# glacierbliss/iceberg_tracking_code

Measured on AMD Instinct MI355X. Metric: frame_pairs_per_sec, higher is better.
Workload: dtype u8/int32/f32

## Files before the change

### iceberg_tracking_code_amd/_lib.py

```python
import ctypes as C
import os

_HERE = os.path.dirname(os.path.abspath(__file__))
LIB_PATH = os.environ.get("ICELK_LIBRARY") or os.path.join(_HERE, "libicelk.so")

OK, EARG, ENOMEM, EHIP, ECAP, ESTATE, EUNSUP = 0, -1, -2, -3, -4, -5, -6

u8p = C.POINTER(C.c_uint8)
f32p = C.POINTER(C.c_float)
i32p = C.POINTER(C.c_int)
i64p = C.POINTER(C.c_int64)
f64p = C.POINTER(C.c_double)
vp = C.c_void_p
handle_p = C.c_void_p
i16p = C.POINTER(C.c_int16)


class JpegInfo(C.Structure):
    _fields_ = [("width", C.c_int32), ("height", C.c_int32), ("ncomp", C.c_int32), ("hmax", C.c_int32), ("vmax", C.c_int32),
                ("mcus_x", C.c_int32), ("mcus_y", C.c_int32), ("restart_interval", C.c_int32),
                ("comp_w", C.c_int32 * 3), ("comp_h", C.c_int32 * 3), ("blocks_x", C.c_int32 * 3), ("blocks_y", C.c_int32 * 3),
                ("coef_offset", C.c_uint64 * 3), ("coef_count", C.c_uint64), ("quant", (C.c_uint16 * 64) * 3)]


jpeg_info_p = C.POINTER(JpegInfo)


class JpegScan(C.Structure):
    _fields_ = [("segments", C.c_uint32), ("blocks_per_mcu", C.c_uint32), ("blocks_per_segment", C.c_uint32),
                ("total_blocks", C.c_uint32), ("component", C.c_uint8 * 8), ("dc_table", C.c_uint8 * 8), ("ac_table", C.c_uint8 * 8)]


class JpegHuffStats(C.Structure):
    _fields_ = [("segments", C.c_uint32), ("subsequences", C.c_uint32), ("rounds", C.c_uint32), ("max_hops", C.c_uint32),
                ("lanes_in_step", C.c_uint32), ("spanning_blocks", C.c_uint32), ("fallback", C.c_uint32), ("reserved", C.c_uint32),
                ("total_hops", C.c_uint64)]


JPEG_TABLE_BYTES = 11328
JPEG_FALLBACK_NONE, JPEG_FALLBACK_BOUND, JPEG_FALLBACK_STREAM, JPEG_FALLBACK_SIZE = 0, 1, 2, 3
jpeg_stats_p = C.POINTER(JpegHuffStats)

SIGNATURES = {
    "icelk_version": (C.c_int, []),
    "icelk_last_error": (C.c_char_p, [handle_p]),
    "icelk_create": (C.c_int, [C.c_int, C.c_int, C.c_int, C.c_int, C.c_int, C.POINTER(handle_p)]),
    "icelk_destroy": (C.c_int, [handle_p]),
    "icelk_set_stream": (C.c_int, [handle_p, vp]),
    "icelk_sync": (C.c_int, [handle_p]),
    "icelk_set_fb_distance": (C.c_int, [handle_p, C.c_int]),
    "icelk_set_lk_kernel": (C.c_int, [handle_p, C.c_int]),
    "icelk_upload_gray": (C.c_int, [handle_p, C.c_int, u8p, C.c_int, C.c_int, C.c_int]),
    "icelk_upload_bgr": (C.c_int, [handle_p, C.c_int, u8p, C.c_int, C.c_int, C.c_int, C.c_int]),
    "icelk_jpeg_describe": (C.c_int, [vp, C.c_uint64, jpeg_info_p]),
    "icelk_jpeg_read_coefficients": (C.c_int, [vp, C.c_uint64, vp, C.c_uint64]),
    "icelk_upload_jpeg": (C.c_int, [handle_p, C.c_int, jpeg_info_p, vp, C.c_int, C.c_int, C.c_int, C.c_int, C.c_int]),
    "icelk_jpeg_decode_rgb": (C.c_int, [handle_p, jpeg_info_p, vp, u8p, C.c_int]),
    "icelk_jpeg_index": (C.c_int, [vp, C.c_uint64, jpeg_info_p, C.POINTER(JpegScan), vp, vp, C.c_uint64, vp]),
    "icelk_jpeg_read_coefficients_lanes": (C.c_int, [vp, C.c_uint64, vp, C.c_uint64, C.c_int, C.c_int, C.c_int, jpeg_stats_p]),
    "icelk_jpeg_huff_config": (C.c_int, [handle_p, C.c_int, C.c_int, C.c_int]),
    "icelk_jpeg_huff_stats": (C.c_int, [handle_p, jpeg_stats_p]),
    "icelk_upload_jpeg_file": (C.c_int, [handle_p, C.c_int, vp, C.c_uint64, C.c_int, C.c_int, C.c_int, C.c_int, C.c_int]),
    "icelk_jpeg_decode_rgb_file": (C.c_int, [handle_p, vp, C.c_uint64, u8p, C.c_int]),
    "icelk_jpeg_device_coefficients": (C.c_int, [handle_p, vp, C.c_uint64, vp, C.c_uint64]),
    "icelk_set_gray_device": (C.c_int, [handle_p, C.c_int, vp, C.c_int, C.c_int, C.c_int]),
    "icelk_cvt_bgr_device": (C.c_int, [handle_p, C.c_int, vp, C.c_int, C.c_int, C.c_int, C.c_int]),
    "icelk_upload_gray_async": (C.c_int, [handle_p, C.c_int, vp, C.c_int, C.c_int, C.c_int]),
    "icelk_host_alloc": (C.c_int, [C.POINTER(vp), C.c_uint64]),
    "icelk_host_free": (C.c_int, [vp]),
    "icelk_synth_frame": (C.c_int, [handle_p, C.c_int, C.c_int, C.c_int, C.c_int64, C.c_int64, C.c_uint32]),
    "icelk_synth_frame_affine": (C.c_int, [handle_p, C.c_int, C.c_int, C.c_int, C.c_int64, C.c_int64, C.c_uint32, i32p]),
    "icelk_drop_pyramid": (C.c_int, [handle_p, C.c_int]),
    "icelk_download_level": (C.c_int, [handle_p, C.c_int, C.c_int, u8p, C.c_int, i32p, i32p]),
    "icelk_build_pyramid": (C.c_int, [handle_p, C.c_int, C.c_int, C.c_int, C.c_int, i32p]),
    "icelk_pyrlk": (C.c_int, [handle_p, C.c_int, C.c_int, f32p, f32p, u8p, f32p, C.c_int, C.c_int, C.c_int, C.c_int,
                              C.c_int, C.c_int, C.c_double, C.c_int, C.c_double]),
    "icelk_track_fb": (C.c_int, [handle_p, C.c_int, C.c_int, f32p, C.c_int, C.c_int, C.c_int, C.c_int, C.c_int,
                                 C.c_int, C.c_double, C.c_double, C.c_float, f32p, f32p, u8p, u8p, f32p, f32p, f32p,
                                 u8p]),
    "icelk_fb_filter": (C.c_int, [handle_p, f32p, f32p, C.c_int, C.c_float, f32p, u8p]),
    "icelk_set_mask": (C.c_int, [handle_p, u8p, C.c_int, C.c_int, C.c_int]),
    "icelk_min_eig_map": (C.c_int, [handle_p, C.c_int, C.c_int, f32p, C.c_int]),
    "icelk_good_features": (C.c_int, [handle_p, C.c_int, C.c_int, C.c_int, C.c_double, C.c_double, C.c_int, f32p,
                                      C.c_int, i32p]),
    "icelk_detect_stats": (C.c_int, [handle_p, i32p, i32p]),
    "icelk_seg_detect": (C.c_int, [handle_p, C.c_int, C.c_int, C.c_int, C.c_double, C.c_double, C.c_int, i32p]),
    "icelk_set_mask_polygon": (C.c_int, [handle_p, f64p, C.c_int, C.c_double, C.c_double, C.c_int, C.c_int]),
    "icelk_download_mask": (C.c_int, [handle_p, u8p, C.c_int, i32p, i32p]),
    "icelk_build_pyramid_ahead": (C.c_int, [handle_p, C.c_int, C.c_int, C.c_int, C.c_int]),
    "icelk_seg_detect_prepare": (C.c_int, [handle_p, C.c_int, C.c_int, C.c_int]),
    "icelk_seg_detect_begin": (C.c_int, [handle_p, C.c_int, C.c_int, C.c_int, C.c_double, C.c_double, C.c_int]),
    "icelk_seg_detect_finish": (C.c_int, [handle_p, C.c_int, i32p]),
    "icelk_seg_detect_cancel": (C.c_int, [handle_p]),
    "icelk_set_variant": (C.c_int, [handle_p, C.c_char_p, C.c_int]),
    "icelk_seg_detect_stage_try": (C.c_int, [handle_p, C.c_int, i32p, i32p]),
    "icelk_detect_fast_stats": (C.c_int, [handle_p, C.c_int, C.c_int, C.POINTER(C.c_longlong)]),
    "icelk_seg_detect_stage": (C.c_int, [handle_p, C.c_int, i32p]),
    "icelk_seg_switch": (C.c_int, [handle_p]),
    "icelk_seg_track": (C.c_int, [handle_p, C.c_int, C.c_int, C.c_int, C.c_int, C.c_int, C.c_int, C.c_int,
                                  C.c_double, C.c_double, C.c_float, i32p]),
    "icelk_seg_track_async": (C.c_int, [handle_p, C.c_int, C.c_int, C.c_int, C.c_int, C.c_int, C.c_int, C.c_int,
                                        C.c_double, C.c_double, C.c_float]),
    "icelk_seg_track_defer": (C.c_int, [handle_p, C.c_int, C.c_int, C.c_int, C.c_int, C.c_int, C.c_int, C.c_int,
                                        C.c_double, C.c_double, C.c_float]),
    "icelk_seg_flush": (C.c_int, [handle_p]),
    "icelk_seg_track_len_hint": (C.c_int, [handle_p, C.c_int]),
    "icelk_seg_template_stats": (C.c_int, [handle_p, C.POINTER(C.c_longlong)]),
    "icelk_seg_tail_stats": (C.c_int, [handle_p, C.POINTER(C.c_longlong)]),
    "icelk_seg_template_info": (C.c_int, [handle_p, C.POINTER(C.c_longlong), C.POINTER(C.c_longlong), i32p]),
    "icelk_seg_read_closed": (C.c_int, [handle_p, f32p, f32p, C.c_int, C.c_int, i32p, i32p]),
    "icelk_seg_archive_closed": (C.c_int, [handle_p, vp, vp, vp, C.c_int, i32p]),
    "icelk_seg_live": (C.c_int, [handle_p, i32p, i64p]),
    "icelk_seg_archive": (C.c_int, [handle_p, vp, vp, vp, C.c_int, i32p]),
    "icelk_project_tracks": (C.c_int, [handle_p, f32p, C.c_int, C.c_int, vp, vp, f64p, f64p, f64p, f64p, f64p, u8p]),
    "icelk_seg_project": (C.c_int, [handle_p, vp, vp, C.c_int, C.c_int, f64p, f64p, f64p, f64p, f64p, u8p, i32p, i32p]),
    "icelk_points_in_polygon": (C.c_int, [handle_p, f64p, C.c_int, f64p, C.c_int, u8p]),
    "icelk_grid_bin": (C.c_int, [handle_p, f64p, f64p, f64p, f64p, C.c_int, C.c_double, C.c_double, C.c_double, C.c_int,
                                 C.c_int, u8p, i32p, f64p, f64p, f64p]),
    "icelk_grid_bin_windows": (C.c_int, [handle_p, f64p, f64p, f64p, f64p, f64p, C.c_int, i64p, i32p, i32p, i32p,
                                         C.c_int, i64p, i64p, C.c_int, C.c_int, C.c_double, C.c_double, C.c_double,
                                         C.c_int, C.c_int, u8p, i32p, f64p, f64p, f64p, i32p, f64p, f64p, f64p]),
    "icelk_cube_set": (C.c_int, [handle_p, f64p, f64p, f64p, C.c_int, C.c_int]),
    "icelk_cube_release": (C.c_int, [handle_p]),
    "icelk_cube_average": (C.c_int, [handle_p, i32p, i32p, C.c_int, C.c_int, C.c_int, C.c_int, f64p, f64p, f64p, f64p,
                                     i32p, f64p]),
    "icelk_calib_set": (C.c_int, [handle_p, f64p, C.c_int, f64p, C.c_int, C.c_double, C.c_double]),
    "icelk_calib_release": (C.c_int, [handle_p]),
    "icelk_calib_residuals": (C.c_int, [handle_p, f64p, C.c_int, f64p, f64p, f64p, f64p]),
    "icelk_calib_cost": (C.c_int, [handle_p, f64p, C.c_int, f64p, f64p]),
    "icelk_seg_read": (C.c_int, [handle_p, f32p, f32p, C.c_int, C.c_int, i32p, i32p]),
    "icelk_prof_enable": (C.c_int, [handle_p, C.c_int]),
    "icelk_prof_reset": (C.c_int, [handle_p]),
    "icelk_prof_iterations": (C.c_int, [handle_p, C.POINTER(C.c_uint32), C.c_int, i32p]),
    "icelk_stream_probe_info": (C.c_int, [handle_p, i32p, f64p, f64p]),
    "icelk_prof_count": (C.c_int, []),
    "icelk_prof_name": (C.c_char_p, [C.c_int]),
    "icelk_prof_get": (C.c_int, [handle_p, C.c_int, i32p, f64p]),
}

_lib = None


class IcelkError(RuntimeError):
    """Raised for ICELK_EHIP / ICELK_ECAP / ICELK_ESTATE; bad arguments raise ValueError."""


def load():
    global _lib
    if _lib is None:
        if not os.path.exists(LIB_PATH):
            raise IcelkError(
                "libicelk.so is missing (%s). Build it with `python -m iceberg_tracking_code_amd.build` "
                "(needs hipcc); this package has no CPU fallback." % LIB_PATH)
        lib = C.CDLL(LIB_PATH)
        for name, (res, args) in SIGNATURES.items():
            fn = getattr(lib, name)
            fn.restype = res
            fn.argtypes = args
        _lib = lib
    return _lib


def check(rc, handle=None):
    if rc == OK:
        return
    msg = load().icelk_last_error(handle)
    msg = msg.decode() if msg else ""
    text = "icelk error %d: %s" % (rc, msg)
    if rc == EARG:
        raise ValueError(text)
    if rc == ENOMEM:
        raise MemoryError(text)
    raise IcelkError(text)
```

### iceberg_tracking_code_amd/context.py

```python
import ctypes as C

import numpy as np

from . import _lib
from ._lib import check, f32p, u8p

TERM_CRITERIA_COUNT = 1
TERM_CRITERIA_MAX_ITER = 1
TERM_CRITERIA_EPS = 2
OPTFLOW_USE_INITIAL_FLOW = 4
OPTFLOW_LK_GET_MIN_EIGENVALS = 8
GRAY_CV3 = 3
GRAY_CV4 = 4
LK_GENERIC_KERNEL = 0x100
LK_MULTI_PER_WAVE = 0x200
FB_HYPOT = 0
FB_SQRT = 1

DEFAULT_CRITERIA = (TERM_CRITERIA_COUNT | TERM_CRITERIA_EPS, 30, 0.01)


def _u8(a):
    return a.ctypes.data_as(u8p)

# ... 175 lines not shown
        st = np.zeros(n, np.uint8)
        er = np.zeros(n, np.float32)
        t, cnt, eps = _criteria(criteria)
        self._ck(self._lib.icelk_pyrlk(self._h, prev_slot, next_slot, _f32(p0), _f32(p1), _u8(st), _f32(er), n,
                                       winSize[0], winSize[1], maxLevel, t, cnt, eps, flags, minEigThreshold))
        return p1.reshape(-1, 1, 2), st.reshape(-1, 1), er.reshape(-1, 1)

    def track_fb(self, slot0, slot1, p0, winSize=(21, 21), maxLevel=3, criteria=DEFAULT_CRITERIA,
                 minEigThreshold=1e-4, fb_threshold=1.0):
        p0 = np.ascontiguousarray(p0, dtype=np.float32).reshape(-1, 2)
        n = p0.shape[0]
        out = dict(p1=np.zeros((n, 2), np.float32), p0r=np.zeros((n, 2), np.float32),
                   st_fwd=np.zeros(n, np.uint8), st_bwd=np.zeros(n, np.uint8),
                   err_fwd=np.zeros(n, np.float32), err_bwd=np.zeros(n, np.float32),
                   dist=np.zeros(n, np.float32), valid=np.zeros(n, np.uint8))
        t, cnt, eps = _criteria(criteria)
        self._ck(self._lib.icelk_track_fb(self._h, slot0, slot1, _f32(p0), n, winSize[0], winSize[1], maxLevel, t,
                                          cnt, eps, minEigThreshold, fb_threshold, _f32(out["p1"]),
                                          _f32(out["p0r"]), _u8(out["st_fwd"]), _u8(out["st_bwd"]),
                                          _f32(out["err_fwd"]), _f32(out["err_bwd"]), _f32(out["dist"]),
                                          _u8(out["valid"])))
        return out

    def fb_filter(self, p0, p0r, fb_threshold=1.0):
        a = np.ascontiguousarray(p0, dtype=np.float32).reshape(-1, 2)
        b = np.ascontiguousarray(p0r, dtype=np.float32).reshape(-1, 2)
        if a.shape != b.shape:
            raise ValueError("p0 and p0r differ in length")
        n = a.shape[0]
        dist, valid = np.zeros(n, np.float32), np.zeros(n, np.uint8)
        self._ck(self._lib.icelk_fb_filter(self._h, _f32(a), _f32(b), n, float(fb_threshold), _f32(dist), _u8(valid)))
        return dist, valid

    def set_mask(self, mask):
        if mask is None:
            self._ck(self._lib.icelk_set_mask(self._h, None, 0, 0, 0))
            return
        m = _gray2d(mask, "mask")
        self._ck(self._lib.icelk_set_mask(self._h, _u8(m), m.shape[1], m.shape[0], m.strides[0]))

    def set_mask_polygon(self, poly, crop_left, crop_top, w, h):
        p = np.ascontiguousarray(poly, dtype=np.float64).reshape(-1, 2)
        self._ck(self._lib.icelk_set_mask_polygon(self._h, p.ctypes.data_as(_lib.f64p), len(p), float(crop_left),
                                                  float(crop_top), int(w), int(h)))

    def download_mask(self):
        w, h = C.c_int(0), C.c_int(0)
        self._ck(self._lib.icelk_download_mask(self._h, None, 0, C.byref(w), C.byref(h)))
        m = np.empty((h.value, w.value), np.uint8)
        self._ck(self._lib.icelk_download_mask(self._h, _u8(m), w.value, C.byref(w), C.byref(h)))
        return m

    def min_eig_map(self, slot, blockSize=3):
        lvl = self.download_level(slot, 0)
        out = np.empty(lvl.shape, np.float32)
        self._ck(self._lib.icelk_min_eig_map(self._h, slot, blockSize, _f32(out), out.shape[1]))
        return out

    def good_features(self, slot, maxCorners, qualityLevel, minDistance, use_mask=False, blockSize=3):
        cap = self.max_pts if maxCorners <= 0 else min(int(maxCorners), self.max_pts)
        out = np.empty((max(cap, 1), 2), np.float32)
        n = C.c_int(0)
        self._ck(self._lib.icelk_good_features(self._h, slot, 1 if use_mask else 0, int(maxCorners),
                                               float(qualityLevel), float(minDistance), int(blockSize), _f32(out), cap,
                                               C.byref(n)))
        if n.value == 0:
            return None
        return out[:n.value].reshape(-1, 1, 2).copy()

    def detect_fast_stats(self, w, h):
        out = (C.c_longlong * 8)()
        self._ck(self._lib.icelk_detect_fast_stats(self._h, int(w), int(h), out))
        return dict(tiles=out[0], listed=out[1], whole_tiles=out[2], ties=out[3], max_listed=out[4], max_overflow_tiles=out[5],
                    longest_list=out[6], evaluated=out[7])

    def detect_stats(self):
        a, b = C.c_int(0), C.c_int(0)
        self._ck(self._lib.icelk_detect_stats(self._h, C.byref(a), C.byref(b)))
        return dict(candidates=a.value, accepted=b.value)

    def seg_detect(self, slot, maxCorners, qualityLevel, minDistance, use_mask=False, blockSize=3):
        n = C.c_int(0)
        self._ck(self._lib.icelk_seg_detect(self._h, slot, 1 if use_mask else 0, int(maxCorners), float(qualityLevel),
                                            float(minDistance), int(blockSize), C.byref(n)))
        return n.value

    def build_pyramid_ahead(self, slot, winSize=(21, 21), maxLevel=3):
        self._ck(self._lib.icelk_build_pyramid_ahead(self._h, slot, winSize[0], winSize[1], maxLevel))

    def seg_detect_prepare(self, slot, use_mask=False, blockSize=3):
        self._ck(self._lib.icelk_seg_detect_prepare(self._h, slot, 1 if use_mask else 0, int(blockSize)))

    def seg_detect_begin(self, slot, maxCorners, qualityLevel, minDistance, use_mask=False, blockSize=3):
        self._ck(self._lib.icelk_seg_detect_begin(self._h, slot, 1 if use_mask else 0, int(maxCorners),
                                                  float(qualityLevel), float(minDistance), int(blockSize)))

    def seg_detect_finish(self, maxCorners):
        n = C.c_int(0)
        self._ck(self._lib.icelk_seg_detect_finish(self._h, int(maxCorners), C.byref(n)))
        return n.value

    def seg_detect_stage(self, maxCorners):
        n = C.c_int(0)
        self._ck(self._lib.icelk_seg_detect_stage(self._h, int(maxCorners), C.byref(n)))
        return n.value

    def seg_detect_stage_try(self, maxCorners):
        n, done = C.c_int(0), C.c_int(0)
        self._ck(self._lib.icelk_seg_detect_stage_try(self._h, int(maxCorners), C.byref(n), C.byref(done)))
        return n.value if done.value else None

    def seg_detect_cancel(self):
        self._ck(self._lib.icelk_seg_detect_cancel(self._h))

    def seg_switch(self):
        self._ck(self._lib.icelk_seg_switch(self._h))

    def seg_track(self, slot_prev, slot_next, winSize=(21, 21), maxLevel=3, criteria=DEFAULT_CRITERIA,
                  minEigThreshold=1e-4, fb_threshold=1.0, wait=True):
        t, cnt, eps = _criteria(criteria)
        if wait:
            n = C.c_int(0)
            self._ck(self._lib.icelk_seg_track(self._h, slot_prev, slot_next, winSize[0], winSize[1], maxLevel, t, cnt,
                                               eps, minEigThreshold, fb_threshold, C.byref(n)))
            return n.value
        self._ck(self._lib.icelk_seg_track_async(self._h, slot_prev, slot_next, winSize[0], winSize[1], maxLevel, t,
                                                 cnt, eps, minEigThreshold, fb_threshold))
        return None

    def seg_track_defer(self, slot_prev, slot_next, winSize=(21, 21), maxLevel=3, criteria=DEFAULT_CRITERIA,
                        minEigThreshold=1e-4, fb_threshold=1.0):
        t, cnt, eps = _criteria(criteria)
        self._ck(self._lib.icelk_seg_track_defer(self._h, slot_prev, slot_next, winSize[0], winSize[1], maxLevel, t,
                                                 cnt, eps, minEigThreshold, fb_threshold))

    def seg_flush(self):
        self._ck(self._lib.icelk_seg_flush(self._h))

    def seg_template_stats(self):
        out = (C.c_longlong * 2)()
        self._ck(self._lib.icelk_seg_template_stats(self._h, out))
        return int(out[0]), int(out[1])

    def seg_template_info(self):
        by, rows, st = C.c_longlong(0), C.c_longlong(0), C.c_int(0)
        self._ck(self._lib.icelk_seg_template_info(self._h, C.byref(by), C.byref(rows), C.byref(st)))
        return int(by.value), int(rows.value), int(st.value)

    def seg_tail_stats(self):
        out = (C.c_longlong * 2)()
        self._ck(self._lib.icelk_seg_tail_stats(self._h, out))
        return int(out[0]), int(out[1])

    def seg_track_len_hint(self, track_len):
        self._ck(self._lib.icelk_seg_track_len_hint(self._h, int(track_len)))

    def seg_live(self):
        n, tot = C.c_int(0), C.c_int64(0)
        self._ck(self._lib.icelk_seg_live(self._h, C.byref(n), C.byref(tot)))
        return n.value, tot.value

    def seg_archive(self, dev_tracks_ptr, dev_quality_ptr, dev_count_ptr, cap_rows, closed=False):
        nv = C.c_int(0)
        fn = self._lib.icelk_seg_archive_closed if closed else self._lib.icelk_seg_archive
        self._ck(fn(self._h, C.c_void_p(dev_tracks_ptr), C.c_void_p(dev_quality_ptr or 0),
                                             C.c_void_p(dev_count_ptr), int(cap_rows), C.byref(nv)))
        return nv.value

    def seg_read(self, closed=False):
        n, nv = C.c_int(0), C.c_int(0)
        fn = self._lib.icelk_seg_read_closed if closed else self._lib.icelk_seg_read
        self._ck(fn(self._h, None, None, 0, 0, C.byref(n), C.byref(nv)))
        tracks = np.zeros((n.value, nv.value, 2), np.float32)
        quality = np.zeros((n.value, max(nv.value - 1, 0)), np.float32)
        if n.value:
            self._ck(fn(self._h, _f32(tracks), _f32(quality), n.value, nv.value, C.byref(n),
                                              C.byref(nv)))
        return tracks, quality

    def prof_enable(self, on=True):
        self._ck(self._lib.icelk_prof_enable(self._h, int(on)))

    def prof_reset(self):
        self._ck(self._lib.icelk_prof_reset(self._h))

    def prof_iterations(self):
        n = C.c_int(0)
        self._ck(self._lib.icelk_prof_iterations(self._h, None, 0, C.byref(n)))
        buf = np.zeros(max(n.value, 1), np.uint32)
        if n.value:
            self._ck(self._lib.icelk_prof_iterations(self._h, buf.ctypes.data_as(C.POINTER(C.c_uint32)), n.value,
                                                     C.byref(n)))
        buf = buf[:n.value]
        buf = buf[buf != 0xffffffff]
        return (buf & 0xffff).astype(np.int64), (buf >> 16).astype(np.int64)

    def stream_probe_info(self):
        picks = (C.c_int * 4)()
        q, lim = C.c_double(0), C.c_double(0)
        self._ck(self._lib.icelk_stream_probe_info(self._h, picks, C.byref(q), C.byref(lim)))
        return dict(detection=picks[0], candidates=picks[1], pyramid=picks[2], tail=picks[3], quickest=q.value,
                    limit=lim.value, probed=picks[0] >= 0)

    def prof_table(self):
        out = {}
        for k in range(self._lib.icelk_prof_count()):
            n, ms = C.c_int(0), C.c_double(0)
            self._ck(self._lib.icelk_prof_get(self._h, k, C.byref(n), C.byref(ms)))
            if n.value:
                out[self._lib.icelk_prof_name(k).decode()] = dict(launches=n.value, total_ms=ms.value,
                                                                  avg_us=1e3 * ms.value / n.value)
        return out
```

### iceberg_tracking_code_amd/csrc/abi_detect.hip

```cpp
#include "icelk_ctx.h"

namespace icelk {

int alloc_eig_out(Ctx* c, Ctx::EigOut& e, int cand_cap)
{
    const int w = c->max_w, h = c->max_h;
    int rc;
    if ((rc = dmalloc(c, &e.max_key, 1)) || (rc = dmalloc(c, &e.raw, (size_t)cand_cap)) ||
        (rc = dmalloc(c, &e.blk_count, candidate_blocks(w, h) * 4)))
        return rc;
    if (getenv("ICELK_TWO_PASS_CORNERS") &&
        ((rc = dmalloc(c, &e.acand, fast_cand_entries(w, h))) || (rc = dmalloc(c, &e.acount, fast_tiles(w, h))) ||
         (rc = dmalloc(c, &e.amaxc, fast_max_entries(w, h))) || (rc = dmalloc(c, &e.amaxn, fast_tiles(w, h))) ||
         (rc = dmalloc(c, &e.aemax, fast_tiles(w, h))) || (rc = dmalloc(c, &e.fmax_key, 8)) ||
         (rc = dmalloc(c, &e.aties, fast_cand_entries(w, h) + fast_tiles(w, h)))))
        return rc;
    if (hipEventCreateWithFlags(&e.done, hipEventDisableTiming) != hipSuccess) FAIL(c, ICELK_EHIP, "hipEventCreate failed");
    return ICELK_OK;
}

void free_eig_out(Ctx::EigOut& e)
{
    void* p[] = {e.raw, e.blk_count, e.max_key, e.acand, e.acount, e.amaxc, e.amaxn, e.aemax, e.fmax_key, e.aties};
    for (void* q : p)
// ... 135 lines not shown
static inline bool counts_here(const int* h_counts, int seq)
{
    return __atomic_load_n(h_counts + kCountsSeq, __ATOMIC_ACQUIRE) == seq;
}

static int fetch_counts(Ctx* c, Ctx::DetSet& S, bool published = false)
{
    if (!published) {
        int rc = publish_counts(c, S);
        if (rc) return rc;
    }
    for (unsigned it = 1;; it++) {
        if (counts_here(S.h_counts, S.counts_seq)) return ICELK_OK;
        if ((it & 4095u) == 0) {
            const hipError_t q = hipEventQuery(S.counts_ev);
            if (q == hipSuccess) break;
            if (q != hipErrorNotReady) HIPCHK(c, q);
            (void)hipGetLastError();
        }
        __builtin_ia32_pause();
    }
    HIPCHK(c, hipEventSynchronize(S.counts_ev));
    return ICELK_OK;
}

static int pick_mask(Ctx* c, int use_mask, int w, int h, const uint8_t** mask)
{
    *mask = nullptr;
    if (!use_mask) return ICELK_OK;
    if (!c->has_mask) FAIL(c, ICELK_ESTATE, "use_mask set but no mask uploaded");
    if (c->mask_w != w || c->mask_h != h) FAIL(c, ICELK_EARG, "mask size differs from the frame");
    *mask = c->d_mask;
    return ICELK_OK;
}

int detect_prepare(Ctx* c, int slot, int use_mask, int block_size)
{
    Range rg("icelk detect_prepare (corner candidates ahead)");
    int rc = check_slot(c, slot, true);
    if (rc) return rc;
    if (!fused_block_size(block_size) || getenv("ICELK_GENERIC_CORNERS") || c->corner_variant) return ICELK_OK;
    Slot& s = c->slots[slot];
    const uint8_t* mask = nullptr;
    if ((rc = pick_mask(c, use_mask, s.w, s.h, &mask))) return rc;
    const Ctx::EigOut want = eo_want(c, slot, use_mask, block_size);
    Ctx::EigOut& e = c->eo[eo_free(c, want)];
    if (eo_holds(e, want)) return ICELK_OK;
    const hipStream_t es = c->eig_stream;
    if (int rcw = wait_event(c, es, s.frame_ev)) return rcw;
    HIPCHK(c, hipMemsetAsync(e.max_key, 0, sizeof(unsigned), es));
    DetectScratch T{};
    point_at_eig_out(T, e);
    const double prep_quality = c->prep_quality;
    {
        ProfScope p(c, K_EIG, es);
        launch_candidates(es, T, s.lv[0], block_size, mask, c->mask_pitch, prep_quality, false, nullptr);
    }
    rc = check_launch(c, "corner candidates (prepared)");
    if (rc) return rc;
    HIPCHK(c, hipEventRecord(e.done, es));
    HIPCHK(c, hipEventRecord(s.eig_used, es));
    e.nblk = T.src_nblk;
    e.region = T.src_region;
    e.valid = true;
    e.slot = slot;
    e.gen = s.gen;
    e.block_size = block_size;
    e.use_mask = use_mask;
    e.mask_gen = c->mask_gen;
    e.quality = prep_quality;
    return ICELK_OK;
}

int detect_begin(Ctx* c, int slot, int use_mask, int max_corners, double quality, double min_distance, int block_size,
                 bool for_segment)
{
    Range rg("icelk detect_begin (candidates + min-distance stage)");
    int rc = check_slot(c, slot, true);
    if (rc) return rc;
    if (!(quality > 0) || min_distance < 0 || block_size <= 0) FAIL(c, ICELK_EARG, "bad detector parameters");
    if (min_eig_lds_bytes(block_size) > 150 * 1024) FAIL(c, ICELK_EARG, "blockSize too large");
    const int k = det_free(c);
    if (k < 0) FAIL(c, ICELK_ESTATE, "two detections are in flight already");
    c->dset_last = k;
    Ctx::DetSet& S = c->dset[k];
    Slot& s = c->slots[slot];
    const hipStream_t ds = c->det_stream;
    const int w = s.w, h = s.h;
    const uint8_t* mask = nullptr;
    if ((rc = pick_mask(c, use_mask, w, h, &mask))) return rc;
    DetectScratch& D = S.D;
    size_t ncell = 0;
    if (min_distance >= 1) {
        const int cell = (int)lrint(min_distance);
        ncell = (size_t)((w + cell - 1) / cell) * ((h + cell - 1) / cell);
        if (ncell + 1 > c->ncell_cap) FAIL(c, ICELK_ECAP, "cell grid larger than allocated");
    }
    if (int rcw = wait_event(c, ds, s.frame_ev)) return rcw;
    if (int rcw = wait_event(c, ds, S.tail_done)) return rcw;
    const bool generic = getenv("ICELK_GENERIC_CORNERS") != nullptr || c->corner_variant != 0;
    const bool need_reset = !S.counters_clean || ncell > S.reset_ncell;
    const Ctx::EigOut want = eo_want(c, slot, use_mask, block_size);
    const int spare_idx = eo_free(c, want);
    Ctx::EigOut& spare = c->eo[spare_idx];
    const bool prepared = eo_holds(spare, want) && !generic && spare.quality <= quality;
    c->prep_quality = quality;
    spare.valid = false;
    if (prepared) {
        if (need_reset) launch_detect_reset(ds, D, (int)ncell, 1);
        activate_eig_out(c, S, spare_idx);
        if (int rcw = wait_event(c, ds, spare.done)) return rcw;
    } else {
        ProfScope p(c, K_EIG, ds);
        activate_eig_out(c, S, spare_idx);
        if (int rcw = wait_event(c, ds, spare.done)) return rcw;
        HIPCHK(c, hipMemsetAsync(spare.max_key, 0, sizeof(unsigned), ds));
        if (need_reset) launch_detect_reset(ds, D, (int)ncell, 1);
        launch_candidates(ds, D, s.lv[0], block_size, mask, c->mask_pitch, quality, generic, nullptr, c->corner_variant);
        HIPCHK(c, hipEventRecord(s.det_used, ds));
    }
    S.counters_clean = false;
    rc = check_launch(c, "corner candidates");
    if (rc) return rc;
    DetectJob& J = S.job;
    J.w = w;
    J.h = h;
    J.quality = quality;
    J.min_distance = min_distance;
    J.ncell = ncell;
    J.prune_want = 0;
    if (min_distance >= 1 && max_corners > 0 && max_corners <= (1 << 24) && !getenv("ICELK_NO_PRUNE"))
        J.prune_want = (int)std::min(8.0 * max_corners, std::ceil(c->prune_factor * max_corners));
    J.dev_tail = false;
    J.seg_set = -1;
    J.max_corners = max_corners;
    const bool dev_tail = for_segment && !c->host_tail && min_distance >= 1;
    if (min_distance >= 1) {
        J.cand_count_ptr = D.cell_start + ncell;
        ProfScope p(c, K_SUPPRESS, ds);
        launch_min_distance(ds, D, w, h, min_distance, quality, J.prune_want, dev_tail);
        if (dev_tail)
            launch_tail_gather(ds, D, (int)ncell, quality, suppress_launch_count() - 1, max_corners, c->max_pts, c->tail_force_status);
    } else {
        J.cand_count_ptr = D.cand_count;
        launch_flatten(ds, D, quality);
    }
    rc = check_launch(c, "min_distance");
    if (rc) return rc;
    if (dev_tail) {
        const Ctx::DetSet& other = c->dset[k ^ 1];
        const int ahead = (c->seg_staged ? 1 : 0) + (other.job.active ? 1 : 0);
        const int target = (c->sb_cur + 1 + ahead) % kSegSets;
        Ctx::SegBuf& nb = c->sb[target];
        if (int rcw = wait_event(c, ds, nb.used)) return rcw;
        S.counts_seq = (S.counts_seq + 1) & 0x3fffffff;
        {
            ProfScope p(c, K_EMIT, ds);
            launch_tail_device(ds, D, quality, nb.live, nb.alive, nb.tracks, kMaxVert, c->use_order ? nb.order : nullptr,
                               nb.order_border, tail_order_geometry(w, h, c->border_px), tail_reset_of(D, (int)ncell),
                               S.h_counts, kCountsSeq, S.counts_seq);
        }
        rc = check_launch(c, "tail (device-driven)");
        if (rc) return rc;
        HIPCHK(c, hipEventRecord(nb.ready, ds));
        HIPCHK(c, hipEventRecord(S.counts_ev, ds));
        J.dev_tail = true;
        J.seg_set = target;
    } else {
        rc = publish_counts(c, S);
        if (rc) return rc;
    }
    J.active = true;
    J.seq = ++c->job_seq;
    return ICELK_OK;
}

int detect_finish(Ctx* c, int max_corners, int cap, int* n_out, Ctx::SegBuf* seg, bool* seg_done, bool* dev_done,
                  DetectJob* finished)
{
    Range rg("icelk detect_finish (host round trip, sort, corner list)");
    if (seg_done) *seg_done = false;
    if (dev_done) *dev_done = false;
    const int k = det_oldest(c);
    if (k < 0) FAIL(c, ICELK_ESTATE, "no detection in flight");
    c->dset_last = k;
    Ctx::DetSet& S = c->dset[k];
    DetectJob& J = S.job;
    J.active = false;
    if (finished) *finished = J;
    *n_out = 0;
    const hipStream_t ds = c->det_stream;
    const hipStream_t ts = c->tail_stream;
    DetectScratch& D = S.D;
    int rc = fetch_counts(c, S, true);
    if (rc) return rc;
    if (J.dev_tail) {
        const int status = S.h_counts[5];
        if (!seg || seg != &c->sb[J.seg_set] || max_corners != J.max_corners)
            FAIL(c, ICELK_ESTATE, "the segment staged is not the one its detection was begun for (set / maxCorners differ)");
        if (status == TAIL_OVERFLOW) FAIL(c, ICELK_ECAP, "more corners than the output capacity (raise max_pts)");
        if (status == TAIL_OK) {
            const int total = S.h_counts[1], n = S.h_counts[4];
            if (n > cap) FAIL(c, ICELK_ECAP, "more corners than the output capacity (raise max_pts)");
            if (J.prune_want > 0 && max_corners > 0)
                c->prune_factor = !S.h_counts[3] || total <= 0 ? 8.0 : std::min(8.0, std::max(2.0, 1.5 * (double)S.h_counts[0] / total));
            c->last_candidates = S.h_counts[0];
            c->last_accepted = total;
            S.reset_ncell = J.ncell;
            S.counters_clean = true;
            c->tails_dev++;
            *n_out = n;
            if (seg_done) *seg_done = true;
            if (dev_done) *dev_done = true;
            return ICELK_OK;
        }
    }
    c->tails_host++;
    const unsigned long long* sorted = nullptr;
    int total = 0;
    if (J.min_distance >= 1) {
        auto converge = [&]() -> int {
            for (int guard = 0; S.h_counts[2] != 0; guard++) {
                if (guard > 100000) FAIL(c, ICELK_EHIP, "min-distance suppression did not converge");
                continue_min_distance(ds, D, J.w, J.h, J.min_distance);
                int r = fetch_counts(c, S);
                if (r) return r;
            }
            return ICELK_OK;
        };
        if ((rc = converge())) return rc;
        bool redone = false;
        if (J.prune_want > 0 && S.h_counts[3] && (max_corners <= 0 || S.h_counts[1] < max_corners)) {
            redone = true;
            launch_detect_reset(ds, D, (int)J.ncell, 0);
            launch_min_distance(ds, D, J.w, J.h, J.min_distance, J.quality, 0);
            if ((rc = check_launch(c, "min_distance (unpruned)"))) return rc;
            if ((rc = fetch_counts(c, S))) return rc;
            if ((rc = converge())) return rc;
        }
        total = S.h_counts[1];
        if (J.prune_want > 0 && max_corners > 0) {
            const bool fell_short = !S.h_counts[3] || redone;
            c->prune_factor = fell_short || total <= 0 ? 8.0 : std::min(8.0, std::max(2.0, 1.5 * (double)S.h_counts[0] / total));
        }
        c->last_candidates = S.h_counts[0];
        c->last_accepted = total;
        if (total == 0) return ICELK_OK;
        sort_keys_desc(ts, D, D.acc, D.acc_sorted, total);
        sorted = D.acc_sorted;
    } else {
        total = S.h_counts[0];
        c->last_candidates = total;
        c->last_accepted = total;
        if (total == 0) return ICELK_OK;
        sort_keys_desc(ts, D, D.cand, D.cell_cand, total);
        sorted = D.cell_cand;
    }
    rc = check_launch(c, "sort");
    if (rc) return rc;
    int n = total;
    if (max_corners > 0 && n > max_corners) n = max_corners;
    if (n > cap || n > c->max_pts) FAIL(c, ICELK_ECAP, "more corners than the output capacity (raise max_pts)");
    if (seg) {
        if (int rcw = wait_event(c, ts, seg->used)) return rcw;
        {
            ProfScope p(c, K_EMIT, ts);
            launch_tail_fused(ts, sorted, n, c->d_corners, seg->live, seg->alive, seg->tracks, kMaxVert, D, (int)J.ncell, 1);
        }
        rc = check_launch(c, "tail");
        if (rc) return rc;
        HIPCHK(c, hipEventRecord(c->det_done, ts));
        HIPCHK(c, hipEventRecord(S.tail_done, ts));
        *seg_done = true;
    } else {
        {
            ProfScope p(c, K_EMIT, ts);
            launch_emit_corners(ts, sorted, n, J.w, c->d_corners);
        }
        rc = check_launch(c, "emit");
        if (rc) return rc;
        HIPCHK(c, hipEventRecord(c->det_done, ts));
        launch_detect_reset(ts, D, (int)J.ncell, 1);
        HIPCHK(c, hipEventRecord(S.tail_done, ts));
    }
    S.reset_ncell = J.ncell;
    S.counters_clean = true;
    *n_out = n;
    return ICELK_OK;
}

static int detect_core(Ctx* c, int slot, int use_mask, int max_corners, double quality, double min_distance,
                       int block_size, int cap, int* n_out)
{
    *n_out = 0;
    if (det_oldest(c) >= 0) FAIL(c, ICELK_ESTATE, "a detection is in flight (icelk_seg_detect_begin without _stage / _finish)");
    int rc = detect_begin(c, slot, use_mask, max_corners, quality, min_distance, block_size, false);
    if (rc) return rc;
    return detect_finish(c, max_corners, cap, n_out);
}

int detect_counts_arrived(Ctx* c, bool* arrived)
{
    *arrived = false;
    const int k = det_oldest(c);
    if (k < 0) FAIL(c, ICELK_ESTATE, "no detection in flight");
    if (!counts_here(c->dset[k].h_counts, c->dset[k].counts_seq)) {
// ... 181 lines not shown
```

### iceberg_tracking_code_amd/csrc/abi_handle.hip

```cpp
#include <dlfcn.h>

#include <chrono>

#include "icelk_ctx.h"

namespace icelk {

static const char* kKernelNames[K_COUNT_] = {
    "bgr2gray", "pyrdown", "lk", "lk_fb", "corner_candidates", "min_distance", "sort_emit",
    "project_tracks", "synth", "lk_fb_pair", "jpeg_idct", "jpeg_out", "jpeg_huff",
};

std::string g_create_err;
std::mutex g_mu;

Roctx::Roctx()
{
    if (!getenv("ICELK_ROCTX")) return;
    void* lib = dlopen("librocprofiler-sdk-roctx.so", RTLD_NOW | RTLD_GLOBAL);
    if (!lib) lib = dlopen("libroctx64.so", RTLD_NOW | RTLD_GLOBAL);
    if (!lib) return;
    push = reinterpret_cast<int (*)(const char*)>(dlsym(lib, "roctxRangePushA"));
    pop = reinterpret_cast<int (*)()>(dlsym(lib, "roctxRangePop"));
    if (!push || !pop) push = nullptr;
}

Roctx& roctx()
{
    static Roctx r;
    return r;
}

void prof_drain(Ctx* c)
{
    for (auto& e : c->evts) {
        hipEventSynchronize(e.b);
        float ms = 0.f;
        if (hipEventElapsedTime(&ms, e.a, e.b) == hipSuccess) {
            c->prof_ms[e.id] += ms;
            c->prof_launches[e.id] += 1;
        }
        c->evt_pool.push_back(e);
    }
    c->evts.clear();
}

hipError_t create_priority_stream(hipStream_t* s)
{
    int least = 0, greatest = 0;
    hipError_t e = hipDeviceGetStreamPriorityRange(&least, &greatest);
    if (e != hipSuccess) return e;
    return hipStreamCreateWithPriority(s, hipStreamNonBlocking, greatest);
}

__global__ void k_probe_idle(unsigned ticks)
{
    const unsigned long long t0 = __builtin_amdgcn_s_memrealtime();
    for (int guard = 0; guard < 200000; guard++) {
        if (__builtin_amdgcn_s_memrealtime() - t0 >= ticks) break;
        __builtin_amdgcn_s_sleep(8);
    }
}

__global__ void k_probe_tick(unsigned* out)
{
    if (out) *out = 1u;
}

static double probe_pair(hipStream_t busy, hipStream_t side, hipEvent_t e_busy, hipEvent_t e_side)
{
    using clk = std::chrono::steady_clock;
    hipStreamSynchronize(busy);
    hipStreamSynchronize(side);
    const auto t0 = clk::now();
    hipLaunchKernelGGL(k_probe_idle, dim3(65536), dim3(64), 0, busy, 2500u);
    hipEventRecord(e_busy, busy);
    hipLaunchKernelGGL(k_probe_tick, dim3(1), dim3(64), 0, side, (unsigned*)nullptr);
    hipEventRecord(e_side, side);
    hipEventSynchronize(e_side);
    const auto t1 = clk::now();
    hipEventSynchronize(e_busy);
    const auto t2 = clk::now();
    const double whole = std::chrono::duration<double>(t2 - t0).count();
    const double frac = whole > 0 ? std::chrono::duration<double>(t1 - t0).count() / whole : 1.0;
    if (getenv("ICELK_STREAM_PROBE_LOG"))
        fprintf(stderr, "icelk probe: busy %p side %p: side done after %.2f of %.0f us\n", (void*)busy, (void*)side, frac, 1e6 * whole);
    return frac;
}

static hipError_t create_side_streams(Ctx* c)
{
    constexpr int NC = 8;
    hipStream_t cand[NC] = {nullptr};
    hipEvent_t ea = nullptr, eb = nullptr;
    hipError_t r = hipEventCreateWithFlags(&ea, hipEventDisableTiming);
    if (r == hipSuccess) r = hipEventCreateWithFlags(&eb, hipEventDisableTiming);
    for (int i = 0; i < NC && r == hipSuccess; i++) r = create_priority_stream(&cand[i]);
    if (r == hipSuccess) {
        probe_pair(c->own_stream, cand[0], ea, eb);
        double beside[NC], quickest = 1.0;
        for (int i = 0; i < NC; i++) {
            beside[i] = std::min(probe_pair(c->own_stream, cand[i], ea, eb), probe_pair(c->own_stream, cand[i], ea, eb));
            quickest = std::min(quickest, beside[i]);
        }
        const double limit = std::max(1.6 * quickest, quickest + 0.12);
        bool used[NC] = {false};
        auto pick = [&](auto ok) {
            for (int i = 0; i < NC; i++)
                if (!used[i] && beside[i] <= limit && ok(cand[i])) { used[i] = true; return i; }
            for (int i = 0; i < NC; i++)
                if (!used[i]) { used[i] = true; return i; }
            return 0;
        };
        const int d = pick([&](hipStream_t) { return true; });
        c->det_stream = cand[d];
        const int e = pick([&](hipStream_t s) { return probe_pair(s, c->det_stream, ea, eb) <= limit; });
        c->eig_stream = cand[e];
        const int q = pick([&](hipStream_t s) { return probe_pair(c->eig_stream, s, ea, eb) <= limit; });
        c->pyr_stream = cand[q];
        const int t = pick([&](hipStream_t s) { return probe_pair(c->eig_stream, s, ea, eb) <= limit; });
        c->tail_stream = cand[t];
        c->side_pick[0] = d;
        c->side_pick[1] = e;
        c->side_pick[2] = q;
        c->side_pick[3] = t;
        c->probe_limit = limit;
        c->probe_quickest = quickest;
        if (getenv("ICELK_STREAM_PROBE_LOG"))
            fprintf(stderr, "icelk probe: detection = candidate %d, candidates stream = %d, pyramid = %d (limit %.2f)\n", d, e, q, limit);
        for (int i = 0; i < NC; i++)
            if (!used[i]) hipStreamDestroy(cand[i]);
    } else {
        for (auto s : cand)
            if (s) hipStreamDestroy(s);
    }
    if (ea) hipEventDestroy(ea);
    if (eb) hipEventDestroy(eb);
    return r;
}

static void destroy_ctx(Ctx* c)
{
    if (!c) return;
    hipSetDevice(c->device);
    if (c->stream) hipStreamSynchronize(c->stream);
    prof_drain(c);
    for (auto& e : c->evt_pool) {
        hipEventDestroy(e.a);
        hipEventDestroy(e.b);
    }
    if (c->d_stamps) {
        std::vector<unsigned long long> hs(3 * c->stamps_cap);
        if (hipMemcpy(hs.data(), c->d_stamps, hs.size() * 8, hipMemcpyDeviceToHost) == hipSuccess) {
            if (FILE* f = fopen(c->stamps_path.c_str(), "wb")) {
                fwrite(hs.data(), 8, hs.size(), f);
                fclose(f);
            }
        }
        hipFree(c->d_stamps);
    }
    if (c->d_iters) hipFree(c->d_iters);
    for (void* b : c->tmpl.buf)
        if (b) hipFree(b);
    for (auto& s : c->slots) {
        if (s.base) hipFree(s.base);
        if (s.ready) hipEventDestroy(s.ready);
        if (s.frame_ev) hipEventDestroy(s.frame_ev);
        if (s.used_own) hipEventDestroy(s.used_own);
        if (s.det_used) hipEventDestroy(s.det_used);
        if (s.eig_used) hipEventDestroy(s.eig_used);
    }
    if (c->det_stream) hipStreamSynchronize(c->det_stream);
    if (c->eig_stream) hipStreamSynchronize(c->eig_stream);
    if (c->det_done) hipEventDestroy(c->det_done);
    if (c->corners_free) hipEventDestroy(c->corners_free);
    if (c->det_stream) hipStreamDestroy(c->det_stream);
    if (c->eig_stream) hipStreamDestroy(c->eig_stream);
    for (auto& b : c->sb) {
        if (b.used_own) hipEventDestroy(b.used_own);
        if (b.ready) hipEventDestroy(b.ready);
    }
    for (auto& e : c->launch_ev)
        if (e) hipEventDestroy(e);
    for (auto& e : c->eo) free_eig_out(e);
    for (auto& S : c->dset) free_det_set(S);
    if (c->h_seg) hipHostFree(c->h_seg);
    void* ptrs[] = {c->d_bgr, c->d_mask, c->d_p0, c->d_p1, c->d_p0r, c->d_err_f, c->d_err_b, c->d_dist, c->d_corners,
                    c->d_st_f, c->d_st_b, c->d_valid, c->dset[0].D.eig, c->d_tracked,
                    c->d_out_tracks, c->d_out_quality, c->post.d_proj, c->post.d_keep, c->post.d_cube_u, c->post.d_cube_v,
                    c->post.d_cube_count, c->calib.d_shore, c->calib.d_water, c->jpeg.d_coef, c->jpeg.d_planes, c->jpeg.d_rgb,
                    c->jpeg.d_file, c->jpeg.d_seg, c->jpeg.d_tabs, c->jpeg.d_T, c->jpeg.d_X, c->jpeg.d_cnt, c->jpeg.d_P, c->jpeg.d_ctl,
                    c->jpeg.d_dc};
    for (void* p : ptrs)
        if (p) hipFree(p);
    for (auto& S : c->sb) {
        void* sp[] = {S.live, S.alive, S.order, S.order_border, S.tracks, S.quality};
        for (void* p : sp)
            if (p) hipFree(p);
    }
    if (c->own_stream) hipStreamDestroy(c->own_stream);
    for (auto q : c->copy_hi)
        if (q) {
            hipStreamSynchronize(q);
            hipStreamDestroy(q);
        }
    if (c->pyr_stream) {
        hipStreamSynchronize(c->pyr_stream);
        hipStreamDestroy(c->pyr_stream);
    }
    if (c->tail_stream) {
        hipStreamSynchronize(c->tail_stream);
        hipStreamDestroy(c->tail_stream);
    }
    delete c;
}

}

using namespace icelk;

extern "C" {

int icelk_version(void) { return 100; }

const char* icelk_last_error(icelk_t* h)
{
    if (!h) return g_create_err.c_str();
    return C(h)->err.c_str();
}

int icelk_create(int device, int max_w, int max_h, int n_slots, int max_pts, icelk_t** out)
{
    std::lock_guard<std::mutex> lk(g_mu);
    if (!out || max_w <= 0 || max_h <= 0 || max_w > 65535 || max_h > 65535 || n_slots <= 0 || max_pts <= 0) {
        g_create_err = "icelk_create: bad argument";
        return ICELK_EARG;
    }
    *out = nullptr;
    int ndev = 0;
    hipError_t e = hipGetDeviceCount(&ndev);
    if (e != hipSuccess || ndev == 0) {
        g_create_err = std::string("icelk_create: no HIP device (") + hipGetErrorString(e) + ")";
        return ICELK_EHIP;
    }
    if (device < 0 || device >= ndev) {
        g_create_err = "icelk_create: device index out of range";
        return ICELK_EARG;
    }
    e = hipSetDevice(device);
    if (e != hipSuccess) {
        g_create_err = std::string("hipSetDevice: ") + hipGetErrorString(e);
        return ICELK_EHIP;
    }
    Ctx* c = new Ctx();
    c->device = device;
    c->max_w = max_w;
    c->max_h = max_h;
    c->n_slots = n_slots;
    c->max_pts = max_pts;
    int rc = ICELK_OK;
    auto fail = [&](int code) {
        g_create_err = c->err;
        destroy_ctx(c);
        return code;
    };
    if (hipStreamCreateWithFlags(&c->own_stream, hipStreamNonBlocking) != hipSuccess ||
        create_side_streams(c) != hipSuccess ||
        hipHostMalloc(reinterpret_cast<void**>(&c->h_seg), 64, hipHostMallocMapped) != hipSuccess ||
        hipEventCreateWithFlags(&c->det_done, hipEventDisableTiming) != hipSuccess ||
        hipEventCreateWithFlags(&c->corners_free, hipEventDisableTiming) != hipSuccess) {
        c->err = "hipStreamCreate failed";
        return fail(ICELK_EHIP);
    }
    c->stream = c->own_stream;
    c->slots.resize(n_slots);
    const size_t sb = slot_bytes(max_w, max_h);
    for (auto& s : c->slots) {
        if ((rc = dmalloc(c, &s.base, sb))) return fail(rc);
        s.bytes = sb;
        if (hipEventCreateWithFlags(&s.ready, hipEventDisableTiming) != hipSuccess ||
            hipEventCreateWithFlags(&s.frame_ev, hipEventDisableTiming) != hipSuccess ||
            hipEventCreateWithFlags(&s.used_own, hipEventDisableTiming) != hipSuccess ||
            hipEventCreateWithFlags(&s.det_used, hipEventDisableTiming) != hipSuccess ||
            hipEventCreateWithFlags(&s.eig_used, hipEventDisableTiming) != hipSuccess) {
            c->err = "hipEventCreate failed";
            return fail(ICELK_EHIP);
        }
        s.used = s.used_own;
        layout_levels(s, max_w, max_h);
        if (!layout_ok(s)) {
            c->err = "slot layout violates the dword-access invariant (internal)";
            return fail(ICELK_ECAP);
        }
    }
    for (auto& S : c->sb) {
        if (hipEventCreateWithFlags(&S.used_own, hipEventDisableTiming) != hipSuccess ||
            hipEventCreateWithFlags(&S.ready, hipEventDisableTiming) != hipSuccess) {
            c->err = "hipEventCreate failed";
            return fail(ICELK_EHIP);
        }
        S.used = S.used_own;
    }
    for (auto& e : c->launch_ev)
        if (hipEventCreateWithFlags(&e, hipEventDisableTiming) != hipSuccess) {
            c->err = "hipEventCreate failed";
            return fail(ICELK_EHIP);
        }
    const size_t npx = (size_t)max_w * max_h;
    c->bgr_pitch = align_up(3 * max_w, kPitchAlign);
    c->mask_pitch = align_up(max_w, kPitchAlign);
    const size_t np = (size_t)max_pts;
    const int cand_cap = (int)std::min<size_t>(candidate_capacity(max_w, max_h), (size_t)1 << 30);
    c->ncell_cap = npx + 1;
    if ((rc = dmalloc(c, &c->d_bgr, (size_t)c->bgr_pitch * max_h)) || (rc = dmalloc(c, &c->d_mask, (size_t)c->mask_pitch * max_h)) ||
        (rc = dmalloc(c, &c->d_p0, 2 * np)) || (rc = dmalloc(c, &c->d_p1, 2 * np)) || (rc = dmalloc(c, &c->d_p0r, 2 * np)) ||
        (rc = dmalloc(c, &c->d_err_f, np)) || (rc = dmalloc(c, &c->d_err_b, np)) || (rc = dmalloc(c, &c->d_dist, np)) ||
        (rc = dmalloc(c, &c->d_corners, 2 * np)) || (rc = dmalloc(c, &c->d_st_f, np)) || (rc = dmalloc(c, &c->d_st_b, np)) ||
        (rc = dmalloc(c, &c->d_valid, np)) || (rc = dmalloc(c, &c->dset[0].D.eig, npx)) || (rc = dmalloc(c, &c->d_tracked, 64)) ||
        (rc = dmalloc(c, &c->d_out_tracks, np * kMaxVert * 2)) || (rc = dmalloc(c, &c->d_out_quality, np * (kMaxVert - 1))))
        return fail(rc);
    for (auto& S : c->sb)
        if ((rc = dmalloc(c, &S.live, 2 * np)) || (rc = dmalloc(c, &S.alive, np)) || (rc = dmalloc(c, &S.order, np)) ||
            (rc = dmalloc(c, &S.order_border, 1)) || (rc = dmalloc(c, &S.tracks, np * kMaxVert * 2)) ||
            (rc = dmalloc(c, &S.quality, np * (kMaxVert - 1))))
            return fail(rc);
    c->use_order = getenv("ICELK_NO_ORDER") == nullptr;
    c->pyr_per_level = getenv("ICELK_PYR_PER_LEVEL") != nullptr;
    c->tmpl.off = getenv("ICELK_NO_TEMPLATE_REUSE") != nullptr;
    if (const char* tb = getenv("ICELK_TEMPLATE_BUDGET_MB")) c->tmpl.budget = (size_t)std::max(atoll(tb), 0LL) << 20;
    c->host_tail = getenv("ICELK_HOST_TAIL") != nullptr;
    if (const char* fs = getenv("ICELK_TAIL_FORCE_STATUS")) c->tail_force_status = std::min(std::max(atoi(fs), 0), 4);
    if ((rc = dmalloc(c, &c->d_iters, (size_t)max_pts))) return fail(rc);
    if (const char* sp = getenv("ICELK_LK_STAMPS")) {
        c->stamps_path = sp;
        c->stamps_cap = (size_t)max_pts + 8;
        if ((rc = dmalloc(c, &c->d_stamps, 3 * c->stamps_cap))) return fail(rc);
    }
    if (const char* k = getenv("ICELK_LK_KERNEL")) {
        if (!strcmp(k, "generic")) c->lk_kernel_flags = ICELK_FLAG_GENERIC_KERNEL;
        else if (!strcmp(k, "multi")) c->lk_kernel_flags = ICELK_FLAG_MULTI_PER_WAVE;
    }
    for (auto& e : c->eo)
        if ((rc = alloc_eig_out(c, e, cand_cap))) return fail(rc);
    for (int k = 0; k < 2; k++) {
        Ctx::DetSet& S = c->dset[k];
        S.D.eig = c->dset[0].D.eig;
        if ((rc = alloc_det_set(c, S, cand_cap))) return fail(rc);
        activate_eig_out(c, S, k);
    }
    if (hipMemset(c->d_tracked, 0, 64 * 8) != hipSuccess) {
        c->err = "hipMemset failed";
        return fail(ICELK_EHIP);
    }
    DetectScratch& D0 = c->dset[0].D;
    if (hipMemsetAsync(D0.acc, 0, 64 * sizeof(unsigned long long), c->tail_stream) != hipSuccess) {
        c->err = "hipMemset failed";
        return fail(ICELK_EHIP);
    }
    sort_keys_desc(c->tail_stream, D0, D0.acc, D0.acc_sorted, 64);
    if (hipStreamSynchronize(c->tail_stream) != hipSuccess) {
        c->err = "warm-up sort failed";
        return fail(ICELK_EHIP);
    }
    *out = reinterpret_cast<icelk_t*>(c);
    return ICELK_OK;
}

int icelk_destroy(icelk_t* h)
{
    if (!h) return ICELK_EARG;
    destroy_ctx(C(h));
    return ICELK_OK;
}

int icelk_set_stream(icelk_t* h, void* hip_stream)
{
    if (!h) return ICELK_EARG;
    Ctx* c = C(h);
    HIPCHK(c, hipSetDevice(c->device));
    HIPCHK(c, hipStreamSynchronize(c->stream));
    c->stream = hip_stream ? reinterpret_cast<hipStream_t>(hip_stream) : c->own_stream;
    return ICELK_OK;
}

int icelk_sync(icelk_t* h)
{
    if (!h) return ICELK_EARG;
    Ctx* c = C(h);
    HIPCHK(c, hipSetDevice(c->device));
    int rcf = flush_deferred(c);
    if (rcf) return rcf;
    for (auto q : c->copy_hi)
        if (q) HIPCHK(c, hipStreamSynchronize(q));
    HIPCHK(c, hipStreamSynchronize(c->pyr_stream));
    HIPCHK(c, hipStreamSynchronize(c->eig_stream));
    HIPCHK(c, hipStreamSynchronize(c->det_stream));
    HIPCHK(c, hipStreamSynchronize(c->tail_stream));
    HIPCHK(c, hipStreamSynchronize(c->stream));
    return ICELK_OK;
}

int icelk_set_lk_kernel(icelk_t* h, int which)
{
    if (!h) return ICELK_EARG;
    Ctx* c = C(h);
    if (which != 0 && which != ICELK_FLAG_GENERIC_KERNEL && which != ICELK_FLAG_MULTI_PER_WAVE)
        FAIL(c, ICELK_EARG, "bad kernel selector");
    c->lk_kernel_flags = which;
    return ICELK_OK;
}

int icelk_set_variant(icelk_t* h, const char* name, int value)
{
    if (!h || !name) return ICELK_EARG;
    Ctx* c = C(h);
    if (!strcmp(name, "lk_sums") && value >= 0 && value <= 2) c->lk_sum_mode = value;
    else if (!strcmp(name, "lk_wide_sums") && (value == 0 || value == 1)) c->lk_wide_sums = value;
    else if (!strcmp(name, "sobel_fma") && value >= 0 && value <= 3) c->corner_variant = (c->corner_variant & 4) | value;
    else if (!strcmp(name, "eig_fma") && (value == 0 || value == 1)) c->corner_variant = (c->corner_variant & 3) | (value << 2);
    else FAIL(c, ICELK_EARG, "unknown variant / value");
    for (auto& e : c->eo) e.valid = false;
    return ICELK_OK;
}

int icelk_set_fb_distance(icelk_t* h, int form)
{
    if (!h) return ICELK_EARG;
    Ctx* c = C(h);
    if (form != ICELK_FB_HYPOT && form != ICELK_FB_SQRT) FAIL(c, ICELK_EARG, "bad forward-backward distance form");
    c->fb_dist_form = form;
    return ICELK_OK;
}

int icelk_prof_enable(icelk_t* h, int on)
{
    if (!h) return ICELK_EARG;
    Ctx* c = C(h);
    if (!on) prof_drain(c);
    c->prof = on != 0;
    c->prof_tracker_only = on == 2;
    return ICELK_OK;
}

int icelk_prof_reset(icelk_t* h)
{
    if (!h) return ICELK_EARG;
    Ctx* c = C(h);
    prof_drain(c);
    for (int i = 0; i < K_COUNT_; i++) {
        c->prof_launches[i] = 0;
        c->prof_ms[i] = 0;
    }
    return ICELK_OK;
}

int icelk_prof_iterations(icelk_t* h, uint32_t* host_out, int cap, int* out_n)
{
    if (!h) return ICELK_EARG;
    Ctx* c = C(h);
    HIPCHK(c, hipSetDevice(c->device));
    if (!out_n || cap < 0 || (cap > 0 && !host_out)) FAIL(c, ICELK_EARG, "bad output buffer");
    *out_n = c->iters_n;
    if (host_out && cap > 0 && c->iters_n > 0) {
        const int n = c->iters_n < cap ? c->iters_n : cap;
        HIPCHK(c, hipStreamSynchronize(c->stream));
        HIPCHK(c, hipMemcpy(host_out, c->d_iters, sizeof(uint32_t) * (size_t)n, hipMemcpyDeviceToHost));
    }
    return ICELK_OK;
}

int icelk_stream_probe_info(icelk_t* h, int* picks, double* quickest, double* limit)
{
    if (!h) return ICELK_EARG;
    Ctx* c = C(h);
    if (picks)
        for (int k = 0; k < 4; k++) picks[k] = c->side_pick[k];
    if (quickest) *quickest = c->probe_quickest;
    if (limit) *limit = c->probe_limit;
    return ICELK_OK;
}

int icelk_prof_count(void) { return K_COUNT_; }

const char* icelk_prof_name(int kernel_id)
{
    if (kernel_id < 0 || kernel_id >= K_COUNT_) return "";
    return kKernelNames[kernel_id];
}

int icelk_prof_get(icelk_t* h, int kernel_id, int* launches, double* total_ms)
{
    if (!h) return ICELK_EARG;
    Ctx* c = C(h);
    if (kernel_id < 0 || kernel_id >= K_COUNT_) FAIL(c, ICELK_EARG, "bad kernel id");
    prof_drain(c);
    if (launches) *launches = c->prof_launches[kernel_id];
    if (total_ms) *total_ms = c->prof_ms[kernel_id];
    return ICELK_OK;
}

}
```

### iceberg_tracking_code_amd/csrc/abi_lk.hip

```cpp
#include "icelk_ctx.h"

namespace icelk {

int make_lk_params(Ctx* c, int w, int h, int win_w, int win_h, int max_level, int crit_type, int max_count,
                   double epsilon, int flags, double min_eig_thr, float fb_thr, LKParams* P)
{
    if (win_w <= 2 || win_h <= 2) FAIL(c, ICELK_EARG, "winSize must be > 2");
    if (max_level < 0) FAIL(c, ICELK_EARG, "maxLevel must be >= 0");
    if (max_level > kMaxLevels - 1) max_level = kMaxLevels - 1;
    if (win_w * win_h > 64 * 64) FAIL(c, ICELK_EARG, "winSize area above 4096 px is not supported");
    P->win_w = win_w;
    P->win_h = win_h;
    P->top_level = pyramid_top_level(w, h, win_w, win_h, max_level);
    if (!(crit_type & ICELK_CRIT_COUNT)) max_count = 30;
    else max_count = std::min(std::max(max_count, 0), 100);
    if (!(crit_type & ICELK_CRIT_EPS)) epsilon = 0.01;
    else epsilon = std::min(std::max(epsilon, 0.), 10.);
    P->max_count = max_count;
    P->eps2 = epsilon * epsilon;
    if (P->eps2 < 1e-30) {
        P->eps2_lo = -1.f;
        P->eps2_hi = INFINITY;
    } else {
        P->eps2_lo = nextafterf((float)(P->eps2 * (1.0 - 1.0 / (1 << 20))), -INFINITY);
        P->eps2_hi = nextafterf((float)(P->eps2 * (1.0 + 1.0 / (1 << 20))), INFINITY);
    }
    P->flags = flags | c->lk_kernel_flags;
    P->min_eig_thr = (float)min_eig_thr;
    P->fb_thr = fb_thr;
    P->margin = 6;
    P->dist_form = c->fb_dist_form;
    P->sum_mode = c->lk_sum_mode;
    P->sum_guard = c->lk_wide_sums ? 0u : 1u << 26;
    return ICELK_OK;
}

static int lk_prologue(Ctx* c, int slot0, int slot1, const float* p0, bool have_bufs, int n, int win_w, int win_h,
                       int max_level, int crit_type, int max_count, double epsilon, int flags, double min_eig_threshold,
                       float fb_threshold, LKParams* P)
{
    int rc = check_slot(c, slot0, true);
    if (!rc) rc = check_slot(c, slot1, true);
    if (rc) return rc;
    if (n < 0) FAIL(c, ICELK_EARG, "negative point count");
    if (n > c->max_pts) FAIL(c, ICELK_ECAP, "more points than max_pts of icelk_create");
    const Slot& s0 = c->slots[slot0];
    const Slot& s1 = c->slots[slot1];
    if (s0.w != s1.w || s0.h != s1.h) FAIL(c, ICELK_EARG, "frame sizes differ");
    rc = make_lk_params(c, s0.w, s0.h, win_w, win_h, max_level, crit_type, max_count, epsilon, flags, min_eig_threshold,
                        fb_threshold, P);
    if (rc) return rc;
    if (n == 0) return ICELK_OK;
    if (!have_bufs) FAIL(c, ICELK_EARG, "null point buffer");
    rc = ensure_pyramid(c, slot0, P->top_level);
    if (!rc) rc = ensure_pyramid(c, slot1, P->top_level);
    if (rc) return rc;
    HIPCHK(c, hipMemcpyAsync(c->d_p0, p0, sizeof(float) * 2 * n, hipMemcpyHostToDevice, c->stream));
    return ICELK_OK;
}

}

using namespace icelk;

extern "C" {

int icelk_pyrlk(icelk_t* h, int prev_slot, int next_slot, const float* prev_xy, float* next_xy, uint8_t* status,
                float* err, int n, int win_w, int win_h, int max_level, int crit_type, int max_count, double epsilon,
                int flags, double min_eig_threshold)
{
    if (!h) return ICELK_EARG;
    Ctx* c = C(h);
    HIPCHK(c, hipSetDevice(c->device));
    LKParams P;
    int rc = lk_prologue(c, prev_slot, next_slot, prev_xy, prev_xy && next_xy, n, win_w, win_h, max_level, crit_type,
                         max_count, epsilon, flags, min_eig_threshold, 1.f, &P);
    if (rc || n == 0) return rc;
    const Slot& s0 = c->slots[prev_slot];
    const Slot& s1 = c->slots[next_slot];
    if (flags & ICELK_FLAG_INITIAL_FLOW)
        HIPCHK(c, hipMemcpyAsync(c->d_p1, next_xy, sizeof(float) * 2 * n, hipMemcpyHostToDevice, c->stream));
    LKBuffers B{};
    B.p_in = c->d_p0;
    B.p_fwd = c->d_p1;
    B.st_fwd = c->d_st_f;
    B.err_fwd = err ? c->d_err_f : nullptr;
    if (c->prof) { B.iters = c->d_iters; c->iters_n = n; }
    {
        ProfScope p(c, K_LK);
        rc = launch_lk(c->stream, pyramid_of(s0), pyramid_of(s1), B, n, P, false);
    }
    if (rc) FAIL(c, rc, "unsupported window size");
    rc = check_launch(c, "lk");
    if (rc) return rc;
    HIPCHK(c, hipMemcpyAsync(next_xy, c->d_p1, sizeof(float) * 2 * n, hipMemcpyDeviceToHost, c->stream));
    if (status) HIPCHK(c, hipMemcpyAsync(status, c->d_st_f, n, hipMemcpyDeviceToHost, c->stream));
    if (err) HIPCHK(c, hipMemcpyAsync(err, c->d_err_f, sizeof(float) * n, hipMemcpyDeviceToHost, c->stream));
    HIPCHK(c, hipStreamSynchronize(c->stream));
    return ICELK_OK;
}

int icelk_track_fb(icelk_t* h, int slot0, int slot1, const float* p0, int n, int win_w, int win_h, int max_level,
                   int crit_type, int max_count, double epsilon, double min_eig_threshold, float fb_threshold,
                   float* p1, float* p0r, uint8_t* st_fwd, uint8_t* st_bwd, float* err_fwd, float* err_bwd, float* dist,
                   uint8_t* valid)
{
    if (!h) return ICELK_EARG;
    Ctx* c = C(h);
    HIPCHK(c, hipSetDevice(c->device));
    LKParams P;
    int rc = lk_prologue(c, slot0, slot1, p0, p0 != nullptr, n, win_w, win_h, max_level, crit_type, max_count, epsilon, 0,
                         min_eig_threshold, fb_threshold, &P);
    if (rc || n == 0) return rc;
    const Slot& s0 = c->slots[slot0];
    const Slot& s1 = c->slots[slot1];
    LKBuffers B{};
    B.p_in = c->d_p0;
    B.p_fwd = c->d_p1;
    B.st_fwd = c->d_st_f;
    B.err_fwd = err_fwd ? c->d_err_f : nullptr;
    B.p_bwd = c->d_p0r;
    B.st_bwd = c->d_st_b;
    B.err_bwd = err_bwd ? c->d_err_b : nullptr;
    B.dist = c->d_dist;
    B.valid = c->d_valid;
    if (c->prof) { B.iters = c->d_iters; c->iters_n = n; }
    {
        ProfScope p(c, K_LK_FB);
        rc = launch_lk(c->stream, pyramid_of(s0), pyramid_of(s1), B, n, P, true);
    }
    if (rc) FAIL(c, rc, "unsupported window size");
    rc = check_launch(c, "lk_fb");
    if (rc) return rc;
    const size_t fb = sizeof(float) * n;
    if (p1) HIPCHK(c, hipMemcpyAsync(p1, c->d_p1, 2 * fb, hipMemcpyDeviceToHost, c->stream));
    if (p0r) HIPCHK(c, hipMemcpyAsync(p0r, c->d_p0r, 2 * fb, hipMemcpyDeviceToHost, c->stream));
    if (st_fwd) HIPCHK(c, hipMemcpyAsync(st_fwd, c->d_st_f, n, hipMemcpyDeviceToHost, c->stream));
    if (st_bwd) HIPCHK(c, hipMemcpyAsync(st_bwd, c->d_st_b, n, hipMemcpyDeviceToHost, c->stream));
    if (err_fwd) HIPCHK(c, hipMemcpyAsync(err_fwd, c->d_err_f, fb, hipMemcpyDeviceToHost, c->stream));
    if (err_bwd) HIPCHK(c, hipMemcpyAsync(err_bwd, c->d_err_b, fb, hipMemcpyDeviceToHost, c->stream));
    if (dist) HIPCHK(c, hipMemcpyAsync(dist, c->d_dist, fb, hipMemcpyDeviceToHost, c->stream));
    if (valid) HIPCHK(c, hipMemcpyAsync(valid, c->d_valid, n, hipMemcpyDeviceToHost, c->stream));
    HIPCHK(c, hipStreamSynchronize(c->stream));
    return ICELK_OK;
}

int icelk_fb_filter(icelk_t* h, const float* p0, const float* p0r, int n, float fb_threshold, float* dist,
                    uint8_t* valid)
{
    if (!h) return ICELK_EARG;
    Ctx* c = C(h);
    HIPCHK(c, hipSetDevice(c->device));
    if (n < 0) FAIL(c, ICELK_EARG, "negative point count");
    if (n > c->max_pts) FAIL(c, ICELK_ECAP, "more points than max_pts of icelk_create");
    if (n == 0) return ICELK_OK;
    if (!p0 || !p0r) FAIL(c, ICELK_EARG, "null point buffer");
    HIPCHK(c, hipMemcpyAsync(c->d_p0, p0, sizeof(float) * 2 * n, hipMemcpyHostToDevice, c->stream));
    HIPCHK(c, hipMemcpyAsync(c->d_p0r, p0r, sizeof(float) * 2 * n, hipMemcpyHostToDevice, c->stream));
    launch_fb_filter(c->stream, c->d_p0, c->d_p0r, n, fb_threshold, c->fb_dist_form, c->d_dist, c->d_valid);
    int rc = check_launch(c, "fb_filter");
    if (rc) return rc;
    if (dist) HIPCHK(c, hipMemcpyAsync(dist, c->d_dist, sizeof(float) * n, hipMemcpyDeviceToHost, c->stream));
    if (valid) HIPCHK(c, hipMemcpyAsync(valid, c->d_valid, n, hipMemcpyDeviceToHost, c->stream));
    HIPCHK(c, hipStreamSynchronize(c->stream));
    return ICELK_OK;
}

}
```

### iceberg_tracking_code_amd/csrc/abi_segments.hip

```cpp
#include "icelk_ctx.h"

namespace icelk {

static int seg_wait(Ctx* c)
{
    if (c->seg_ready_pending) {
        if (int rcw = wait_event(c, c->stream, c->sb[c->sb_cur].ready)) return rcw;
        c->seg_ready_pending = false;
    }
    return ICELK_OK;
}

static LKJob seg_job(Ctx* c, int set, const Slot& s0, const Slot& s1, const LKParams& P, bool primary)
{
    Ctx::SegBuf& S = c->sb[set];
    LKJob j{};
    j.I = pyramid_of(s0);
    j.J = pyramid_of(s1);
    j.n = S.upper;
    LKBuffers& B = j.B;
    B.p_in = S.live;
    if (primary) {
        B.p_fwd = c->d_p1;
        B.st_fwd = c->d_st_f;
        B.p_bwd = c->d_p0r;
        B.st_bwd = c->d_st_b;
        B.dist = c->d_dist;
        B.valid = c->d_valid;
    }
    B.seg_alive = S.alive;
    B.order = c->use_order ? S.order : nullptr;
    B.order_border = c->use_order ? S.order_border : nullptr;
    const double overlap = (double)(P.win_w + 12) * (P.win_h + 12) * S.upper / ((double)s0.w * s0.h);
    B.order_plain = overlap >= 2.0 ? 1 : 0;
    B.seg_xy = S.live;
    B.seg_tracks = S.tracks;
    B.seg_quality = S.quality;
    B.seg_vert = S.vert;
    B.seg_max_vert = kMaxVert;
    B.seg_tracked = c->d_tracked;
    const int quads = lk_fast_eligible(P) ? lk_template_quads(P.win_w, P.win_h) : 0;
    const int key = (P.win_w << 16) | (P.win_h << 8) | (P.top_level + 1);
    const int slot0 = (int)(&s0 - c->slots.data()), slot1 = (int)(&s1 - c->slots.data());
    bool take = quads > 0 && S.tmpl_for == S.vert && S.tmpl_key == key && S.tmpl_slot == slot0 && S.tmpl_gen == s0.gen;
    S.tmpl_for = -1;
    if (quads > 0 && !c->tmpl.off) {
        const bool last = c->track_len_hint > 0 && S.vert >= c->track_len_hint;
        const size_t per_row = (size_t)(P.top_level + 1) * ((size_t)quads * 64) * 16;
        const size_t need = (size_t)std::max(S.upper, 1) * per_row;
        if (!last && c->tmpl.row_bytes != per_row) {
            if (c->defer.pending) (void)flush_deferred(c);
            for (void*& b : c->tmpl.buf) {
                if (b) hipFree(b);
                b = nullptr;
            }
            c->tmpl.bytes = 0;
            c->tmpl.row_bytes = per_row;
            for (Ctx::SegBuf& o : c->sb) o.tmpl_for = -1;
            size_t free_b = 0, total_b = 0;
            if (hipMemGetInfo(&free_b, &total_b) != hipSuccess) free_b = 0;
            const size_t budget = std::min(c->tmpl.budget / 2, free_b / 4);
            const size_t rows = std::min((size_t)std::max(c->max_pts, 1), budget / per_row);
            const size_t alloc = rows * per_row;
            if (rows > 0 && hipMalloc(&c->tmpl.buf[0], alloc) == hipSuccess && hipMalloc(&c->tmpl.buf[1], alloc) == hipSuccess) {
                c->tmpl.bytes = alloc;
            } else {
                (void)hipGetLastError();
                if (c->tmpl.buf[0]) hipFree(c->tmpl.buf[0]);
                c->tmpl.buf[0] = c->tmpl.buf[1] = nullptr;
                c->tmpl.off = true;
                c->tmpl.failed = true;
            }
        }
        if (c->tmpl.row_bytes != per_row) take = false;
        if (c->tmpl.bytes >= need && c->tmpl.row_bytes == per_row) {
            B.tmpl_levels = P.top_level + 1;
            if (take) {
                B.tmpl_in = c->tmpl.buf[set & 1];
                c->tmpl.taken++;
            }
            if (!last) {
                c->tmpl.left++;
                B.tmpl_out = c->tmpl.buf[set & 1];
                S.tmpl_for = S.vert + 1;
                S.tmpl_key = key;
                S.tmpl_slot = slot1;
                S.tmpl_gen = s1.gen;
            }
        }
    }
    return j;
}

static int record_launch(Ctx* c, hipEvent_t* ev)
{
    *ev = c->launch_ev[c->launch_seq++ % kLaunchEvents];
    HIPCHK(c, hipEventRecord(*ev, c->stream));
    return ICELK_OK;
}

static void seg_launched(Ctx* c, hipEvent_t ev, int set, int slot_prev, int slot_next)
{
    c->slots[slot_prev].used = ev;
    c->slots[slot_next].used = ev;
    c->sb[set].used = ev;
}

int flush_deferred(Ctx* c)
{
    if (!c->defer.pending) return ICELK_OK;
    Ctx::Deferred& d = c->defer;
    d.pending = false;
    int rc;
    {
        ProfScope p(c, K_LK_FB);
        rc = launch_lk(c->stream, d.job.I, d.job.J, d.job.B, d.job.n, d.P, true);
    }
    if (rc) FAIL(c, rc, "unsupported window size");
    rc = check_launch(c, "lk_fb");
    if (rc) return rc;
    hipEvent_t ev;
    rc = record_launch(c, &ev);
    if (rc) return rc;
    seg_launched(c, ev, d.set, d.slot_prev, d.slot_next);
    return ICELK_OK;
}

int flush_deferred_slot(Ctx* c, int slot)
{
    if (c->defer.pending && (c->defer.slot_prev == slot || c->defer.slot_next == slot)) return flush_deferred(c);
    return ICELK_OK;
}

static bool same_lk_params(const LKParams& a, const LKParams& b)
{
    return a.win_w == b.win_w && a.win_h == b.win_h && a.top_level == b.top_level && a.max_count == b.max_count &&
           a.eps2 == b.eps2 && a.flags == b.flags && a.min_eig_thr == b.min_eig_thr && a.fb_thr == b.fb_thr &&
           a.margin == b.margin && a.dist_form == b.dist_form && a.sum_mode == b.sum_mode &&
           a.sum_guard == b.sum_guard;
}

static int seg_track_core(Ctx* c, int slot_prev, int slot_next, int win_w, int win_h, int max_level, int crit_type,
                          int max_count, double epsilon, double min_eig_threshold, float fb_threshold, bool defer)
{
    Range rg(defer ? "icelk seg_track_defer" : "icelk seg_track (fused forward+backward LK launch)");
    int rc = check_slot(c, slot_prev, true);
    if (!rc) rc = check_slot(c, slot_next, true);
    if (rc) return rc;
    if (!c->seg_active) FAIL(c, ICELK_ESTATE, "icelk_seg_detect has not been called");
    Ctx::SegBuf& S = c->sb[c->sb_cur];
    if (S.vert >= kMaxVert) FAIL(c, ICELK_ECAP, "segment longer than the device track table");
    Slot& s0 = c->slots[slot_prev];
    Slot& s1 = c->slots[slot_next];
    if (s0.w != s1.w || s0.h != s1.h) FAIL(c, ICELK_EARG, "frame sizes differ");
    LKParams P;
    rc = make_lk_params(c, s0.w, s0.h, win_w, win_h, max_level, crit_type, max_count, epsilon, 0, min_eig_threshold,
                        fb_threshold, &P);
    if (rc) return rc;
    if (c->defer.pending && c->defer.set == c->sb_cur) {
        rc = flush_deferred(c);
        if (rc) return rc;
    }
    rc = ensure_pyramid(c, slot_prev, P.top_level);
    if (!rc) rc = ensure_pyramid(c, slot_next, P.top_level);
    if (rc) return rc;
    rc = seg_wait(c);
    if (rc) return rc;
    if (S.upper > 0) {
        c->border_px = (std::max(win_w, win_h) / 2 + kLkTileMargin + 2) << std::max(P.top_level - 1, 0);
        LKJob job = seg_job(c, c->sb_cur, s0, s1, P, true);
        static const bool stamp_pairs = getenv("ICELK_LK_STAMPS_PAIR") != nullptr;
        const bool diag = c->d_stamps != nullptr && !stamp_pairs;
        if (defer && !c->defer.pending && !diag) {
            Ctx::Deferred& d = c->defer;
            d.pending = true;
            d.set = c->sb_cur;
            d.slot_prev = slot_prev;
            d.slot_next = slot_next;
            d.job = job;
            d.P = P;
            S.vert += 1;
            return ICELK_OK;
        }
        bool paired = false;
        if (c->defer.pending) {
            Ctx::Deferred& d = c->defer;
            if (!diag && same_lk_params(d.P, P)) {
                LKJob other = d.job;
                other.B.p_fwd = other.B.p_bwd = other.B.err_fwd = other.B.err_bwd = other.B.dist = nullptr;
                other.B.st_fwd = other.B.st_bwd = other.B.valid = nullptr;
                if (c->d_stamps && stamp_pairs && (size_t)(other.n + job.n + 32) <= c->stamps_cap) {
                    other.B.stamps = job.B.stamps = c->d_stamps;
                    hipMemsetAsync(c->d_stamps, 0, 3 * c->stamps_cap * 8, c->stream);
                }
                {
                    ProfScope p(c, K_LK_FB_PAIR);
                    paired = launch_lk_pair(c->stream, other, job, P);
                }
                if (paired) {
                    d.pending = false;
                    rc = check_launch(c, "lk_fb_pair");
                    if (rc) return rc;
                }
            }
            if (!paired) {
                rc = flush_deferred(c);
                if (rc) return rc;
            }
        }
        if (!paired) {
            LKBuffers& B = job.B;
            if (c->prof) {
                B.iters = c->d_iters;
                c->iters_n = S.upper;
                hipMemsetAsync(c->d_iters, 0xff, sizeof(uint32_t) * (size_t)S.upper, c->stream);
            }
            if (c->d_stamps && !stamp_pairs) {
                B.stamps = c->d_stamps;
                hipMemsetAsync(c->d_stamps, 0, 3 * c->stamps_cap * 8, c->stream);
            }
            {
                ProfScope p(c, K_LK_FB);
                rc = launch_lk(c->stream, job.I, job.J, B, job.n, P, true);
            }
            if (rc) FAIL(c, rc, "unsupported window size");
            rc = check_launch(c, "lk_fb");
            if (rc) return rc;
        }
        hipEvent_t ev;
        rc = record_launch(c, &ev);
        if (rc) return rc;
        if (paired) seg_launched(c, ev, c->defer.set, c->defer.slot_prev, c->defer.slot_next);
        seg_launched(c, ev, c->sb_cur, slot_prev, slot_next);
    } else if (c->defer.pending && !defer) {
        rc = flush_deferred(c);
        if (rc) return rc;
    }
    S.vert += 1;
    return ICELK_OK;
}

}

using namespace icelk;

extern "C" {

int icelk_seg_detect_begin(icelk_t* h, int slot, int use_mask, int max_corners, double quality_level,
                            double min_distance, int block_size)
{
    if (!h) return ICELK_EARG;
    Ctx* c = C(h);
    HIPCHK(c, hipSetDevice(c->device));
    return detect_begin(c, slot, use_mask, max_corners, quality_level, min_distance, block_size, true);
}

int icelk_seg_detect_prepare(icelk_t* h, int slot, int use_mask, int block_size)
{
    if (!h) return ICELK_EARG;
    Ctx* c = C(h);
    HIPCHK(c, hipSetDevice(c->device));
    if (block_size <= 0) FAIL(c, ICELK_EARG, "bad detector parameters");
    return detect_prepare(c, slot, use_mask, block_size);
}

static int seg_stage(Ctx* c, int max_corners, int* out_n)
{
    if (c->seg_staged) FAIL(c, ICELK_ESTATE, "a staged segment is waiting for icelk_seg_switch");
    int n = 0;
    Ctx::SegBuf& nb = c->sb[(c->sb_cur + 1) % kSegSets];
    bool tables_written = false, dev_done = false;
    DetectJob job;
    int rc = detect_finish(c, max_corners, c->max_pts, &n, &nb, &tables_written, &dev_done, &job);
    if (rc) return rc;
    if (!dev_done) {
        const hipStream_t ds = c->tail_stream;
        if (!tables_written) {
            if (int rcw = wait_event(c, ds, nb.used)) return rcw;
            launch_seg_init(ds, c->d_corners, n, nb.live, nb.alive, nb.tracks, kMaxVert);
        }
        if (c->use_order) launch_seg_order(ds, c->d_corners, n, job.w, job.h, c->border_px, nb.order, nb.order_border);
        rc = check_launch(c, "seg_init");
        if (rc) return rc;
        HIPCHK(c, hipEventRecord(c->corners_free, ds));
        HIPCHK(c, hipEventRecord(nb.ready, ds));
    }
    c->seg_staged = true;
    c->staged_n = n;
    if (out_n) *out_n = n;
    return ICELK_OK;
}

static int seg_switch(Ctx* c)
{
    if (!c->seg_staged) FAIL(c, ICELK_ESTATE, "no staged segment (icelk_seg_detect_stage has not been called)");
    if (c->defer.pending && c->defer.set != c->sb_cur) {
        int rc = flush_deferred(c);
        if (rc) return rc;
    }
    c->seg_staged = false;
    c->closed_valid = c->seg_active;
    c->sb_cur = (c->sb_cur + 1) % kSegSets;
    c->seg_ready_pending = true;
    c->sb[c->sb_cur].vert = 1;
    c->sb[c->sb_cur].tmpl_for = -1;
    c->sb[c->sb_cur].upper = c->staged_n;
    c->seg_active = true;
    return ICELK_OK;
}

int icelk_seg_detect_stage(icelk_t* h, int max_corners, int* out_n)
{
    if (!h) return ICELK_EARG;
    Ctx* c = C(h);
    HIPCHK(c, hipSetDevice(c->device));
    return seg_stage(c, max_corners, out_n);
}

int icelk_seg_detect_stage_try(icelk_t* h, int max_corners, int* out_n, int* out_done)
{
    if (!h || !out_done) return ICELK_EARG;
    Ctx* c = C(h);
    HIPCHK(c, hipSetDevice(c->device));
    *out_done = 0;
    if (c->seg_staged) FAIL(c, ICELK_ESTATE, "a staged segment is waiting for icelk_seg_switch");
    bool arrived = false;
    int rc = detect_counts_arrived(c, &arrived);
    if (rc || !arrived) return rc;
    rc = seg_stage(c, max_corners, out_n);
    if (rc) return rc;
    *out_done = 1;
    return ICELK_OK;
}

int icelk_seg_switch(icelk_t* h)
{
    if (!h) return ICELK_EARG;
    return seg_switch(C(h));
}

int icelk_seg_detect_cancel(icelk_t* h)
{
    if (!h) return ICELK_EARG;
    Ctx* c = C(h);
    HIPCHK(c, hipSetDevice(c->device));
    HIPCHK(c, hipStreamSynchronize(c->eig_stream));
    HIPCHK(c, hipStreamSynchronize(c->det_stream));
    HIPCHK(c, hipStreamSynchronize(c->tail_stream));
    for (auto& S : c->dset)
        if (S.job.active) {
            S.job.active = false;
            S.counters_clean = false;
        }
    for (auto& e : c->eo) e.valid = false;
    c->seg_staged = false;
    return ICELK_OK;
}

int icelk_seg_detect_finish(icelk_t* h, int max_corners, int* out_n)
{
    if (!h) return ICELK_EARG;
    Ctx* c = C(h);
    HIPCHK(c, hipSetDevice(c->device));
    int rc = seg_stage(c, max_corners, out_n);
    if (rc) return rc;
    return seg_switch(c);
}

int icelk_seg_detect(icelk_t* h, int slot, int use_mask, int max_corners, double quality_level, double min_distance,
                     int block_size, int* out_n)
{
    int rc = icelk_seg_detect_begin(h, slot, use_mask, max_corners, quality_level, min_distance, block_size);
    if (rc) return rc;
    return icelk_seg_detect_finish(h, max_corners, out_n);
}

int icelk_seg_track_async(icelk_t* h, int slot_prev, int slot_next, int win_w, int win_h, int max_level, int crit_type,
                          int max_count, double epsilon, double min_eig_threshold, float fb_threshold)
{
    if (!h) return ICELK_EARG;
    Ctx* c = C(h);
    HIPCHK(c, hipSetDevice(c->device));
    return seg_track_core(c, slot_prev, slot_next, win_w, win_h, max_level, crit_type, max_count, epsilon,
                          min_eig_threshold, fb_threshold, false);
}

int icelk_seg_track_defer(icelk_t* h, int slot_prev, int slot_next, int win_w, int win_h, int max_level, int crit_type,
                          int max_count, double epsilon, double min_eig_threshold, float fb_threshold)
{
    if (!h) return ICELK_EARG;
    Ctx* c = C(h);
    HIPCHK(c, hipSetDevice(c->device));
    return seg_track_core(c, slot_prev, slot_next, win_w, win_h, max_level, crit_type, max_count, epsilon,
                          min_eig_threshold, fb_threshold, true);
}

int icelk_seg_track_len_hint(icelk_t* h, int track_len)
{
    if (!h || track_len < 0) return ICELK_EARG;
    C(h)->track_len_hint = track_len;
    return ICELK_OK;
}

int icelk_seg_template_stats(icelk_t* h, long long* out)
{
    if (!h || !out) return ICELK_EARG;
    out[0] = C(h)->tmpl.taken;
    out[1] = C(h)->tmpl.left;
    return ICELK_OK;
}

int icelk_seg_template_info(icelk_t* h, long long* bytes_per_table, long long* rows, int* state)
{
    if (!h) return ICELK_EARG;
    Ctx* c = C(h);
    if (bytes_per_table) *bytes_per_table = (long long)c->tmpl.bytes;
    if (rows) *rows = c->tmpl.row_bytes ? (long long)(c->tmpl.bytes / c->tmpl.row_bytes) : 0;
    if (state) *state = c->tmpl.failed ? 2 : (c->tmpl.off ? 1 : 0);
    return ICELK_OK;
}

int icelk_seg_tail_stats(icelk_t* h, long long* out)
{
    if (!h || !out) return ICELK_EARG;
    out[0] = C(h)->tails_dev;
    out[1] = C(h)->tails_host;
    return ICELK_OK;
}

int icelk_seg_flush(icelk_t* h)
{
    if (!h) return ICELK_EARG;
    Ctx* c = C(h);
    HIPCHK(c, hipSetDevice(c->device));
    return flush_deferred(c);
}

static int seg_pick(Ctx* c, bool closed, int* set)
{
    if (!c->seg_active) FAIL(c, ICELK_ESTATE, "icelk_seg_detect has not been called");
    if (closed && !c->closed_valid) FAIL(c, ICELK_ESTATE, "no closed segment");
    *set = closed ? (c->sb_cur + kSegSets - 1) % kSegSets : c->sb_cur;
    if (c->defer.pending && c->defer.set == *set) {
        int rc = flush_deferred(c);
        if (rc) return rc;
    }
    return closed ? ICELK_OK : seg_wait(c);
}

static int seg_live_core(Ctx* c, bool closed, int* out_live, int64_t* out_tracked_total)
{
    int set = 0;
    int rc = seg_pick(c, closed, &set);
    if (rc) return rc;
    launch_seg_stats(c->stream, c->sb[set].alive, c->sb[set].upper, c->d_tracked, c->h_seg);
    rc = check_launch(c, "seg_stats");
    if (rc) return rc;
    HIPCHK(c, hipStreamSynchronize(c->stream));
    const int n = (int)c->h_seg[0];
    const unsigned long long t = c->h_seg[1];
    if (out_live) *out_live = n;
    if (out_tracked_total) *out_tracked_total = (int64_t)t;
    return ICELK_OK;
}

int icelk_seg_live(icelk_t* h, int* out_live, int64_t* out_tracked_total)
{
    if (!h) return ICELK_EARG;
    Ctx* c = C(h);
    HIPCHK(c, hipSetDevice(c->device));
    return seg_live_core(c, false, out_live, out_tracked_total);
}

int icelk_seg_track(icelk_t* h, int slot_prev, int slot_next, int win_w, int win_h, int max_level, int crit_type,
                    int max_count, double epsilon, double min_eig_threshold, float fb_threshold, int* out_live)
{
    int rc = icelk_seg_track_async(h, slot_prev, slot_next, win_w, win_h, max_level, crit_type, max_count, epsilon,
                                   min_eig_threshold, fb_threshold);
    if (rc) return rc;
    return icelk_seg_live(h, out_live, nullptr);
}

static int seg_read_core(Ctx* c, bool closed, float* tracks, float* quality, int cap, int max_vertices, int* out_n,
                         int* out_vertices)
{
    int n = 0;
    int rc = seg_live_core(c, closed, &n, nullptr);
    if (rc) return rc;
    Ctx::SegBuf& S = c->sb[closed ? (c->sb_cur + kSegSets - 1) % kSegSets : c->sb_cur];
    const int nv = S.vert;
    if (out_n) *out_n = n;
    if (out_vertices) *out_vertices = nv;
    if (!tracks && !quality) return ICELK_OK;
    if (n > cap || nv > max_vertices) FAIL(c, ICELK_ECAP, "host track buffers too small");
    if (n == 0) return ICELK_OK;
    launch_seg_gather(c->stream, S.alive, S.upper, S.tracks, S.quality, nv, kMaxVert, c->d_out_tracks, c->d_out_quality);
    rc = check_launch(c, "seg_gather");
    if (rc) return rc;
    if (tracks)
        HIPCHK(c, hipMemcpy2DAsync(tracks, sizeof(float) * 2 * max_vertices, c->d_out_tracks, sizeof(float) * 2 * nv,
                                   sizeof(float) * 2 * nv, n, hipMemcpyDeviceToHost, c->stream));
    if (quality && nv > 1)
        HIPCHK(c, hipMemcpy2DAsync(quality, sizeof(float) * (max_vertices - 1), c->d_out_quality, sizeof(float) * (nv - 1),
                                   sizeof(float) * (nv - 1), n, hipMemcpyDeviceToHost, c->stream));
    HIPCHK(c, hipStreamSynchronize(c->stream));
    return ICELK_OK;
}

int icelk_seg_read(icelk_t* h, float* tracks, float* quality, int cap, int max_vertices, int* out_n, int* out_vertices)
{
    if (!h) return ICELK_EARG;
    Ctx* c = C(h);
    HIPCHK(c, hipSetDevice(c->device));
    return seg_read_core(c, false, tracks, quality, cap, max_vertices, out_n, out_vertices);
}

int icelk_seg_read_closed(icelk_t* h, float* tracks, float* quality, int cap, int max_vertices, int* out_n,
                          int* out_vertices)
{
    if (!h) return ICELK_EARG;
    Ctx* c = C(h);
    HIPCHK(c, hipSetDevice(c->device));
    return seg_read_core(c, true, tracks, quality, cap, max_vertices, out_n, out_vertices);
}

static int seg_archive_core(Ctx* c, bool closed, void* dev_tracks, void* dev_quality, void* dev_count, int cap_rows,
                            int* out_vertices)
{
    if (!dev_tracks || !dev_count) FAIL(c, ICELK_EARG, "null device buffer");
    int set = 0;
    int rc = seg_pick(c, closed, &set);
    if (rc) return rc;
    Ctx::SegBuf& S = c->sb[set];
    if (cap_rows < S.upper) FAIL(c, ICELK_ECAP, "archive rows < tracks of the segment");
    const int nv = S.vert;
    if (out_vertices) *out_vertices = nv;
    launch_seg_gather(c->stream, S.alive, S.upper, S.tracks, S.quality, nv, kMaxVert, reinterpret_cast<float*>(dev_tracks),
                      dev_quality ? reinterpret_cast<float*>(dev_quality) : c->d_out_quality, reinterpret_cast<int*>(dev_count));
    rc = check_launch(c, "seg_archive");
    if (rc) return rc;
    HIPCHK(c, hipEventRecord(S.used_own, c->stream));
    S.used = S.used_own;
    return ICELK_OK;
}

int icelk_seg_archive(icelk_t* h, void* dev_tracks, void* dev_quality, void* dev_count, int cap_rows, int* out_vertices)
{
    if (!h) return ICELK_EARG;
    Ctx* c = C(h);
    HIPCHK(c, hipSetDevice(c->device));
    return seg_archive_core(c, false, dev_tracks, dev_quality, dev_count, cap_rows, out_vertices);
}

int icelk_seg_archive_closed(icelk_t* h, void* dev_tracks, void* dev_quality, void* dev_count, int cap_rows,
                             int* out_vertices)
{
    if (!h) return ICELK_EARG;
    Ctx* c = C(h);
    HIPCHK(c, hipSetDevice(c->device));
    return seg_archive_core(c, true, dev_tracks, dev_quality, dev_count, cap_rows, out_vertices);
}

int icelk_seg_project(icelk_t* h, const icelk_camera_t* cam, const icelk_utm_filter_t* filt, int cap, int max_vectors,
                      double* x, double* y, double* u, double* v, double* speed, uint8_t* keep, int* out_n,
                      int* out_vectors)
{
    if (!h) return ICELK_EARG;
    Ctx* c = C(h);
    HIPCHK(c, hipSetDevice(c->device));
    int rc = check_projection_args(c, cam, filt);
    if (rc) return rc;
    if (!c->seg_active) FAIL(c, ICELK_ESTATE, "icelk_seg_detect has not been called");
    int n = 0;
    rc = icelk_seg_live(h, &n, nullptr);
    if (rc) return rc;
    Ctx::SegBuf& S = c->sb[c->sb_cur];
    const int nv = S.vert;
    if (out_n) *out_n = n;
    if (out_vectors) *out_vectors = nv - 1;
    if (n > cap || nv - 1 > max_vectors) FAIL(c, ICELK_ECAP, "host buffers too small");
    if (n == 0) return ICELK_OK;
    launch_seg_gather(c->stream, S.alive, S.upper, S.tracks, S.quality, nv, kMaxVert, c->d_out_tracks, c->d_out_quality);
    rc = check_launch(c, "seg_gather");
    if (rc) return rc;
    return project_core(c, c->d_out_tracks, n, nv, cam, filt, max_vectors, x, y, u, v, speed, keep);
}

}
```

### iceberg_tracking_code_amd/csrc/icelk_ctx.h

```cpp
#pragma once
#include <math.h>
#include <stdio.h>
#include <stdlib.h>
#include <string.h>

#include <algorithm>
#include <mutex>

#include "icelk_internal.h"

namespace icelk {

constexpr int kSegSets = 6;
constexpr int kLaunchEvents = 32;
constexpr int kMaxVert = 17;

struct DetectJob {
    bool active = false;
    int w = 0, h = 0;
    double quality = 0, min_distance = 0;
    size_t ncell = 0;
    const int* cand_count_ptr = nullptr;
    int prune_want = 0;
    unsigned long long seq = 0;
    bool dev_tail = false;
    int seg_set = -1;
    int max_corners = 0;
};

struct Ctx {
    int device = 0;
    int max_w = 0, max_h = 0, n_slots = 0, max_pts = 0;
    hipStream_t own_stream = nullptr, stream = nullptr;
    std::string err;
    int side_pick[4] = {-1, -1, -1, -1};
    double probe_limit = 0, probe_quickest = 0;
    int fb_dist_form = ICELK_FB_HYPOT;
    int lk_sum_mode = 0;
    int lk_wide_sums = 0;
    int corner_variant = 0;
    int lk_kernel_flags = 0;
    uint32_t* d_iters = nullptr;
    int iters_n = 0;
    unsigned long long* d_stamps = nullptr;
    size_t stamps_cap = 0;
    std::string stamps_path;
    bool prof = false;
    bool prof_tracker_only = false;
    std::vector<ProfEvt> evts, evt_pool;
    int prof_launches[K_COUNT_] = {0};
    double prof_ms[K_COUNT_] = {0};

    std::vector<Slot> slots;
    hipStream_t copy_hi[2] = {nullptr, nullptr};
    unsigned upload_seq = 0;
    hipStream_t pyr_stream = nullptr;
    uint8_t* d_bgr = nullptr;
    int bgr_pitch = 0;
    bool pyr_per_level = false;
    struct Jpeg {
        int16_t* d_coef = nullptr;
        uint8_t *d_planes = nullptr, *d_rgb = nullptr;
        size_t coef_cap = 0, planes_cap = 0, rgb_cap = 0;
        uint8_t* d_file = nullptr;
        lanes::Seg* d_seg = nullptr;
        lanes::HuffTable* d_tabs = nullptr;
        uint64_t *d_T = nullptr, *d_X = nullptr;
        uint32_t *d_cnt = nullptr, *d_P = nullptr, *d_ctl = nullptr;
        int32_t* d_dc = nullptr;
        size_t file_cap = 0, seg_cap = 0, lane_cap = 0, group_cap = 0, dc_cap = 0;
        int subseq_bits = 512, max_hops = lanes::kGroup, max_rounds = 8;
        icelk_jpeg_huff_stats_t stats{};
    } jpeg;

    float *d_p0 = nullptr, *d_p1 = nullptr, *d_p0r = nullptr, *d_err_f = nullptr, *d_err_b = nullptr, *d_dist = nullptr;
    uint8_t *d_st_f = nullptr, *d_st_b = nullptr, *d_valid = nullptr;

    hipStream_t det_stream = nullptr;
    hipEvent_t det_done = nullptr;
    hipEvent_t corners_free = nullptr;
    float* d_corners = nullptr;
    uint8_t* d_mask = nullptr;
    int mask_pitch = 0;
    bool has_mask = false;
    int mask_w = 0, mask_h = 0;
    size_t ncell_cap = 0;
    struct EigOut {
        unsigned long long* raw = nullptr;
        int* blk_count = nullptr;
        unsigned* max_key = nullptr;
        uint2* acand = nullptr;
        int* acount = nullptr;
        uint2* amaxc = nullptr;
        int* amaxn = nullptr;
        float* aemax = nullptr;
        unsigned* fmax_key = nullptr;
        unsigned* aties = nullptr;
        double quality = 0;
        int nblk = 0, region = 0;
        bool valid = false;
        int slot = -1, block_size = 0, use_mask = 0;
        unsigned long long gen = 0, mask_gen = 0;
        hipEvent_t done = nullptr;
    } eo[3];
    struct DetSet {
        DetectScratch D{};
        DetectJob job{};
        int* h_counts = nullptr;
        int counts_seq = 0;
        hipEvent_t counts_ev = nullptr;
        hipEvent_t tail_done = nullptr;
        size_t reset_ncell = 0;
        bool counters_clean = false;
        int eo_active = 0;
    } dset[2];
    int dset_last = 0;
    hipStream_t tail_stream = nullptr;
    unsigned long long job_seq = 0;
    hipStream_t eig_stream = nullptr;
    unsigned long long mask_gen = 0;
    double prep_quality = 0;

    bool host_tail = false;
    int tail_force_status = 0;
    long long tails_dev = 0, tails_host = 0;
    int last_candidates = 0, last_accepted = 0;
    double prune_factor = 8.0;

    struct SegBuf {
        float* live = nullptr;
        uint8_t* alive = nullptr;
        int* order = nullptr;
        int* order_border = nullptr;
        float* tracks = nullptr;
        float* quality = nullptr;
        hipEvent_t used = nullptr, used_own = nullptr;
        hipEvent_t ready = nullptr;
        int vert = 0, upper = 0;
        int tmpl_for = -1, tmpl_key = 0, tmpl_slot = -1;
        unsigned long long tmpl_gen = 0;
    } sb[kSegSets];
    struct {
        void* buf[2] = {nullptr, nullptr};
        size_t bytes = 0;
        size_t row_bytes = 0;
        size_t budget = (size_t)8 << 30;
        int quads = 0, levels = 0;
        bool off = false;
        bool failed = false;
        long long taken = 0, left = 0;
    } tmpl;
    int track_len_hint = 0;
    hipEvent_t launch_ev[kLaunchEvents] = {nullptr};
    int launch_seq = 0;
    int sb_cur = 0;
    bool closed_valid = false;
    struct Deferred {
        bool pending = false;
        int set = 0, slot_prev = 0, slot_next = 0;
        LKJob job{};
        LKParams P{};
    } defer;
    bool seg_ready_pending = false;
    bool use_order = true;
    int border_px = (10 + kLkTileMargin + 2) << 2;
    bool seg_active = false;
    bool seg_staged = false;
    int staged_n = 0;
    unsigned long long* d_tracked = nullptr;
    unsigned long long* h_seg = nullptr;
    float *d_out_tracks = nullptr, *d_out_quality = nullptr;

    struct Post {
        double* d_proj = nullptr;
        uint8_t* d_keep = nullptr;
        size_t proj_cap = 0;
        double *d_cube_u = nullptr, *d_cube_v = nullptr, *d_cube_count = nullptr;
        int cube_ncells = 0, cube_nt = 0;
    } post;

    struct Calib {
        double* d_shore = nullptr;
        double* d_water = nullptr;
        int M = 0, W = 0;
        double E = 0, N = 0;
    } calib;
};

extern std::string g_create_err;
extern std::mutex g_mu;

#define HIPCHK(c, expr)                                                                      \
    do {                                                                                     \
        hipError_t e_ = (expr);                                                              \
        if (e_ != hipSuccess) {                                                              \
            (c)->err = std::string(#expr) + ": " + hipGetErrorString(e_);                    \
            return ICELK_EHIP;                                                               \
        }                                                                                    \
    } while (0)

#define FAIL(c, code, msg)   \
    do {                     \
        (c)->err = (msg);    \
        return (code);       \
    } while (0)

inline Ctx* C(icelk_t* h) { return reinterpret_cast<Ctx*>(h); }

inline int check_launch(Ctx* c, const char* what)
{
    hipError_t e = hipGetLastError();
    if (e != hipSuccess) {
        c->err = std::string(what) + ": " + hipGetErrorString(e);
        return ICELK_EHIP;
    }
    return ICELK_OK;
}

struct Roctx {
    int (*push)(const char*) = nullptr;
    int (*pop)() = nullptr;
    Roctx();
};
Roctx& roctx();
struct Range {
    bool on;
    explicit Range(const char* name) : on(roctx().push != nullptr)
    {
        if (on) roctx().push(name);
    }
    ~Range()
    {
        if (on) roctx().pop();
    }
};

struct ProfScope {
    Ctx* c;
    int id;
    hipStream_t st;
    ProfEvt ev{};
    ProfScope(Ctx* c_, int id_, hipStream_t st_ = nullptr) : c(c_), id(id_), st(st_ ? st_ : c_->stream)
    {
        on = c->prof && (!c->prof_tracker_only || id == K_LK_FB || id == K_LK_FB_PAIR || id == K_LK);
        if (on) {
            if (!c->evt_pool.empty()) {
                ev = c->evt_pool.back();
                c->evt_pool.pop_back();
            } else {
                hipEventCreate(&ev.a);
                hipEventCreate(&ev.b);
            }
            ev.id = id;
            hipEventRecord(ev.a, st);
        }
    }
    ~ProfScope()
    {
        if (on) {
            hipEventRecord(ev.b, st);
            c->evts.push_back(ev);
        }
    }
    bool on = false;
};

inline int align_up(int v, int a) { return (v + a - 1) / a * a; }

template <typename T>
int dmalloc(Ctx* c, T** p, size_t count)
{
    hipError_t e = hipMalloc(reinterpret_cast<void**>(p), sizeof(T) * (count ? count : 1));
    if (e != hipSuccess) {
        c->err = std::string("hipMalloc: ") + hipGetErrorString(e);
        return ICELK_ENOMEM;
    }
    return ICELK_OK;
}

struct DevBufs {
    std::vector<void*> p;
    bool failed = false;
    ~DevBufs()
    {
        for (void* q : p)
            if (q) hipFree(q);
    }
    template <typename T>
    T* get(size_t count)
    {
        void* q = nullptr;
        if (hipMalloc(&q, sizeof(T) * (count ? count : 1)) != hipSuccess) return failed = true, nullptr;
        p.push_back(q);
        return reinterpret_cast<T*>(q);
    }
    bool ok() const { return !failed; }
};

template <typename D, typename S>
inline hipError_t copy_n(D* dst, const S* src, size_t n, hipMemcpyKind kind, hipStream_t s)
{
    static_assert(sizeof(D) == sizeof(S), "element sizes differ");
    return hipMemcpyAsync(dst, src, sizeof(D) * n, kind, s);
}
constexpr hipMemcpyKind kH2D = hipMemcpyHostToDevice, kD2H = hipMemcpyDeviceToHost;

struct EvPair {
    hipEvent_t a = nullptr, b = nullptr;
    ~EvPair()
    {
        if (a) hipEventDestroy(a);
        if (b) hipEventDestroy(b);
    }
    int create(Ctx* c)
    {
        HIPCHK(c, hipEventCreate(&a));
        HIPCHK(c, hipEventCreate(&b));
        return ICELK_OK;
    }
};

void prof_drain(Ctx* c);
hipError_t create_priority_stream(hipStream_t* s);
bool layout_ok(const Slot& s);
void layout_levels(Slot& s, int w, int h);
size_t slot_bytes(int w, int h);
int pyramid_top_level(int w, int h, int win_w, int win_h, int max_level);
int check_slot(Ctx* c, int slot, bool need_image);
int wait_event(Ctx* c, hipStream_t s, hipEvent_t e);
int wait_slot(Ctx* c, int slot);
int ensure_pyramid(Ctx* c, int slot, int top_level);
Pyramid pyramid_of(const Slot& s);
bool jpeg_info_ok(const icelk_jpeg_info_t& in);
struct JpegIndex {
    icelk_jpeg_info_t info;
    lanes::HuffTable tabs[lanes::kTables];
    lanes::Scan scan;
    std::vector<lanes::Seg> seg;
};
int jpeg_index(const uint8_t* d, size_t len, JpegIndex& X);
void jpeg_index_lanes(JpegIndex& X, uint32_t S, int max_hops);
bool jpeg_huff_config_ok(int subseq_bits, int max_hops, int max_rounds);
int jpeg_host_decode(const uint8_t* data, size_t len, int16_t* coef, uint64_t capacity);
int make_lk_params(Ctx* c, int w, int h, int win_w, int win_h, int max_level, int crit_type, int max_count,
                   double epsilon, int flags, double min_eig_thr, float fb_thr, LKParams* P);
int alloc_eig_out(Ctx* c, Ctx::EigOut& e, int cand_cap);
void free_eig_out(Ctx::EigOut& e);
int alloc_det_set(Ctx* c, Ctx::DetSet& S, int cand_cap);
void free_det_set(Ctx::DetSet& S);
void activate_eig_out(Ctx* c, Ctx::DetSet& S, int idx);
int detect_prepare(Ctx* c, int slot, int use_mask, int block_size);
int detect_begin(Ctx* c, int slot, int use_mask, int max_corners, double quality, double min_distance, int block_size,
                 bool for_segment);
int detect_finish(Ctx* c, int max_corners, int cap, int* n_out, Ctx::SegBuf* seg = nullptr, bool* seg_done = nullptr,
                  bool* dev_done = nullptr, DetectJob* finished = nullptr);
int detect_counts_arrived(Ctx* c, bool* arrived);
int flush_deferred(Ctx* c);
int flush_deferred_slot(Ctx* c, int slot);
int check_projection_args(Ctx* c, const icelk_camera_t* cam, const icelk_utm_filter_t* filt);
int project_core(Ctx* c, const float* d_tracks_in, int n, int nv, const icelk_camera_t* cam, const icelk_utm_filter_t* filt,
                 int host_pitch, double* x, double* y, double* u, double* v, double* speed, uint8_t* keep);

}
```

### iceberg_tracking_code_amd/csrc/icelk_internal.h

```cpp
#pragma once
#include <hip/hip_runtime.h>
#include <stdint.h>
#include <string>
#include <vector>

#include "../../include/icelk.h"
#include "jpeg_lanes.h"

namespace icelk {

constexpr int kMaxLevels = ICELK_MAX_LEVELS;
constexpr int kPitchAlign = 64;

struct Level {
    uint8_t* ptr;
    int w, h, pitch;
};

struct Pyramid {
    Level lv[kMaxLevels];
};

struct LKParams {
    int win_w, win_h;
    int top_level;
    int max_count;
    double eps2;
    int flags;
    float min_eig_thr;
    float fb_thr;
    int margin;
    float eps2_lo, eps2_hi;
    int dist_form;
    int sum_mode;
    unsigned sum_guard;
};

enum KernelId {
    K_GRAY = 0,
    K_PYRDOWN,
    K_LK,
    K_LK_FB,
    K_EIG,
    K_SUPPRESS,
    K_EMIT,
    K_PROJECT,
    K_SYNTH,
    K_LK_FB_PAIR,
    K_JPEG_IDCT,
    K_JPEG_OUT,
    K_JPEG_HUFF,
    K_COUNT_
};

struct Slot {
    uint8_t* base = nullptr;
    size_t bytes = 0;
    int w = 0, h = 0;
    int levels_built = 0;
    Level lv[kMaxLevels];
    hipEvent_t ready = nullptr;
    bool pending = false;
    hipEvent_t frame_ev = nullptr;
    hipEvent_t used = nullptr, used_own = nullptr, det_used = nullptr;
    hipEvent_t eig_used = nullptr;
    unsigned long long gen = 0;
};

struct ProfEvt {
    hipEvent_t a, b;
    int id;
};

struct Ctx;

void launch_bgr2gray(hipStream_t s, const uint8_t* src, int src_pitch, uint8_t* dst, int dst_pitch,
                     int w, int h, int variant);
void launch_pyrdown(hipStream_t s, const Level& src, const Level& dst);
void launch_pyramid_fused(hipStream_t s, const Level* lv, int first, int n, bool one_wave = false);
void launch_synth(hipStream_t s, const Level& dst, int64_t ux, int64_t uy, uint32_t seed, const int* affine);

struct JpegIdctArgs {
    const int16_t* coef[3];
    uint8_t* plane[3];
    int pitch[3], blocks_x[3];
    int bx0[3], by0[3], nbx[3];
    int first[4];
    uint16_t quant[3][64];
};
struct JpegOutArgs {
    const uint8_t* plane[3];
    int pitch[3];
    int W;
    int cw, ch;
    int mode;
    int left, top, ow, oh;
    uint8_t* dst;
    int dst_pitch;
    int k0, k1, k2, shift;
};
void launch_jpeg_idct(hipStream_t s, const JpegIdctArgs& A);
void launch_jpeg_gray(hipStream_t s, JpegOutArgs A, int variant);
void launch_jpeg_rgb(hipStream_t s, JpegOutArgs A);

constexpr int kJpegMaxRounds = 255;
constexpr int kJpegDcChunk = 16;
enum JpegHuffCtl {
    JH_BOUND = 0,
    JH_IRREGULAR,
    JH_IN_STEP,
    JH_SPANS,
    JH_MAX_HOPS,
    JH_TOTAL_HOPS,
    JH_ROUND0 = 8,
    JH_WORDS = JH_ROUND0 + kJpegMaxRounds + 1
};
struct JpegHuffArgs {
    lanes::Scan A;
    const uint8_t* data;
    const lanes::Seg* seg;
    const lanes::HuffTable* tabs;
    uint64_t* T;
    uint32_t* cnt;
    uint32_t* P;
    uint64_t* X;
    uint32_t* ctl;
    int16_t* coef;
    int32_t* dc;
    uint32_t ngroups;
    uint32_t ri_mcus, cps;
};
void launch_jpeg_huff_sync(hipStream_t s, const JpegHuffArgs& H, int round);
void launch_jpeg_huff_scan(hipStream_t s, const JpegHuffArgs& H);
void launch_jpeg_huff_write(hipStream_t s, const JpegHuffArgs& H);
void launch_jpeg_huff_dc(hipStream_t s, const JpegHuffArgs& H);

struct LKBuffers {
    const float* p_in;
    float* p_fwd;
    uint8_t* st_fwd;
    float* err_fwd;
    float* p_bwd;
    uint8_t* st_bwd;
    float* err_bwd;
    float* dist;
    uint8_t* valid;
    const int* n_dev;
    const int* order;
    int order_plain;
    const int* order_border;
    uint8_t* seg_alive;
    float* seg_xy;
    float* seg_tracks;
    float* seg_quality;
    int seg_vert, seg_max_vert;
    unsigned long long* seg_tracked;
    unsigned long long* stamps;
    uint32_t* iters;
    void* tmpl_out;
    const void* tmpl_in;
    int tmpl_levels;
};
int lk_template_quads(int win_w, int win_h);
bool lk_fast_eligible(const LKParams& P);
constexpr int kLkTileMargin = 1;
struct LKJob {
    Pyramid I, J;
    LKBuffers B;
    int n;
};
size_t lk_lds_bytes(const LKParams& P);
int launch_lk(hipStream_t s, const Pyramid& I, const Pyramid& J, const LKBuffers& B, int n, const LKParams& P,
              bool fb);
bool launch_lk_pair(hipStream_t s, const LKJob& a, const LKJob& b, const LKParams& P);

struct DetectScratch {
    float* eig;
    unsigned* max_key;
    unsigned long long* cand;
    int* cand_count;
    int cand_cap;
    int* cell_count;
    int* cell_start;
    int* cell_fill;
    int* chunk_tot;
    unsigned long long* cell_cand;
    uint8_t* state;
    int* undecided;
    unsigned long long* acc;
    unsigned long long* acc_sorted;
    unsigned long long* raw;
    int* acc_count;
    void* sort_tmp;
    size_t sort_tmp_bytes;
    int* blk_count;
    unsigned* key_hist;
    unsigned* prune_key;
    int src_nblk, src_region;
    uint2* acand;
    int* acount;
    uint2* amaxc;
    int* amaxn;
    float* aemax;
    unsigned* fmax_key;
    unsigned* aties;
    int* tail_ctl;
    int* tail_resp;
    int* tail_bins;
};
enum TailCtl { TC_TICKET_GATHER = 0, TC_TICKET_RANK, TC_TICKET_ORDER, TC_NOUT, TC_STATUS, TC_CAND, TC_ACC, TC_UNDECIDED, TC_PRUNED, TC_WORDS_ = 16 };
enum TailStatus { TAIL_OK = 0, TAIL_UNDECIDED = 1, TAIL_PRUNED_SHORT = 2, TAIL_OVERFLOW = 3, TAIL_SKEWED = 4 };
constexpr int kTailOrderBins = 8192;
constexpr int kTailRespBins = 4096;
struct TailOrderGeo {
    int cw_shift, ch_shift, cells_x, ncells, w, h, border_px;
};
struct TailReset {
    int* cell_count;
    int* cell_fill;
    int ncell;
    int* chunk_tot;
    int* undecided;
    int* acc_count;
    int* cand_count;
    unsigned* key_hist;
    unsigned* prune_key;
    int scan_chunk, chunk_stride, key_bins;
};
TailOrderGeo tail_order_geometry(int w, int h, int border_px);
size_t tail_resp_words();
TailReset tail_reset_of(DetectScratch& D, int ncell);
void launch_tail_gather(hipStream_t s, DetectScratch& D, int ncell, double quality, int undecided_index, int max_corners,
                        int cap, int force_status);
void launch_tail_device(hipStream_t s, DetectScratch& D, double quality, float* seg_xy, uint8_t* seg_alive, float* seg_tracks,
                        int max_vert, int* order, int* order_border, const TailOrderGeo& geo, const TailReset& rs,
                        int* host_counts, int counts_seq_word, int seq);
void launch_min_eig(hipStream_t s, const Level& img, int block_size, float* eig, const uint8_t* mask,
                    int mask_pitch, unsigned* max_key, int variant = 0);
bool fused_block_size(int bs);
void launch_detect_reset(hipStream_t s, DetectScratch& D, int ncell, int mode);
void launch_candidates(hipStream_t s, DetectScratch& D, const Level& img, int block_size, const uint8_t* mask,
                       int mask_pitch, double quality, bool use_generic, float* eig_out_or_null, int variant = 0);
bool launch_candidates_fast(hipStream_t s, DetectScratch& D, const Level& img, int block_size, const uint8_t* mask,
                            int mask_pitch, double quality);
size_t fast_tiles(int w, int h);
size_t fast_cand_entries(int w, int h);
size_t fast_max_entries(int w, int h);
size_t fast_key_capacity(int w, int h);
size_t fast_regions(int w, int h);
size_t candidate_capacity(int w, int h);
size_t candidate_blocks(int w, int h);
void launch_flatten(hipStream_t s, DetectScratch& D, double quality);
void launch_min_distance(hipStream_t s, DetectScratch& D, int w, int h, double min_distance, double quality,
                         int prune_want, bool no_gather = false);
void continue_min_distance(hipStream_t s, DetectScratch& D, int w, int h, double min_distance);
int suppress_launch_count();
size_t sort_tmp_bytes(int n);
void sort_keys_desc(hipStream_t s, DetectScratch& D, const unsigned long long* in, unsigned long long* out,
                    int n);
void launch_emit_corners(hipStream_t s, const unsigned long long* keys, int n, int w, float* xy);
void launch_tail_fused(hipStream_t s, const unsigned long long* keys, int n, float* corners, float* seg_xy,
                       uint8_t* seg_alive, float* seg_tracks, int max_vert, DetectScratch& D, int ncell, int mode);

void launch_fb_filter(hipStream_t s, const float* p0, const float* p0r, int n, float thr, int form, float* dist,
                      uint8_t* valid);
void launch_seg_init(hipStream_t s, const float* corners, int n, float* xy, uint8_t* alive, float* tracks,
                     int max_vert);
typedef icelk_camera_t UtmCamera;
typedef icelk_utm_filter_t UtmFilter;
void launch_project_tracks(hipStream_t s, const float* tracks, int n, int nv, const UtmCamera& cam, const UtmFilter& f,
                           double* x, double* y, double* u, double* v, double* speed, uint8_t* keep);
void launch_points_in_polygon(hipStream_t s, const double* poly, int n, const double* pts, int m, uint8_t* out);
void launch_grid_assign(hipStream_t s, const double* x, const double* y, int n, double left, double top, double spacing,
                        int cols, int rows, const uint8_t* cell_on, unsigned long long* keys, int* key_count, int key_cap);
void launch_grid_day_assign(hipStream_t s, const double* x, const double* y, const double* t, int n,
                            const long long* file_off, const int* file_cam, const int* win_f0, const int* win_f1,
                            int nfiles, const long long* t_lo, const long long* t_hi, int ncam, int nw, double left,
                            double top, double spacing, int cols, int rows, const uint8_t* cell_on,
                            unsigned long long* keys, int* key_count, int key_cap, int* sel_count,
                            unsigned long long* t_min, unsigned long long* t_max);
void launch_grid_reduce(hipStream_t s, const unsigned long long* keys, const int* key_count, const double* u,
                        const double* v, int ncells, int* count, double* mean_u, double* mean_v, double* speed);
void launch_cube_temporal(hipStream_t s, const double* u, const double* v, const double* cnt, int ncells,
                          const int* sel_offset, const int* sel_index, int nperiods, double* mean_u, double* mean_v,
                          double* speed, double* count_sum, int* has_data);
void launch_cube_spatial(hipStream_t s, const double* mean_u, const double* mean_v, const double* count_sum, int rows,
                         int cols, int coarseness, int nperiods, double* out_u, double* out_v, double* out_speed,
                         double* out_count);
void launch_calib_residuals(hipStream_t s, const double* cand, int P, const double* shore, int M, const double* water,
                            int W, double E, double N, double* out_dist, double* out_tx, double* out_ty);
void launch_calib_cost(hipStream_t s, const double* cand, int P, const double* shore, int M, const double* water, int W,
                       double E, double N, double* out_meansq);
int calib_cost_max_points();
size_t sort_keys_asc(hipStream_t s, void* tmp, size_t tmp_bytes, const unsigned long long* in, unsigned long long* out,
                     int n, int end_bit);
void launch_polygon_mask(hipStream_t s, const double* poly, int n, double crop_left, double crop_top, int w, int h,
                         uint8_t* mask, int pitch);
void launch_seg_order(hipStream_t s, const float* xy, int n, int w, int h, int border_px, int* order, int* border_count);
void launch_seg_stats(hipStream_t s, const uint8_t* alive, int n, const unsigned long long* tracked_shards,
                      unsigned long long* host_out);
void launch_seg_gather(hipStream_t s, const uint8_t* alive, int n, const float* tracks, const float* quality,
                       int nvert, int max_vert, float* out_tracks, float* out_quality, int* out_count = nullptr);
size_t min_eig_lds_bytes(int block_size);

}
```

### iceberg_tracking_code_amd/csrc/k_lk.hip

```cpp
#include "lk_common.h"

namespace icelk {

bool launch_lk_fast(hipStream_t s, const Pyramid& I, const Pyramid& J, const LKBuffers& B, int n, const LKParams& P,
                    bool fb);
bool launch_lk_multi(hipStream_t s, const Pyramid& I, const Pyramid& J, const LKBuffers& B, int n, const LKParams& P,
                     bool fb);

namespace {

using namespace lk;

struct LdsPlan {
    int s_pitch;
    int d_pitch;
    int j_pitch;
    int j_w, j_h;
    int deriv_off;
};

__host__ __device__ inline LdsPlan make_plan(int win_w, int win_h, int margin)
{
    LdsPlan p;
    p.s_pitch = (win_w + 3 + 3) & ~3;
    p.d_pitch = win_w + 1;
    p.j_w = win_w + 1 + 2 * margin;
    p.j_h = win_h + 1 + 2 * margin;
    p.j_pitch = (p.j_w + 3) & ~3;
    int s_bytes = p.s_pitch * (win_h + 3);
    int j_bytes = p.j_pitch * p.j_h;
    int tile = s_bytes > j_bytes ? s_bytes : j_bytes;
    p.deriv_off = (tile + 15) & ~15;
    return p;
}

__device__ __forceinline__ void stage_tile(uint8_t* lds, int pitch, int tw, int th, const Level& L, int x0, int y0,
                                           int lane)
{
    const int n = tw * th;
    const bool inside = x0 >= 0 && y0 >= 0 && x0 + tw <= L.w && y0 + th <= L.h;
    if (inside) {
        for (int i = lane; i < n; i += 64) {
            const int ty = i / tw, tx = i - ty * tw;
            lds[ty * pitch + tx] = L.ptr[(size_t)(y0 + ty) * L.pitch + (x0 + tx)];
        }
    } else {
        for (int i = lane; i < n; i += 64) {
            const int ty = i / tw, tx = i - ty * tw;
            const int sx = reflect101(x0 + tx, L.w), sy = reflect101(y0 + ty, L.h);
            lds[ty * pitch + tx] = L.ptr[(size_t)sy * L.pitch + sx];
        }
    }
}

template <int PPL>
__device__ __forceinline__ TrackResult track_point(const Pyramid& PI, const Pyramid& PJ, float p0x, float p0y,
                                                   bool have_init, float initx, float inity,
                                                   const LKParams& P, uint8_t* lds, int lane)
{
    const int win_w = P.win_w, win_h = P.win_h;
    const int npx = win_w * win_h;
    const LdsPlan plan = make_plan(win_w, win_h, P.margin);
    uint8_t* tile = lds;
    uint32_t* dtile = reinterpret_cast<uint32_t*>(lds + plan.deriv_off);
    const float half_x = (win_w - 1) * 0.5f, half_y = (win_h - 1) * 0.5f;
    const float FLT_SCALE = 1.f / (1 << 20);

    int wx[PPL], wy[PPL];
#pragma unroll
    for (int k = 0; k < PPL; k++) {
        const int idx = lane + 64 * k;
        const int yy = idx / win_w;
        wy[k] = yy;
        wx[k] = idx - yy * win_w;
    }

    TrackResult R;
    R.status = 1;
    R.err = 0.f;
    R.iters = 0;
    float sx = 0.f, sy = 0.f;
    float* fsum = reinterpret_cast<float*>(lds + plan.deriv_off + 4 * (win_w + 1) * (win_h + 1));
    auto lane_chain_sums = [&](int planes, int whole, bool pairwise, float (&out)[3]) {
        __syncthreads();
        float acc = 0.f;
        if (lane < 5 * planes) {
            const int p = lane / 5, c = lane - 5 * p;
            const float* src = fsum + p * npx;
            for (int y = 0; y < win_h; y++) {
                if (c < 4) for (int x = c; x < whole; x += 4) acc = __fadd_rn(acc, src[y * win_w + x]);
                else for (int x = whole; x < win_w; x++) acc = __fadd_rn(acc, src[y * win_w + x]);
            }
        }
#pragma unroll
        for (int p = 0; p < 3; p++) {
            if (p >= planes) break;
            const float q0 = __shfl(acc, 5 * p), q1 = __shfl(acc, 5 * p + 1), q2 = __shfl(acc, 5 * p + 2), q3 = __shfl(acc, 5 * p + 3);
            const float t = __shfl(acc, 5 * p + 4);
            out[p] = pairwise ? __fadd_rn(t, __fadd_rn(__fadd_rn(q0, q2), __fadd_rn(q1, q3)))
                              : __fadd_rn(t, __fadd_rn(__fadd_rn(__fadd_rn(q0, q1), q2), q3));
        }
        __syncthreads();
    };

    for (int level = P.top_level; level >= 0; level--) {
        const Level LI = PI.lv[level];
        const Level LJ = PJ.lv[level];
        const float scale = 1.f / (float)(1 << level);
        float px = p0x * scale, py = p0y * scale;
        if (level == P.top_level) {
            if (have_init) { sx = initx * scale; sy = inity * scale; }
            else { sx = px; sy = py; }
        } else {
            sx = sx * 2.f; sy = sy * 2.f;
        }
        px -= half_x; py -= half_y;
        const int ipx = (int)floorf(px), ipy = (int)floorf(py);
        if (ipx < -win_w || ipx >= LI.w || ipy < -win_h || ipy >= LI.h) {
            if (level == 0) { R.status = 0; R.err = 0.f; }
            continue;
        }
        const Weights wi = bilinear_weights(px - (float)ipx, py - (float)ipy);

        __syncthreads();
        stage_tile(tile, plan.s_pitch, win_w + 3, win_h + 3, LI, ipx - 1, ipy - 1, lane);
        __syncthreads();
        {
            const int dn = (win_w + 1) * (win_h + 1);
            for (int i = lane; i < dn; i += 64) {
                const int ty = i / (win_w + 1), tx = i - ty * (win_w + 1);
                const int gx = ipx + tx, gy = ipy + ty;
                uint32_t packed = 0;
                if (gx >= 0 && gx < LI.w && gy >= 0 && gy < LI.h) {
                    const uint8_t* r0 = tile + ty * plan.s_pitch + tx;
                    const uint8_t* r1 = r0 + plan.s_pitch;
                    const uint8_t* r2 = r1 + plan.s_pitch;
                    const int t0l = (r0[0] + r2[0]) * 3 + r1[0] * 10;
                    const int t0r = (r0[2] + r2[2]) * 3 + r1[2] * 10;
                    const int t1l = r2[0] - r0[0], t1c = r2[1] - r0[1], t1r = r2[2] - r0[2];
                    const int ix = t0r - t0l;
                    const int iy = (t1r + t1l) * 3 + t1c * 10;
                    packed = ((uint32_t)ix & 0xffffu) | ((uint32_t)iy << 16);
                }
                dtile[ty * plan.d_pitch + tx] = packed;
            }
        }
        __syncthreads();

        int Ival[PPL];
        uint32_t dIval[PPL];
        int a11 = 0, a12 = 0, a22 = 0;
#pragma unroll
        for (int k = 0; k < PPL; k++) {
            Ival[k] = 0;
            dIval[k] = 0;
            if (lane + 64 * k < npx) {
                const uint8_t* s0 = tile + (wy[k] + 1) * plan.s_pitch + (wx[k] + 1);
                const uint8_t* s1 = s0 + plan.s_pitch;
// ... 32 lines not shown
        const float minEig = __fdiv_rn(__fsub_rn(__fadd_rn(A22, A11), sqrtf(rad)), (float)(2 * win_w * win_h));
        if (P.flags & ICELK_FLAG_MIN_EIGENVALS) R.err = minEig;
        if (minEig < P.min_eig_thr || D < 1.1920928955078125e-07f) {
            if (level == 0) R.status = 0;
            continue;
        }
        D = __fdiv_rn(1.f, D);

        float nx = sx - half_x, ny = sy - half_y;
        float pdx = 0.f, pdy = 0.f;
        int jx0 = 0, jy0 = 0;
        bool staged = false;
        for (int j = 0; j < P.max_count; j++) {
            const int inx = (int)floorf(nx), iny = (int)floorf(ny);
            if (inx < -win_w || inx >= LJ.w || iny < -win_h || iny >= LJ.h) {
                if (level == 0) R.status = 0;
                break;
            }
            R.iters++;
            if (!staged || inx < jx0 || inx > jx0 + 2 * P.margin || iny < jy0 || iny > jy0 + 2 * P.margin) {
                jx0 = inx - P.margin; jy0 = iny - P.margin;
                __syncthreads();
                stage_tile(tile, plan.j_pitch, plan.j_w, plan.j_h, LJ, jx0, jy0, lane);
                __syncthreads();
                staged = true;
            }
            const Weights wj = bilinear_weights(nx - (float)inx, ny - (float)iny);
            const uint8_t* jbase = tile + (iny - jy0) * plan.j_pitch + (inx - jx0);
            int b1 = 0, b2 = 0;
#pragma unroll
            for (int k = 0; k < PPL; k++) {
                if (lane + 64 * k < npx) {
                    const uint8_t* j0 = jbase + wy[k] * plan.j_pitch + wx[k];
                    const uint8_t* j1 = j0 + plan.j_pitch;
                    const int diff = descale(j0[0] * wj.w00 + j0[1] * wj.w01 + j1[0] * wj.w10 + j1[1] * wj.w11,
                                             W_BITS - 5) - Ival[k];
                    b1 += diff * (int)(short)(dIval[k] & 0xffff);
                    b2 += diff * ((int)dIval[k] >> 16);
                    if (P.sum_mode) {
                        const int idx = lane + 64 * k;
                        fsum[idx] = (float)(diff * (int)(short)(dIval[k] & 0xffff));
                        fsum[npx + idx] = (float)(diff * ((int)dIval[k] >> 16));
                    }
                }
            }
            float fb1 = (float)wave_sum_exact(b1) * FLT_SCALE;
            float fb2 = (float)wave_sum_exact(b2) * FLT_SCALE;
            if (P.sum_mode) {
                float o[3];
                lane_chain_sums(2, win_w & ~7, true, o);
                fb1 = __fmul_rn(o[0], FLT_SCALE); fb2 = __fmul_rn(o[1], FLT_SCALE);
            }
            const float dx = __fmul_rn(__fsub_rn(__fmul_rn(A12, fb2), __fmul_rn(A22, fb1)), D);
            const float dy = __fmul_rn(__fsub_rn(__fmul_rn(A12, fb1), __fmul_rn(A11, fb2)), D);
            nx = __fadd_rn(nx, dx); ny = __fadd_rn(ny, dy);
            sx = __fadd_rn(nx, half_x); sy = __fadd_rn(ny, half_y);
            if (__dadd_rn(__dmul_rn((double)dx, (double)dx), __dmul_rn((double)dy, (double)dy)) <= P.eps2) break;
            if (j > 0 && fabs((double)__fadd_rn(dx, pdx)) < 0.01 && fabs((double)__fadd_rn(dy, pdy)) < 0.01) {
                sx = __fsub_rn(sx, __fmul_rn(dx, 0.5f));
                sy = __fsub_rn(sy, __fmul_rn(dy, 0.5f));
                break;
            }
            pdx = dx; pdy = dy;
        }

        if (R.status && level == 0 && !(P.flags & ICELK_FLAG_MIN_EIGENVALS)) {
            const float qx = sx - half_x, qy = sy - half_y;
            const int iqx = (int)floorf(qx), iqy = (int)floorf(qy);
            if (iqx < -win_w || iqx >= LJ.w || iqy < -win_h || iqy >= LJ.h) {
                R.status = 0;
                continue;
            }
            if (!staged || iqx < jx0 || iqx > jx0 + 2 * P.margin || iqy < jy0 || iqy > jy0 + 2 * P.margin) {
                jx0 = iqx - P.margin; jy0 = iqy - P.margin;
                __syncthreads();
                stage_tile(tile, plan.j_pitch, plan.j_w, plan.j_h, LJ, jx0, jy0, lane);
                __syncthreads();
                staged = true;
            }
            const Weights we = bilinear_weights(qx - (float)iqx, qy - (float)iqy);
            const uint8_t* jbase = tile + (iqy - jy0) * plan.j_pitch + (iqx - jx0);
            int es = 0;
#pragma unroll
            for (int k = 0; k < PPL; k++) {
                if (lane + 64 * k < npx) {
                    const uint8_t* j0 = jbase + wy[k] * plan.j_pitch + wx[k];
                    const uint8_t* j1 = j0 + plan.j_pitch;
                    const int diff = descale(j0[0] * we.w00 + j0[1] * we.w01 + j1[0] * we.w10 + j1[1] * we.w11,
                                             W_BITS - 5) - Ival[k];
                    es += diff < 0 ? -diff : diff;
                }
            }
            const float errval = (float)wave_sum_exact(es);
            R.err = __fdiv_rn(__fmul_rn(errval, 1.f), (float)(32 * win_w * win_h));
        }
    }
    R.x = sx;
    R.y = sy;
    return R;
}

template <int PPL, bool FB>
__global__ __launch_bounds__(64) void k_lk(Pyramid PI, Pyramid PJ, LKBuffers B, int n, LKParams P)
{
    extern __shared__ __attribute__((aligned(16))) uint8_t lds[];
    const int f = launch_slot(B, blockIdx.x, B.n_dev ? *B.n_dev : n);
    if (f < 0) return;
    if (B.seg_alive && !B.seg_alive[f]) return;
    const int lane = threadIdx.x;
    const float p0x = B.p_in[2 * f], p0y = B.p_in[2 * f + 1];
    const bool init = (P.flags & ICELK_FLAG_INITIAL_FLOW) != 0;
    float ix = 0.f, iy = 0.f;
    if (init) { ix = B.p_fwd[2 * f]; iy = B.p_fwd[2 * f + 1]; }
    const TrackResult r1 = track_point<PPL>(PI, PJ, p0x, p0y, init, ix, iy, P, lds, lane);
    if (lane == 0) {
        if (B.p_fwd) { B.p_fwd[2 * f] = r1.x; B.p_fwd[2 * f + 1] = r1.y; }
        if (B.st_fwd) B.st_fwd[f] = (uint8_t)r1.status;
        if (B.err_fwd) B.err_fwd[f] = r1.err;
        if (B.iters && !FB) B.iters[f] = (uint32_t)r1.iters;
    }
    if (FB) {
        const TrackResult r2 = track_point<PPL>(PJ, PI, r1.x, r1.y, false, 0.f, 0.f, P, lds, lane);
        if (lane == 0) {
            if (B.p_bwd) { B.p_bwd[2 * f] = r2.x; B.p_bwd[2 * f + 1] = r2.y; }
            if (B.st_bwd) B.st_bwd[f] = (uint8_t)r2.status;
            if (B.err_bwd) B.err_bwd[f] = r2.err;
            if (B.iters) B.iters[f] = (uint32_t)r1.iters | ((uint32_t)r2.iters << 16);
            const float d = fb_distance(p0x, p0y, r2.x, r2.y, P.dist_form);
            if (B.dist) B.dist[f] = d;
            if (B.valid) B.valid[f] = d < P.fb_thr ? 1 : 0;
            if (B.seg_alive) seg_append(B, f, r1.x, r1.y, d, d < P.fb_thr);
        }
    }
}

template <int PPL>
void launch_ppl(hipStream_t s, const Pyramid& I, const Pyramid& J, const LKBuffers& B, int n, const LKParams& P,
                bool fb, size_t lds)
{
    if (fb) hipLaunchKernelGGL((k_lk<PPL, true>), dim3(B.order ? (n + 15) & ~7 : n), dim3(64), lds, s, I, J, B, n, P);
    else hipLaunchKernelGGL((k_lk<PPL, false>), dim3(B.order ? (n + 15) & ~7 : n), dim3(64), lds, s, I, J, B, n, P);
}

}

size_t lk_lds_bytes(const LKParams& P)
{
    const LdsPlan p = make_plan(P.win_w, P.win_h, P.margin);
    const size_t lane_sums = P.sum_mode ? 12u * (size_t)P.win_w * P.win_h : 0u;
    return (size_t)p.deriv_off + 4u * (size_t)(P.win_w + 1) * (P.win_h + 1) + lane_sums;
}

int launch_lk(hipStream_t s, const Pyramid& I, const Pyramid& J, const LKBuffers& B, int n, const LKParams& P,
              bool fb)
{
    if (n <= 0) return ICELK_OK;
    const bool generic = (P.flags & ICELK_FLAG_GENERIC_KERNEL) != 0;
    if ((P.flags & ICELK_FLAG_MULTI_PER_WAVE) && !generic && !P.sum_mode && launch_lk_multi(s, I, J, B, n, P, fb))
        return ICELK_OK;
    if (!generic && launch_lk_fast(s, I, J, B, n, P, fb)) return ICELK_OK;
    const int npx = P.win_w * P.win_h;
    const int ppl = (npx + 63) / 64;
    const size_t lds = lk_lds_bytes(P);
    if (lds > 64 * 1024) return ICELK_EARG;
    if (ppl <= 2) launch_ppl<2>(s, I, J, B, n, P, fb, lds);
    else if (ppl <= 4) launch_ppl<4>(s, I, J, B, n, P, fb, lds);
    else if (ppl <= 7) launch_ppl<7>(s, I, J, B, n, P, fb, lds);
    else if (ppl <= 10) launch_ppl<10>(s, I, J, B, n, P, fb, lds);
    else if (ppl <= 16) launch_ppl<16>(s, I, J, B, n, P, fb, lds);
    else if (ppl <= 20) launch_ppl<20>(s, I, J, B, n, P, fb, lds);
    else if (ppl <= 28) launch_ppl<28>(s, I, J, B, n, P, fb, lds);
    else if (ppl <= 40) launch_ppl<40>(s, I, J, B, n, P, fb, lds);
    else if (ppl <= 64) launch_ppl<64>(s, I, J, B, n, P, fb, lds);
    else return ICELK_EARG;
    return ICELK_OK;
}

}
```

### iceberg_tracking_code_amd/csrc/k_lk_fast.hip

```cpp
#include "lk_fast_tiles.h"

namespace icelk {

namespace {

using namespace lk;
using namespace lkf;

__device__ __forceinline__ float sum_to_float(long long t)
{
    const int hi = (int)(t >> 16), lo = (int)(t & 0xffff);
    return __fadd_rn(__fmul_rn((float)hi, 65536.f), (float)lo);
}

__device__ __forceinline__ int floor_uni(float x)
{
    int i = (int)floorf(x);
    asm volatile("" : "+v"(i));
    return uni(i);
}
__device__ __forceinline__ int floor_uni(float x, float& fx)
{
    fx = floorf(x);
    int i = (int)fx;
    asm volatile("" : "+v"(i));
    return uni(i);
}

template <int WW, int WH>
struct TmplIO {
    using C = Cfg<WW, WH>;
    static constexpr int HP = (C::S + 1) / 2;
    static constexpr int NI = C::TPL * C::S;
    static constexpr bool PACKED = ((NI + 1) / 2 + C::TPL * 2 * HP + 1 + 3) / 4 < (NI + C::TPL * 2 * HP + 1 + 3) / 4;
    static constexpr int NIP = PACKED ? (NI + 1) / 2 : NI;
    static constexpr int NDW = NIP + C::TPL * 2 * HP;
    static constexpr int NQ = (NDW + 1 + 3) / 4;
    static constexpr int LEVEL = NQ * 64;
    static constexpr int WAVES = C::TPL == 1 ? 5 : 3;
    static constexpr bool FITS = (C::LDS_DW * 4 + NQ * 1024) * 4 * WAVES <= 160 * 1024;
    static constexpr int LDS_Q = FITS ? NQ * 64 : 1;
};

template <int WW, int WH>
__device__ __forceinline__ void tmpl_store(const Template<WW, WH, 1>& T, float A11, float A12, float A22,
                                           uint4* __restrict__ dst, int lane)
{
    using IO = TmplIO<WW, WH>;
    using C = Cfg<WW, WH>;
    uint32_t d[IO::NQ * 4];
#pragma unroll
    for (int i = 0; i < IO::NQ * 4; i++) d[i] = 0u;
    d[IO::NDW] = __float_as_uint(lane == 0 ? A11 : (lane == 1 ? A12 : A22));
    constexpr int kSeed = 1 << (W_BITS - 6), kShift = W_BITS - 5;
    if constexpr (IO::PACKED) {
#pragma unroll
        for (int p = 0; p < IO::NIP; p++) {
            const uint32_t lo = (uint32_t)(kSeed - T.Ineg[0][(2 * p) / C::S][(2 * p) % C::S]) >> kShift;
            uint32_t hi = 0u;
            if (2 * p + 1 < IO::NI) hi = (uint32_t)(kSeed - T.Ineg[0][(2 * p + 1) / C::S][(2 * p + 1) % C::S]) << (16 - kShift);
            d[p] = lo | hi;
        }
    } else {
#pragma unroll
        for (int n = 0; n < IO::NI; n++) d[n] = (uint32_t)T.Ineg[0][n / C::S][n % C::S];
    }
#pragma unroll
    for (int k = 0; k < C::TPL; k++) {
#pragma unroll
        for (int q = 0; q < IO::HP; q++) {
            d[IO::NIP + k * 2 * IO::HP + q] = T.Ixp[0][k][q];
            d[IO::NIP + k * 2 * IO::HP + IO::HP + q] = T.Iyp[0][k][q];
        }
    }
    typedef uint32_t u4v __attribute__((ext_vector_type(4)));
#pragma unroll
    for (int q = 0; q < IO::NQ; q++) {
        const u4v v = {d[4 * q], d[4 * q + 1], d[4 * q + 2], d[4 * q + 3]};
        __builtin_nontemporal_store(v, reinterpret_cast<u4v*>(dst + q * 64 + lane));
    }
}

template <int WW, int WH>
__device__ __forceinline__ void tmpl_unpack(Template<WW, WH, 1>& T, float& A11, float& A12, float& A22,
                                            const uint4 (&v)[TmplIO<WW, WH>::NQ])
{
    using IO = TmplIO<WW, WH>;
    using C = Cfg<WW, WH>;
    uint32_t d[IO::NQ * 4];
#pragma unroll
    for (int q = 0; q < IO::NQ; q++) { d[4 * q] = v[q].x; d[4 * q + 1] = v[q].y; d[4 * q + 2] = v[q].z; d[4 * q + 3] = v[q].w; }
    A11 = __uint_as_float((uint32_t)__builtin_amdgcn_readlane((int)d[IO::NDW], 0));
    A12 = __uint_as_float((uint32_t)__builtin_amdgcn_readlane((int)d[IO::NDW], 1));
    A22 = __uint_as_float((uint32_t)__builtin_amdgcn_readlane((int)d[IO::NDW], 2));
    constexpr int kSeed = 1 << (W_BITS - 6), kShift = W_BITS - 5;
#pragma unroll
    for (int n = 0; n < IO::NI; n++) {
        if constexpr (IO::PACKED) {
            const uint32_t w = d[n / 2];
            const uint32_t sh = (n & 1) ? ((w >> (16 - kShift)) & ~((1u << kShift) - 1u)) : ((w & 0xffffu) << kShift);
            T.Ineg[0][n / C::S][n % C::S] = kSeed - (int)sh;
        } else {
            T.Ineg[0][n / C::S][n % C::S] = (int)d[n];
        }
    }
#pragma unroll
    for (int k = 0; k < C::TPL; k++) {
#pragma unroll
        for (int q = 0; q < IO::HP; q++) {
            T.Ixp[0][k][q] = d[IO::NIP + k * 2 * IO::HP + q];
            T.Iyp[0][k][q] = d[IO::NIP + k * 2 * IO::HP + IO::HP + q];
        }
    }
}

template <int WW, int WH, int WHOLE>
__device__ __forceinline__ void chain_sums_t(const float* fsum, int planes, bool pairwise, float (&out)[3], int lane)
{
    constexpr int NPX = WW * WH;
    constexpr int NI = WHOLE / 4, NT = WW - WHOLE, MAXN = NI > NT ? NI : NT, INFL = Cfg<WW, WH>::TPL > 1 ? 16 : 32,
                  RB = INFL / MAXN > 0 ? INFL / MAXN : 1;
    __syncthreads();
    float acc = 0.f;
    const int p = lane / 5, c = lane - 5 * p;
    const bool busy = lane < 5 * planes;
    const int x0 = c < 4 ? c : WHOLE, stride = c < 4 ? 4 : 1, count = busy ? (c < 4 ? NI : NT) : 0;
    const float* src = fsum + (busy ? p : 0) * NPX + x0;
#pragma unroll 1
    for (int y0 = 0; y0 < WH; y0 += RB) {
        float v[RB][MAXN];
#pragma unroll
        for (int r = 0; r < RB; r++)
#pragma unroll
            for (int i = 0; i < MAXN; i++) {
                const bool ok = i < count && y0 + r < WH;
                v[r][i] = ok ? src[(y0 + r) * WW + i * stride] : 0.f;
            }
#pragma unroll
        for (int r = 0; r < RB; r++)
#pragma unroll
            for (int i = 0; i < MAXN; i++) acc = __fadd_rn(acc, v[r][i]);
    }
#pragma unroll
    for (int q = 0; q < 3; q++) {
        if (q >= planes) break;
        const float q0 = __shfl(acc, 5 * q), q1 = __shfl(acc, 5 * q + 1), q2 = __shfl(acc, 5 * q + 2), q3 = __shfl(acc, 5 * q + 3);
        const float t = __shfl(acc, 5 * q + 4);
        out[q] = pairwise ? __fadd_rn(t, __fadd_rn(__fadd_rn(q0, q2), __fadd_rn(q1, q3)))
                          : __fadd_rn(t, __fadd_rn(__fadd_rn(__fadd_rn(q0, q1), q2), q3));
    }
    __syncthreads();
}

// ... 145 lines not shown
                A11 = lane63_float_u32(n11) * FLT_SCALE;
                A12 = lane63_float_i32(n12) * FLT_SCALE;
                A22 = lane63_float_u32(n22) * FLT_SCALE;
            } else {
                long long s11, s12, s22;
                if constexpr (kSmall) wave_sum_mat_i64(a11, a12, a22, s11, s12, s22);
                else wave_sum3_i64<1>(a11, a12, a22, s11, s12, s22);
                A11 = sum_to_float(s11) * FLT_SCALE;
                A12 = sum_to_float(s12) * FLT_SCALE;
                A22 = sum_to_float(s22) * FLT_SCALE;
            }
            if (fsum) {
                float o[3];
                chain_sums<WW, WH>(fsum, 3, P.sum_mode == 1 ? (WW & ~3) : (WW & ~7), P.sum_mode == 2, o, lane);
                A11 = __fmul_rn(o[0], FLT_SCALE); A12 = __fmul_rn(o[1], FLT_SCALE); A22 = __fmul_rn(o[2], FLT_SCALE);
            }
        }
        if (IO::FITS && tmode == 2) tmpl_store<WW, WH>(T, A11, A12, A22, tio + level * IO::LEVEL, lane);
        float D = __fsub_rn(__fmul_rn(A11, A22), __fmul_rn(A12, A12));
        const float dif = __fsub_rn(A11, A22);
        const float rad = __fadd_rn(__fmul_rn(dif, dif), __fmul_rn(__fmul_rn(4.f, A12), A12));
        const float tr = __fadd_rn(A22, A11);
        const float approx = (tr - __builtin_amdgcn_sqrtf(rad)) * (1.f / (float)(2 * WW * WH));
        const bool clear_pass = __builtin_amdgcn_ballot_w64(approx > P.min_eig_thr + tr * 2e-6f) != 0 &&
                                !(P.flags & ICELK_FLAG_MIN_EIGENVALS);
        if (!clear_pass) {
            const float minEig = __fdiv_rn(__fsub_rn(tr, sqrtf(rad)), (float)(2 * WW * WH));
            if (P.flags & ICELK_FLAG_MIN_EIGENVALS) Rz.err = minEig;
            if (minEig < P.min_eig_thr) {
                if (level == 0) Rz.status = 0;
                continue;
            }
        }
        if (D < 1.1920928955078125e-07f) {
            if (level == 0) Rz.status = 0;
            continue;
        }
        D = __fdiv_rn(1.f, D);

        float pdx = __builtin_nanf(""), pdy = __builtin_nanf("");
        for (int j = 0; j < P.max_count; j++) {
            float fnx, fny;
            const int inx = floor_uni(nx, fnx), iny = floor_uni(ny, fny);
            if (!origin_ok<WW, WH>(LJ, inx, iny)) {
                if (level == 0) Rz.status = 0;
                break;
            }
            if (!tile_covers(jx0, jy0, inx, iny)) {
                jx0 = inx - R; jy0 = iny - R;
                __syncthreads();
                TileRegs<C::JPD, C::JTH> tj;
                Level LR = LJ;
                asm volatile("" : "+s"(LR.pitch));
                if (tile_inside(LR, jx0, jy0, C::JTW, C::JTH)) tile_issue(tj, LR, jx0, jy0, lane);
                else tile_issue_reflect(tj, LR, jx0, jy0, lane);
                tile_commit(tj, ldsJ, lane);
                __syncthreads();
            }
            Rz.iters++;
            uint32_t wj0, wj1;
            packed_weights<true>(nx - fnx, ny - fny, wj0, wj1);
            const int jb = uni((iny - jy0) * (C::JPD * 4) + (jx0 & 3) + (inx - jx0));
            int b1, b2;
            if constexpr (kPackSeg) {
                int row_l[C::TPL], col_l[C::TPL], len_l[C::TPL], joff_l[C::TPL];
                seg_rows_cols(row_l, col_l, len_l);
#pragma unroll
                for (int k = 0; k < C::TPL; k++) joff_l[k] = row_l[k] * (C::JPD * 4) + col_l[k];
                residual_pixels<WW, WH, 1, 0, false>(T, ldsJ, jb, (uint32_t)uni((int)wj0),
                                                     (uint32_t)uni((int)wj1), joff_l, len_l, b1, b2, fsum, row_l, col_l);
            } else
            residual_pixels<WW, WH, 1, 0, false>(T, ldsJ, jb, (uint32_t)uni((int)wj0),
                                                 (uint32_t)uni((int)wj1), joff, tlen, b1, b2, fsum, trow, tcol);
            float fb1, fb2;
            const bool wide2 = fsum != nullptr ||
                __builtin_amdgcn_ballot_w64((((unsigned)b1 + kSumGuardBias) | ((unsigned)b2 + kSumGuardBias)) >= P.sum_guard) != 0;
            if (__builtin_expect_with_probability(!wide2, 1, 0.7)) {
                const int n1 = dpp_all_steps(b1), n2 = dpp_all_steps(b2);
                fb1 = lane63_float_i32(n1) * FLT_SCALE;
                fb2 = lane63_float_i32(n2) * FLT_SCALE;
            } else {
                long long t1, t2;
                wave_sum2_i64<kSmall ? 8 : 1>(b1, b2, t1, t2);
                fb1 = sum_to_float(t1) * FLT_SCALE;
                fb2 = sum_to_float(t2) * FLT_SCALE;
            }
            if (fsum) {
                float o[3];
                chain_sums<WW, WH>(fsum, 2, WW & ~7, true, o, lane);
                fb1 = __fmul_rn(o[0], FLT_SCALE); fb2 = __fmul_rn(o[1], FLT_SCALE);
            }
            const float dx = __fmul_rn(__fsub_rn(__fmul_rn(A12, fb2), __fmul_rn(A22, fb1)), D);
            const float dy = __fmul_rn(__fsub_rn(__fmul_rn(A12, fb1), __fmul_rn(A11, fb2)), D);
            nx = __fadd_rn(nx, dx); ny = __fadd_rn(ny, dy);
            sx = __fadd_rn(nx, half_x); sy = __fadd_rn(ny, half_y);
            const float q = __fadd_rn(__fmul_rn(dx, dx), __fmul_rn(dy, dy));
            bool conv = q < P.eps2_lo;
            if (__builtin_amdgcn_ballot_w64(!conv && !(q > P.eps2_hi)) != 0) {
                asm volatile("" ::: "memory");
                conv = __dadd_rn(__dmul_rn((double)dx, (double)dx), __dmul_rn((double)dy, (double)dy)) <= P.eps2;
            }
            if (conv) break;
            if (fabsf(__fadd_rn(dx, pdx)) <= 0.01f && fabsf(__fadd_rn(dy, pdy)) <= 0.01f) {
                sx = __fsub_rn(sx, __fmul_rn(dx, 0.5f));
                sy = __fsub_rn(sy, __fmul_rn(dy, 0.5f));
                break;
            }
            pdx = dx; pdy = dy;
        }

        if (Rz.status && level == 0 && !(P.flags & ICELK_FLAG_MIN_EIGENVALS)) {
            const float qx = sx - half_x, qy = sy - half_y;
            const int iqx = floor_uni(qx), iqy = floor_uni(qy);
            if (!origin_ok<WW, WH>(LJ, iqx, iqy)) {
                Rz.status = 0;
                continue;
            }
            if (!want_err) continue;
            if (!tile_covers(jx0, jy0, iqx, iqy)) {
                jx0 = iqx - R; jy0 = iqy - R;
                __syncthreads();
                TileRegs<C::JPD, C::JTH> tj;
                if (tile_inside(LJ, jx0, jy0, C::JTW, C::JTH)) tile_issue(tj, LJ, jx0, jy0, lane);
                else tile_issue_reflect(tj, LJ, jx0, jy0, lane);
                tile_commit(tj, ldsJ, lane);
                __syncthreads();
            }
            uint32_t we0, we1;
            packed_weights<true>(qx - (float)iqx, qy - (float)iqy, we0, we1);
            const int jb = uni((iqy - jy0) * (C::JPD * 4) + (jx0 & 3) + (iqx - jx0));
            int es, unused;
            if constexpr (kPackSeg) {
                int row_l[C::TPL], col_l[C::TPL], len_l[C::TPL], joff_l[C::TPL];
                seg_rows_cols(row_l, col_l, len_l);
#pragma unroll
                for (int k = 0; k < C::TPL; k++) joff_l[k] = row_l[k] * (C::JPD * 4) + col_l[k];
                residual_pixels<WW, WH, 1, 0, true>(T, ldsJ, jb, (uint32_t)uni((int)we0),
                                                    (uint32_t)uni((int)we1), joff_l, len_l, es, unused);
            } else
            residual_pixels<WW, WH, 1, 0, true>(T, ldsJ, jb, (uint32_t)uni((int)we0),
                                                (uint32_t)uni((int)we1), joff, tlen, es, unused);
            const float errval = sum_to_float(sum_pick<kSmall, 8>(es));
            Rz.err = __fdiv_rn(__fmul_rn(errval, 1.f), (float)(32 * WW * WH));
        }
    }
    Rz.x = sx;
    Rz.y = sy;
    return Rz;
}

struct LKJobs {
    LKJob job[2];
    int g0, g1;
};

template <int WW, int WH, bool FB, bool SM = false>
__device__ __forceinline__ void lk_fast_body(const LKJobs& JJ, const LKParams& P)
{
    using C = Cfg<WW, WH>;
    constexpr int kTileQ = (C::LDS_DW + 3) / 4;
    __shared__ uint4 lds_q[kTileQ + (SM ? 1 : TmplIO<WW, WH>::LDS_Q)];
    uint4* const tlds = lds_q + kTileQ;
    __shared__ float fs_[SM ? 3 * WW * WH : 1];
    float* const fsum = SM ? fs_ : nullptr;
    int which = 0, b = blockIdx.x;
    if (JJ.g1 > 0) {
        const int G = b >> 3, m = (JJ.g0 < JJ.g1 ? JJ.g0 : JJ.g1) >> 3;
        const int mb = m & ~31;
        int Gj;
        if (G < 2 * mb) {
            which = (G >> 5) & 1;
            Gj = ((G >> 6) << 5) | (G & 31);
        } else if (G < 2 * m) {
            const int r = G - 2 * mb;
            which = r & 1;
            Gj = mb + (r >> 1);
        } else {
            which = JJ.g0 < JJ.g1 ? 1 : 0;
            Gj = G - m;
        }
        b = (Gj << 3) | (b & 7);
    }
    const LKJob& J = JJ.job[which];
    const LKBuffers& B = J.B;
    const int f = __builtin_amdgcn_readfirstlane(launch_slot(B, b, B.n_dev ? *B.n_dev : J.n));
    if (f < 0) return;
    if (B.seg_alive && !B.seg_alive[f]) return;
    const int lane = threadIdx.x;
    uint32_t* ldsJ = reinterpret_cast<uint32_t*>(lds_q);
    uint32_t* ldsI = ldsJ + C::J_DW;
    const float p0x = B.p_in[2 * f], p0y = B.p_in[2 * f + 1];
    if (lane == 0) stamp(B, 0);
    using IO = TmplIO<WW, WH>;
    const size_t t_off = (size_t)f * ((size_t)B.tmpl_levels * IO::LEVEL);
    const TrackResult r1 = track_point_fast<WW, WH>(J.I, J.J, p0x, p0y, P, ldsI, ldsJ, lane, B.err_fwd != nullptr,
                                                    const_cast<uint4*>(static_cast<const uint4*>(B.tmpl_in)) + t_off,
                                                    !SM && B.tmpl_in ? 1 : 0, tlds, fsum);
    if (lane == 0) {
        if (B.p_fwd) { B.p_fwd[2 * f] = r1.x; B.p_fwd[2 * f + 1] = r1.y; }
        if (B.st_fwd) B.st_fwd[f] = (uint8_t)r1.status;
        if (B.err_fwd) B.err_fwd[f] = r1.err;
        if (B.iters && !FB) B.iters[f] = (uint32_t)r1.iters;
    }
    if (FB) {
        const TrackResult r2 = track_point_fast<WW, WH>(J.J, J.I, r1.x, r1.y, P, ldsI, ldsJ, lane, B.err_bwd != nullptr,
                                                        static_cast<uint4*>(B.tmpl_out) + t_off, !SM && B.tmpl_out ? 2 : 0, tlds,
                                                        fsum);
        if (lane == 0) {
            if (B.p_bwd) { B.p_bwd[2 * f] = r2.x; B.p_bwd[2 * f + 1] = r2.y; }
            if (B.st_bwd) B.st_bwd[f] = (uint8_t)r2.status;
            if (B.err_bwd) B.err_bwd[f] = r2.err;
            if (B.iters) B.iters[f] = (uint32_t)r1.iters | ((uint32_t)r2.iters << 16);
            const float d = fb_distance(p0x, p0y, r2.x, r2.y, P.dist_form);
            if (B.dist) B.dist[f] = d;
            if (B.valid) B.valid[f] = d < P.fb_thr ? 1 : 0;
            if (B.seg_alive) seg_append(B, f, r1.x, r1.y, d, d < P.fb_thr);
        }
    }
    if (lane == 0) stamp(B, 1);
}

template <int WW, int WH, bool FB>
__global__ __launch_bounds__(64, 3) void k_lk_fast(LKJobs JJ, LKParams P)
{
    lk_fast_body<WW, WH, FB>(JJ, P);
}

template <int WW, int WH, bool FB>
__global__ __launch_bounds__(64, 4) __attribute__((amdgpu_num_vgpr(44))) void k_lk_fast88(LKJobs JJ, LKParams P)
{
    lk_fast_body<WW, WH, FB>(JJ, P);
}

template <int WW, int WH, bool FB>
__global__ __launch_bounds__(64, 2) void k_lk_fast_sums(LKJobs JJ, LKParams P)
{
    lk_fast_body<WW, WH, FB, true>(JJ, P);
}

int grid_of(const LKBuffers& B, int n) { return B.order ? (n + 15) & ~7 : (n + 7) & ~7; }

template <int WW, int WH>
void launch_fast(hipStream_t s, const LKJob& a, const LKJob* b, const LKParams& P, bool fb)
{
    LKJobs JJ;
    JJ.job[0] = a;
    JJ.job[1] = b ? *b : a;
    JJ.g0 = grid_of(a.B, a.n);
    JJ.g1 = b ? grid_of(b->B, b->n) : 0;
    const int grid = JJ.g0 + JJ.g1;
    if (P.sum_mode) {
        if (fb) hipLaunchKernelGGL((k_lk_fast_sums<WW, WH, true>), dim3(grid), dim3(64), 0, s, JJ, P);
        else hipLaunchKernelGGL((k_lk_fast_sums<WW, WH, false>), dim3(grid), dim3(64), 0, s, JJ, P);
        return;
    }
    if constexpr (Cfg<WW, WH>::TPL == 1) {
        if (fb) hipLaunchKernelGGL((k_lk_fast88<WW, WH, true>), dim3(grid), dim3(64), 0, s, JJ, P);
        else hipLaunchKernelGGL((k_lk_fast88<WW, WH, false>), dim3(grid), dim3(64), 0, s, JJ, P);
    } else {
        if (fb) hipLaunchKernelGGL((k_lk_fast<WW, WH, true>), dim3(grid), dim3(64), 0, s, JJ, P);
        else hipLaunchKernelGGL((k_lk_fast<WW, WH, false>), dim3(grid), dim3(64), 0, s, JJ, P);
    }
}

bool dispatch_fast(hipStream_t s, const LKJob& a, const LKJob* b, const LKParams& P, bool fb)
{
    if (P.flags & ICELK_FLAG_INITIAL_FLOW) return false;
    if (P.win_w == 21 && P.win_h == 21) launch_fast<21, 21>(s, a, b, P, fb);
    else if (P.win_w == 31 && P.win_h == 31) launch_fast<31, 31>(s, a, b, P, fb);
    else if (P.win_w == 35 && P.win_h == 35) launch_fast<35, 35>(s, a, b, P, fb);
    else if (P.win_w == 15 && P.win_h == 15) launch_fast<15, 15>(s, a, b, P, fb);
    else return false;
    return true;
}

}

int lk_template_quads(int win_w, int win_h)
{
    if (win_w == 21 && win_h == 21) return TmplIO<21, 21>::FITS ? TmplIO<21, 21>::NQ : 0;
    if (win_w == 31 && win_h == 31) return TmplIO<31, 31>::FITS ? TmplIO<31, 31>::NQ : 0;
    if (win_w == 35 && win_h == 35) return TmplIO<35, 35>::FITS ? TmplIO<35, 35>::NQ : 0;
    if (win_w == 15 && win_h == 15) return TmplIO<15, 15>::FITS ? TmplIO<15, 15>::NQ : 0;
    return 0;
}

bool lk_fast_eligible(const LKParams& P)
{
    if (P.flags & (ICELK_FLAG_INITIAL_FLOW | ICELK_FLAG_GENERIC_KERNEL | ICELK_FLAG_MULTI_PER_WAVE)) return false;
    return P.sum_mode == 0 && lk_template_quads(P.win_w, P.win_h) > 0;
}

bool launch_lk_fast(hipStream_t s, const Pyramid& I, const Pyramid& J, const LKBuffers& B, int n, const LKParams& P,
                    bool fb)
{
    LKJob a;
    a.I = I;
    a.J = J;
    a.B = B;
    a.n = n;
    return dispatch_fast(s, a, nullptr, P, fb);
}

bool launch_lk_pair(hipStream_t s, const LKJob& a, const LKJob& b, const LKParams& P)
{
    if (P.flags & (ICELK_FLAG_GENERIC_KERNEL | ICELK_FLAG_MULTI_PER_WAVE)) return false;
    if (a.n <= 0 || b.n <= 0) return false;
    return dispatch_fast(s, a, &b, P, true);
}

}
```

### iceberg_tracking_code_amd/csrc/k_tracks.hip

```cpp
#include "lk_common.h"

namespace icelk {

namespace {

__global__ void k_seg_init(const float* __restrict__ corners, int n, float* __restrict__ xy,
                           uint8_t* __restrict__ alive, float* __restrict__ tracks, int max_vert)
{
    const int i = blockIdx.x * blockDim.x + threadIdx.x;
    if (i >= n) return;
    const float x = corners[2 * i], y = corners[2 * i + 1];
    xy[2 * i] = x; xy[2 * i + 1] = y;
    alive[i] = 1;
    tracks[((size_t)i * max_vert) * 2] = x;
    tracks[((size_t)i * max_vert) * 2 + 1] = y;
}

constexpr int kOrderBins = 8192;
__global__ __launch_bounds__(1024) void k_seg_order(const float* __restrict__ xy, int n, int cw_shift, int ch_shift,
                                                    int cells_x, int ncells, int w, int h, int border_px,
                                                    int* __restrict__ order, int* __restrict__ border_count)
{
    __shared__ int bins[kOrderBins + 1];
    __shared__ int wave_tot[16];
    const int tid = threadIdx.x, lane = tid & 63, wave = tid >> 6;
    const int nb = ncells + 1;
    for (int i = tid; i < nb; i += 1024) bins[i] = 0;
    __syncthreads();
    auto cell_of = [&](int i) {
        const int x = (int)xy[2 * i], y = (int)xy[2 * i + 1];
        if (x < border_px || y < border_px || x >= w - border_px || y >= h - border_px) return 0;
        int c = (y >> ch_shift) * cells_x + (x >> cw_shift);
        return 1 + (c < 0 ? 0 : (c >= ncells ? ncells - 1 : c));
    };
    for (int i = tid; i < n; i += 1024) atomicAdd(&bins[cell_of(i)], 1);
    __syncthreads();
    if (tid == 0) *border_count = bins[0];
    int v[9], tsum = 0;
#pragma unroll
    for (int k = 0; k < 9; k++) {
        const int b = tid * 9 + k;
        v[k] = b < nb ? bins[b] : 0;
        tsum += v[k];
    }
    int incl = tsum;
#pragma unroll
    for (int o = 1; o < 64; o <<= 1) {
        const int t = __shfl_up(incl, o);
        if (lane >= o) incl += t;
    }
    if (lane == 63) wave_tot[wave] = incl;
    __syncthreads();
    int base = incl - tsum;
    for (int k = 0; k < wave; k++) base += wave_tot[k];
#pragma unroll
    for (int k = 0; k < 9; k++) {
        const int b = tid * 9 + k;
        if (b < nb) bins[b] = base;
        base += v[k];
    }
    __syncthreads();
    for (int i = tid; i < n; i += 1024) order[atomicAdd(&bins[cell_of(i)], 1)] = i;
}

__global__ __launch_bounds__(1024) void k_seg_stats(const uint8_t* __restrict__ alive, int n,
                                                    const unsigned long long* __restrict__ shards,
                                                    unsigned long long* __restrict__ host_out)
{
    __shared__ int wave_tot[16];
    int cnt = 0;
    for (int i = threadIdx.x; i < n; i += 1024) cnt += alive[i] ? 1 : 0;
#pragma unroll
    for (int o = 32; o >= 1; o >>= 1) cnt += __shfl_xor(cnt, o);
    if ((threadIdx.x & 63) == 0) wave_tot[threadIdx.x >> 6] = cnt;
    __syncthreads();
    if (threadIdx.x == 0) {
        int t = 0;
        for (int k = 0; k < 16; k++) t += wave_tot[k];
        unsigned long long tr = 0;
        for (int k = 0; k < 64; k++) tr += shards[k];
        host_out[0] = (unsigned long long)t;
        host_out[1] = tr;
        __threadfence_system();
    }
}

constexpr int kGatherTile = 256;
__global__ __launch_bounds__(kGatherTile) void k_seg_gather(const uint8_t* __restrict__ alive, int n,
                                                            const float* __restrict__ tracks,
                                                            const float* __restrict__ quality, int nvert, int max_vert,
                                                            float* __restrict__ out_tracks, float* __restrict__ out_quality,
                                                            int* __restrict__ out_count)
{
    constexpr int NW = kGatherTile / 64;
    __shared__ int wave_tot[NW];
    __shared__ int wave_before[NW];
    const int tid = threadIdx.x, lane = tid & 63, wave = tid >> 6;
    const int base = blockIdx.x * kGatherTile;
    int mine = 0;
    const uint32_t* a32 = reinterpret_cast<const uint32_t*>(alive);
    for (int i = tid; i < (base >> 2); i += kGatherTile) mine += __builtin_popcount(a32[i] & 0x01010101u);
#pragma unroll
    for (int d = 32; d > 0; d >>= 1) mine += __shfl_xor(mine, d, 64);
    const int i = base + tid;
    const bool keep = i < n && alive[i];
    const unsigned long long m = __ballot(keep);
    if (lane == 0) {
        wave_tot[wave] = __popcll(m);
        wave_before[wave] = mine;
    }
    __syncthreads();
    int before = 0, wbase = 0, tile_total = 0;
#pragma unroll
    for (int k = 0; k < NW; k++) {
        const int t = wave_tot[k];
        before += wave_before[k];
        wbase += k < wave ? t : 0;
        tile_total += t;
    }
    if (keep) {
        const int j = before + wbase + __popcll(m & ((1ull << lane) - 1ull));
        const float2* src = reinterpret_cast<const float2*>(tracks) + (size_t)i * max_vert;
        if ((reinterpret_cast<uintptr_t>(out_tracks) & 7u) == 0) {
            float2* dst = reinterpret_cast<float2*>(out_tracks) + (size_t)j * nvert;
            for (int v = 0; v < nvert; v++) dst[v] = src[v];
        } else {
            float* dst = out_tracks + (size_t)j * nvert * 2;
            for (int v = 0; v < nvert; v++) { const float2 p = src[v]; dst[2 * v] = p.x; dst[2 * v + 1] = p.y; }
        }
        for (int v = 0; v + 1 < nvert; v++)
            out_quality[(size_t)j * (nvert - 1) + v] = quality[(size_t)i * (max_vert - 1) + v];
    }
    if (out_count && tid == 0 && base + kGatherTile >= n) *out_count = before + tile_total;
}

__global__ void k_fb_filter(const float* __restrict__ p0, const float* __restrict__ p0r, int n, float thr, int form,
                            float* __restrict__ dist, uint8_t* __restrict__ valid)
{
    const int i = blockIdx.x * blockDim.x + threadIdx.x;
    if (i >= n) return;
    const float d = lk::fb_distance(p0[2 * i], p0[2 * i + 1], p0r[2 * i], p0r[2 * i + 1], form);
    dist[i] = d;
    valid[i] = d < thr ? 1 : 0;
}

}

void launch_fb_filter(hipStream_t s, const float* p0, const float* p0r, int n, float thr, int form, float* dist,
                      uint8_t* valid)
{
    if (n <= 0) return;
    hipLaunchKernelGGL(k_fb_filter, dim3((n + 255) / 256), dim3(256), 0, s, p0, p0r, n, thr, form, dist, valid);
}

void launch_seg_init(hipStream_t s, const float* corners, int n, float* xy, uint8_t* alive, float* tracks,
                     int max_vert)
{
    if (n <= 0) return;
    hipLaunchKernelGGL(k_seg_init, dim3((n + 255) / 256), dim3(256), 0, s, corners, n, xy, alive, tracks, max_vert);
}

void launch_seg_order(hipStream_t s, const float* xy, int n, int w, int h, int border_px, int* order, int* border_count)
{
    if (n <= 0) return;
    int cw = 5, ch = 6;
    auto cells = [&](int& cx) {
        cx = ((w - 1) >> cw) + 1;
        return cx * (((h - 1) >> ch) + 1);
    };
    int cx = 0;
    while (cells(cx) > kOrderBins) {
        if (cw <= ch) cw++;
        else ch++;
    }
    const int nc = cells(cx);
    hipLaunchKernelGGL(k_seg_order, dim3(1), dim3(1024), 0, s, xy, n, cw, ch, cx, nc, w, h, border_px, order, border_count);
}

void launch_seg_stats(hipStream_t s, const uint8_t* alive, int n, const unsigned long long* tracked_shards,
                      unsigned long long* host_out)
{
    hipLaunchKernelGGL(k_seg_stats, dim3(1), dim3(1024), 0, s, alive, n, tracked_shards, host_out);
}

void launch_seg_gather(hipStream_t s, const uint8_t* alive, int n, const float* tracks, const float* quality,
                       int nvert, int max_vert, float* out_tracks, float* out_quality, int* out_count)
{
    if (n <= 0) {
        if (out_count) hipMemsetAsync(out_count, 0, sizeof(int), s);
        return;
    }
    hipLaunchKernelGGL(k_seg_gather, dim3((n + kGatherTile - 1) / kGatherTile), dim3(kGatherTile), 0, s, alive, n, tracks, quality, nvert, max_vert, out_tracks,
                       out_quality, out_count);
}

}
```

### include/icelk.h

```cpp
#ifndef ICELK_H
#define ICELK_H

#include <stdint.h>

#ifdef __cplusplus
extern "C" {
#endif

typedef struct icelk_ctx icelk_t;

#define ICELK_OK 0
#define ICELK_EARG (-1)
#define ICELK_ENOMEM (-2)
#define ICELK_EHIP (-3)
#define ICELK_ECAP (-4)
#define ICELK_ESTATE (-5)
#define ICELK_EUNSUP (-6)

#define ICELK_CRIT_COUNT 1
#define ICELK_CRIT_EPS 2
#define ICELK_FLAG_INITIAL_FLOW 4
#define ICELK_FLAG_MIN_EIGENVALS 8
#define ICELK_FLAG_GENERIC_KERNEL 0x100
#define ICELK_FLAG_MULTI_PER_WAVE 0x200
#define ICELK_GRAY_CV3 3
#define ICELK_GRAY_CV4 4
#define ICELK_FB_HYPOT 0
#define ICELK_FB_SQRT 1

#define ICELK_MAX_LEVELS 12

int icelk_version(void);
const char* icelk_last_error(icelk_t* h);
int icelk_create(int device, int max_w, int max_h, int n_slots, int max_pts, icelk_t** out);
int icelk_destroy(icelk_t* h);
int icelk_set_stream(icelk_t* h, void* hip_stream);
int icelk_sync(icelk_t* h);
int icelk_set_lk_kernel(icelk_t* h, int which);
int icelk_set_fb_distance(icelk_t* h, int form);
int icelk_set_variant(icelk_t* h, const char* name, int value);

int icelk_upload_gray(icelk_t* h, int slot, const uint8_t* host, int w, int h_, int stride);
int icelk_upload_bgr(icelk_t* h, int slot, const uint8_t* host, int w, int h_, int stride, int gray_variant);
int icelk_set_gray_device(icelk_t* h, int slot, const void* dev, int w, int h_, int stride);
int icelk_cvt_bgr_device(icelk_t* h, int slot, const void* dev_bgr, int w, int h_, int stride, int gray_variant);
int icelk_upload_gray_async(icelk_t* h, int slot, const uint8_t* pinned_host, int w, int h_, int stride);
int icelk_host_alloc(void** out, uint64_t bytes);
int icelk_host_free(void* p);
int icelk_synth_frame(icelk_t* h, int slot, int w, int h_, int64_t ux, int64_t uy, uint32_t seed);
int icelk_synth_frame_affine(icelk_t* h, int slot, int w, int h_, int64_t ux, int64_t uy, uint32_t seed,
                             const int32_t* affine);
int icelk_drop_pyramid(icelk_t* h, int slot);
int icelk_download_level(icelk_t* h, int slot, int level, uint8_t* host, int stride, int* w, int* h_);

int icelk_build_pyramid(icelk_t* h, int slot, int win_w, int win_h, int max_level, int* out_levels);
int icelk_build_pyramid_ahead(icelk_t* h, int slot, int win_w, int win_h, int max_level);

int icelk_pyrlk(icelk_t* h, int prev_slot, int next_slot, const float* prev_xy, float* next_xy,
                uint8_t* status, float* err, int n, int win_w, int win_h, int max_level,
                int crit_type, int max_count, double epsilon, int flags, double min_eig_threshold);
int icelk_track_fb(icelk_t* h, int slot0, int slot1, const float* p0, int n, int win_w, int win_h,
                   int max_level, int crit_type, int max_count, double epsilon, double min_eig_threshold,
                   float fb_threshold, float* p1, float* p0r, uint8_t* st_fwd, uint8_t* st_bwd,
                   float* err_fwd, float* err_bwd, float* dist, uint8_t* valid);

int icelk_fb_filter(icelk_t* h, const float* p0, const float* p0r, int n, float fb_threshold, float* dist,
                    uint8_t* valid);

int icelk_set_mask(icelk_t* h, const uint8_t* host_mask, int w, int h_, int stride);
int icelk_set_mask_polygon(icelk_t* h, const double* poly_xy, int n, double crop_left, double crop_top, int w, int h_);
int icelk_download_mask(icelk_t* h, uint8_t* host_mask, int stride, int* w, int* h_);
int icelk_min_eig_map(icelk_t* h, int slot, int block_size, float* host_out, int stride_elems);
int icelk_good_features(icelk_t* h, int slot, int use_mask, int max_corners, double quality_level,
                        double min_distance, int block_size, float* out_xy, int cap, int* out_n);

int icelk_detect_stats(icelk_t* h, int* n_candidates, int* n_accepted);
int icelk_detect_fast_stats(icelk_t* h, int frame_w, int frame_h, long long* out);

int icelk_seg_detect(icelk_t* h, int slot, int use_mask, int max_corners, double quality_level,
                     double min_distance, int block_size, int* out_n);
int icelk_seg_detect_begin(icelk_t* h, int slot, int use_mask, int max_corners, double quality_level,
                           double min_distance, int block_size);
int icelk_seg_detect_finish(icelk_t* h, int max_corners, int* out_n);
int icelk_seg_detect_cancel(icelk_t* h);
int icelk_seg_detect_stage(icelk_t* h, int max_corners, int* out_n);
int icelk_seg_detect_stage_try(icelk_t* h, int max_corners, int* out_n, int* out_done);
int icelk_seg_switch(icelk_t* h);
int icelk_seg_detect_prepare(icelk_t* h, int slot, int use_mask, int block_size);
int icelk_seg_track(icelk_t* h, int slot_prev, int slot_next, int win_w, int win_h, int max_level,
                    int crit_type, int max_count, double epsilon, double min_eig_threshold,
                    float fb_threshold, int* out_live);
int icelk_seg_read(icelk_t* h, float* tracks, float* quality, int cap, int max_vertices, int* out_n,
                   int* out_vertices);
int icelk_seg_archive(icelk_t* h, void* dev_tracks, void* dev_quality, void* dev_count, int cap_rows, int* out_vertices);
int icelk_seg_track_defer(icelk_t* h, int slot_prev, int slot_next, int win_w, int win_h, int max_level,
                          int crit_type, int max_count, double epsilon, double min_eig_threshold,
                          float fb_threshold);
int icelk_seg_flush(icelk_t* h);
int icelk_seg_track_len_hint(icelk_t* h, int track_len);
int icelk_seg_template_stats(icelk_t* h, long long* out);
int icelk_seg_template_info(icelk_t* h, long long* bytes_per_table, long long* rows, int* state);
int icelk_seg_tail_stats(icelk_t* h, long long* out);
int icelk_seg_read_closed(icelk_t* h, float* tracks, float* quality, int cap, int max_vertices, int* out_n,
                          int* out_vertices);
int icelk_seg_archive_closed(icelk_t* h, void* dev_tracks, void* dev_quality, void* dev_count, int cap_rows,
                             int* out_vertices);
int icelk_seg_track_async(icelk_t* h, int slot_prev, int slot_next, int win_w, int win_h, int max_level,
                          int crit_type, int max_count, double epsilon, double min_eig_threshold,
                          float fb_threshold);
int icelk_seg_live(icelk_t* h, int* out_live, int64_t* out_tracked_total);

typedef struct icelk_camera {
    double X[3], U[3], V[3];
    double sigma;
    double H, E, N;
    double half_w, half_h;
    double crop_left, crop_top;
} icelk_camera_t;
typedef struct icelk_utm_filter {
    double interval_s;
    double max_speed, min_speed, max_speedfactor, max_angle, speed_threshold;
} icelk_utm_filter_t;
int icelk_project_tracks(icelk_t* h, const float* tracks, int n, int n_vertices, const icelk_camera_t* cam,
                         const icelk_utm_filter_t* filt, double* x, double* y, double* u, double* v, double* speed,
                         uint8_t* keep);
int icelk_seg_project(icelk_t* h, const icelk_camera_t* cam, const icelk_utm_filter_t* filt, int cap, int max_vectors,
                      double* x, double* y, double* u, double* v, double* speed, uint8_t* keep, int* out_n,
                      int* out_vectors);

int icelk_points_in_polygon(icelk_t* h, const double* poly_xy, int n_poly, const double* pts_xy, int n_pts,
                            uint8_t* inside);
int icelk_grid_bin(icelk_t* h, const double* x, const double* y, const double* u, const double* v, int n, double left,
                   double top, double spacing, int cols, int rows, const uint8_t* cell_on, int* count, double* mean_u,
                   double* mean_v, double* speed);
int icelk_grid_bin_windows(icelk_t* h, const double* x, const double* y, const double* u, const double* v,
                           const double* t, int n, const int64_t* file_offset, const int* file_cam, const int* win_f0,
                           const int* win_f1, int nfiles, const int64_t* t_lo, const int64_t* t_hi, int ncam, int nw,
                           double left, double top, double spacing, int cols, int rows, const uint8_t* cell_on,
                           int* count, double* mean_u, double* mean_v, double* speed, int* sel_count, double* t_min,
                           double* t_max, double* device_ms);

int icelk_cube_set(icelk_t* h, const double* u, const double* v, const double* count, int ncells, int nt);
int icelk_cube_release(icelk_t* h);
int icelk_cube_average(icelk_t* h, const int* sel_offset, const int* sel_index, int nperiods, int rows, int cols,
                       int coarseness, double* out_u, double* out_v, double* out_speed, double* out_count,
                       int* out_has_data, double* device_ms);

int icelk_calib_set(icelk_t* h, const double* shore_xy, int M, const double* water_xy, int W, double E, double N);
int icelk_calib_release(icelk_t* h);
int icelk_calib_residuals(icelk_t* h, const double* cand, int P, double* out_dist, double* out_tx, double* out_ty,
                          double* device_ms);
int icelk_calib_cost(icelk_t* h, const double* cand, int P, double* out_meansq, double* device_ms);

typedef struct icelk_jpeg_info {
    int32_t width, height, ncomp;
    int32_t hmax, vmax;
    int32_t mcus_x, mcus_y;
    int32_t restart_interval;
    int32_t comp_w[3], comp_h[3];
    int32_t blocks_x[3], blocks_y[3];
    uint64_t coef_offset[3];
    uint64_t coef_count;
    uint16_t quant[3][64];
} icelk_jpeg_info_t;
int icelk_jpeg_describe(const uint8_t* data, uint64_t len, icelk_jpeg_info_t* info);
int icelk_jpeg_read_coefficients(const uint8_t* data, uint64_t len, int16_t* coef, uint64_t capacity);
int icelk_upload_jpeg(icelk_t* h, int slot, const icelk_jpeg_info_t* info, const int16_t* coef, int gray_variant,
                      int crop_left, int crop_top, int crop_right, int crop_bottom);
int icelk_jpeg_decode_rgb(icelk_t* h, const icelk_jpeg_info_t* info, const int16_t* coef, uint8_t* out, int stride);

#define ICELK_JPEG_TABLE_BYTES 11328
#define ICELK_JPEG_FALLBACK_NONE 0
#define ICELK_JPEG_FALLBACK_BOUND 1
#define ICELK_JPEG_FALLBACK_STREAM 2
#define ICELK_JPEG_FALLBACK_SIZE 3
typedef struct icelk_jpeg_scan {
    uint32_t segments;
    uint32_t blocks_per_mcu, blocks_per_segment , total_blocks;
    uint8_t component[8], dc_table[8], ac_table[8];
} icelk_jpeg_scan_t;
typedef struct icelk_jpeg_huff_stats {
    uint32_t segments, subsequences;
    uint32_t rounds;
    uint32_t max_hops;
    uint32_t lanes_in_step;
    uint32_t spanning_blocks;
    uint32_t fallback;
    uint32_t reserved;
    uint64_t total_hops;
} icelk_jpeg_huff_stats_t;
int icelk_jpeg_index(const uint8_t* data, uint64_t len, icelk_jpeg_info_t* info, icelk_jpeg_scan_t* scan, uint32_t* seg_begin,
                     uint32_t* seg_end, uint64_t seg_capacity, void* tables);
int icelk_jpeg_read_coefficients_lanes(const uint8_t* data, uint64_t len, int16_t* coef, uint64_t capacity, int subseq_bits,
                                       int max_hops, int max_rounds, icelk_jpeg_huff_stats_t* stats);
int icelk_jpeg_huff_config(icelk_t* h, int subseq_bits, int max_hops, int max_rounds);
int icelk_jpeg_huff_stats(icelk_t* h, icelk_jpeg_huff_stats_t* stats);
int icelk_upload_jpeg_file(icelk_t* h, int slot, const uint8_t* data, uint64_t len, int gray_variant, int crop_left, int crop_top,
                           int crop_right, int crop_bottom);
int icelk_jpeg_decode_rgb_file(icelk_t* h, const uint8_t* data, uint64_t len, uint8_t* out, int stride);
int icelk_jpeg_device_coefficients(icelk_t* h, const uint8_t* data, uint64_t len, int16_t* coef, uint64_t capacity);

int icelk_prof_enable(icelk_t* h, int on);
int icelk_prof_reset(icelk_t* h);
int icelk_prof_iterations(icelk_t* h, uint32_t* host_out, int cap, int* out_n);
int icelk_stream_probe_info(icelk_t* h, int* picks, double* quickest, double* limit);
int icelk_prof_count(void);
const char* icelk_prof_name(int kernel_id);
int icelk_prof_get(icelk_t* h, int kernel_id, int* launches, double* total_ms);

#ifdef __cplusplus
}
#endif
#endif
```

Measured before the change: 7598.

## Defer closed-segment archive gather and fold it into the next LK launch

Archiving a closed segment no longer launches its own gather kernel. The request is recorded as pending and carried into the next fast LK kernel launch as extra leading wave-sized blocks that do the compaction copy. If no eligible launch is available, or at sync, flush and buffer-reuse points, the gather is issued as a standalone kernel as before. This removes a separate kernel launch per segment, at the cost of more state tracking and slightly heavier LK grids.

```diff
diff --git a/iceberg_tracking_code_amd/_lib.py b/iceberg_tracking_code_amd/_lib.py
--- a/iceberg_tracking_code_amd/_lib.py
+++ b/iceberg_tracking_code_amd/_lib.py
@@ -107,6 +107,7 @@
     "icelk_seg_track_len_hint": (C.c_int, [handle_p, C.c_int]),
     "icelk_seg_template_stats": (C.c_int, [handle_p, C.POINTER(C.c_longlong)]),
     "icelk_seg_tail_stats": (C.c_int, [handle_p, C.POINTER(C.c_longlong)]),
+    "icelk_seg_archive_stats": (C.c_int, [handle_p, C.POINTER(C.c_longlong)]),
     "icelk_seg_template_info": (C.c_int, [handle_p, C.POINTER(C.c_longlong), C.POINTER(C.c_longlong), i32p]),
     "icelk_seg_read_closed": (C.c_int, [handle_p, f32p, f32p, C.c_int, C.c_int, i32p, i32p]),
     "icelk_seg_archive_closed": (C.c_int, [handle_p, vp, vp, vp, C.c_int, i32p]),
@@ -154,7 +155,11 @@
                 "(needs hipcc); this package has no CPU fallback." % LIB_PATH)
         lib = C.CDLL(LIB_PATH)
         for name, (res, args) in SIGNATURES.items():
-            fn = getattr(lib, name)
+            fn = getattr(lib, name, None)
+            if fn is None:
+                if os.environ.get("ICELK_LIBRARY"):
+                    continue
+                raise IcelkError("%s lacks %s: rebuild it (`python -m iceberg_tracking_code_amd.build`)" % (LIB_PATH, name))
             fn.restype = res
             fn.argtypes = args
         _lib = lib
diff --git a/iceberg_tracking_code_amd/context.py b/iceberg_tracking_code_amd/context.py
--- a/iceberg_tracking_code_amd/context.py
+++ b/iceberg_tracking_code_amd/context.py
@@ -351,6 +351,11 @@
         self._ck(self._lib.icelk_seg_tail_stats(self._h, out))
         return int(out[0]), int(out[1])
 
+    def seg_archive_stats(self):
+        out = (C.c_longlong * 2)()
+        self._ck(self._lib.icelk_seg_archive_stats(self._h, out))
+        return int(out[0]), int(out[1])
+
     def seg_track_len_hint(self, track_len):
         self._ck(self._lib.icelk_seg_track_len_hint(self._h, int(track_len)))
 
diff --git a/iceberg_tracking_code_amd/csrc/abi_detect.hip b/iceberg_tracking_code_amd/csrc/abi_detect.hip
--- a/iceberg_tracking_code_amd/csrc/abi_detect.hip
+++ b/iceberg_tracking_code_amd/csrc/abi_detect.hip
@@ -311,6 +311,7 @@
         const int ahead = (c->seg_staged ? 1 : 0) + (other.job.active ? 1 : 0);
         const int target = (c->sb_cur + 1 + ahead) % kSegSets;
         Ctx::SegBuf& nb = c->sb[target];
+        if (int rca = archive_flush_set(c, target)) return rca;
         if (int rcw = wait_event(c, ds, nb.used)) return rcw;
         S.counts_seq = (S.counts_seq + 1) & 0x3fffffff;
         {
diff --git a/iceberg_tracking_code_amd/csrc/abi_handle.hip b/iceberg_tracking_code_amd/csrc/abi_handle.hip
--- a/iceberg_tracking_code_amd/csrc/abi_handle.hip
+++ b/iceberg_tracking_code_amd/csrc/abi_handle.hip
@@ -143,7 +143,10 @@
 {
     if (!c) return;
     hipSetDevice(c->device);
-    if (c->stream) hipStreamSynchronize(c->stream);
+    if (c->stream) {
+        (void)archive_flush(c);
+        hipStreamSynchronize(c->stream);
+    }
     prof_drain(c);
     for (auto& e : c->evt_pool) {
         hipEventDestroy(e.a);
@@ -378,6 +381,7 @@
     if (!h) return ICELK_EARG;
     Ctx* c = C(h);
     HIPCHK(c, hipSetDevice(c->device));
+    if (int rca = archive_flush(c)) return rca;
     HIPCHK(c, hipStreamSynchronize(c->stream));
     c->stream = hip_stream ? reinterpret_cast<hipStream_t>(hip_stream) : c->own_stream;
     return ICELK_OK;
@@ -389,6 +393,7 @@
     Ctx* c = C(h);
     HIPCHK(c, hipSetDevice(c->device));
     int rcf = flush_deferred(c);
+    if (!rcf) rcf = archive_flush(c);
     if (rcf) return rcf;
     for (auto q : c->copy_hi)
         if (q) HIPCHK(c, hipStreamSynchronize(q));
diff --git a/iceberg_tracking_code_amd/csrc/abi_lk.hip b/iceberg_tracking_code_amd/csrc/abi_lk.hip
--- a/iceberg_tracking_code_amd/csrc/abi_lk.hip
+++ b/iceberg_tracking_code_amd/csrc/abi_lk.hip
@@ -86,12 +86,17 @@
     B.st_fwd = c->d_st_f;
     B.err_fwd = err ? c->d_err_f : nullptr;
     if (c->prof) { B.iters = c->d_iters; c->iters_n = n; }
+    LKArchive arch;
+    const LKArchive* carry = nullptr;
+    rc = archive_for_launch(c, P, n, B.iters != nullptr, &arch, &carry);
+    if (rc) return rc;
     {
         ProfScope p(c, K_LK);
-        rc = launch_lk(c->stream, pyramid_of(s0), pyramid_of(s1), B, n, P, false);
+        rc = launch_lk(c->stream, pyramid_of(s0), pyramid_of(s1), B, n, P, false, carry);
     }
     if (rc) FAIL(c, rc, "unsupported window size");
     rc = check_launch(c, "lk");
+    if (!rc) rc = archive_launched(c, carry, nullptr);
     if (rc) return rc;
     HIPCHK(c, hipMemcpyAsync(next_xy, c->d_p1, sizeof(float) * 2 * n, hipMemcpyDeviceToHost, c->stream));
     if (status) HIPCHK(c, hipMemcpyAsync(status, c->d_st_f, n, hipMemcpyDeviceToHost, c->stream));
@@ -125,12 +130,17 @@
     B.dist = c->d_dist;
     B.valid = c->d_valid;
     if (c->prof) { B.iters = c->d_iters; c->iters_n = n; }
+    LKArchive arch;
+    const LKArchive* carry = nullptr;
+    rc = archive_for_launch(c, P, n, B.iters != nullptr, &arch, &carry);
+    if (rc) return rc;
     {
         ProfScope p(c, K_LK_FB);
-        rc = launch_lk(c->stream, pyramid_of(s0), pyramid_of(s1), B, n, P, true);
+        rc = launch_lk(c->stream, pyramid_of(s0), pyramid_of(s1), B, n, P, true, carry);
     }
     if (rc) FAIL(c, rc, "unsupported window size");
     rc = check_launch(c, "lk_fb");
+    if (!rc) rc = archive_launched(c, carry, nullptr);
     if (rc) return rc;
     const size_t fb = sizeof(float) * n;
     if (p1) HIPCHK(c, hipMemcpyAsync(p1, c->d_p1, 2 * fb, hipMemcpyDeviceToHost, c->stream));
diff --git a/iceberg_tracking_code_amd/csrc/abi_segments.hip b/iceberg_tracking_code_amd/csrc/abi_segments.hip
--- a/iceberg_tracking_code_amd/csrc/abi_segments.hip
+++ b/iceberg_tracking_code_amd/csrc/abi_segments.hip
@@ -106,15 +106,72 @@
     c->sb[set].used = ev;
 }
 
+int archive_flush(Ctx* c)
+{
+    if (!c->arch.pending) return ICELK_OK;
+    Ctx::ArchivePending& a = c->arch;
+    a.pending = false;
+    Ctx::SegBuf& S = c->sb[a.set];
+    launch_seg_gather(c->stream, S.alive, S.upper, S.tracks, S.quality, a.nvert, kMaxVert, a.tracks, a.quality, a.count);
+    int rc = check_launch(c, "seg_archive");
+    if (rc) return rc;
+    HIPCHK(c, hipEventRecord(S.used_own, c->stream));
+    S.used = S.used_own;
+    c->archives_standalone++;
+    return ICELK_OK;
+}
+
+int archive_flush_set(Ctx* c, int set)
+{
+    return c->arch.pending && c->arch.set == set ? archive_flush(c) : ICELK_OK;
+}
+
+int archive_for_launch(Ctx* c, const LKParams& P, int n, bool diag, LKArchive* store, const LKArchive** out)
+{
+    *out = nullptr;
+    if (!c->arch.pending) return ICELK_OK;
+    if (diag || n <= 0 || !lk_fast_eligible(P)) return archive_flush(c);
+    const Ctx::ArchivePending& a = c->arch;
+    const Ctx::SegBuf& S = c->sb[a.set];
+    store->alive = S.alive;
+    store->tracks = S.tracks;
+    store->quality = S.quality;
+    store->out_tracks = a.tracks;
+    store->out_quality = a.quality;
+    store->out_count = a.count;
+    store->n = S.upper;
+    store->nvert = a.nvert;
+    store->max_vert = kMaxVert;
+    *out = store;
+    return ICELK_OK;
+}
+
+int archive_launched(Ctx* c, const LKArchive* carried, hipEvent_t ev)
+{
+    if (!carried) return ICELK_OK;
+    Ctx::SegBuf& S = c->sb[c->arch.set];
+    c->arch.pending = false;
+    c->archives_carried++;
+    if (!ev) {
+        HIPCHK(c, hipEventRecord(S.used_own, c->stream));
+        ev = S.used_own;
+    }
+    S.used = ev;
+    return ICELK_OK;
+}
+
 int flush_deferred(Ctx* c)
 {
     if (!c->defer.pending) return ICELK_OK;
     Ctx::Deferred& d = c->defer;
     d.pending = false;
-    int rc;
+    LKArchive arch;
+    const LKArchive* carry = nullptr;
+    int rc = archive_for_launch(c, d.P, d.job.n, d.job.B.stamps || d.job.B.iters, &arch, &carry);
+    if (rc) return rc;
     {
         ProfScope p(c, K_LK_FB);
-        rc = launch_lk(c->stream, d.job.I, d.job.J, d.job.B, d.job.n, d.P, true);
+        rc = launch_lk(c->stream, d.job.I, d.job.J, d.job.B, d.job.n, d.P, true, carry);
     }
     if (rc) FAIL(c, rc, "unsupported window size");
     rc = check_launch(c, "lk_fb");
@@ -123,7 +180,7 @@
     rc = record_launch(c, &ev);
     if (rc) return rc;
     seg_launched(c, ev, d.set, d.slot_prev, d.slot_next);
-    return ICELK_OK;
+    return archive_launched(c, carry, ev);
 }
 
 int flush_deferred_slot(Ctx* c, int slot)
@@ -183,6 +240,8 @@
             return ICELK_OK;
         }
         bool paired = false;
+        LKArchive arch;
+        const LKArchive* carry = nullptr;
         if (c->defer.pending) {
             Ctx::Deferred& d = c->defer;
             if (!diag && same_lk_params(d.P, P)) {
@@ -193,14 +252,18 @@
                     other.B.stamps = job.B.stamps = c->d_stamps;
                     hipMemsetAsync(c->d_stamps, 0, 3 * c->stamps_cap * 8, c->stream);
                 }
+                rc = archive_for_launch(c, P, std::min(other.n, job.n), other.B.stamps != nullptr, &arch, &carry);
+                if (rc) return rc;
                 {
                     ProfScope p(c, K_LK_FB_PAIR);
-                    paired = launch_lk_pair(c->stream, other, job, P);
+                    paired = launch_lk_pair(c->stream, other, job, P, carry);
                 }
                 if (paired) {
                     d.pending = false;
                     rc = check_launch(c, "lk_fb_pair");
                     if (rc) return rc;
+                } else {
+                    carry = nullptr;
                 }
             }
             if (!paired) {
@@ -219,9 +282,11 @@
                 B.stamps = c->d_stamps;
                 hipMemsetAsync(c->d_stamps, 0, 3 * c->stamps_cap * 8, c->stream);
             }
+            rc = archive_for_launch(c, P, job.n, B.stamps || B.iters, &arch, &carry);
+            if (rc) return rc;
             {
                 ProfScope p(c, K_LK_FB);
-                rc = launch_lk(c->stream, job.I, job.J, B, job.n, P, true);
+                rc = launch_lk(c->stream, job.I, job.J, B, job.n, P, true, carry);
             }
             if (rc) FAIL(c, rc, "unsupported window size");
             rc = check_launch(c, "lk_fb");
@@ -232,6 +297,8 @@
         if (rc) return rc;
         if (paired) seg_launched(c, ev, c->defer.set, c->defer.slot_prev, c->defer.slot_next);
         seg_launched(c, ev, c->sb_cur, slot_prev, slot_next);
+        rc = archive_launched(c, carry, ev);
+        if (rc) return rc;
     } else if (c->defer.pending && !defer) {
         rc = flush_deferred(c);
         if (rc) return rc;
@@ -271,7 +338,9 @@
     Ctx::SegBuf& nb = c->sb[(c->sb_cur + 1) % kSegSets];
     bool tables_written = false, dev_done = false;
     DetectJob job;
-    int rc = detect_finish(c, max_corners, c->max_pts, &n, &nb, &tables_written, &dev_done, &job);
+    int rc = archive_flush_set(c, (c->sb_cur + 1) % kSegSets);
+    if (rc) return rc;
+    rc = detect_finish(c, max_corners, c->max_pts, &n, &nb, &tables_written, &dev_done, &job);
     if (rc) return rc;
     if (!dev_done) {
         const hipStream_t ds = c->tail_stream;
@@ -344,6 +413,7 @@
     if (!h) return ICELK_EARG;
     Ctx* c = C(h);
     HIPCHK(c, hipSetDevice(c->device));
+    if (int rca = archive_flush(c)) return rca;
     HIPCHK(c, hipStreamSynchronize(c->eig_stream));
     HIPCHK(c, hipStreamSynchronize(c->det_stream));
     HIPCHK(c, hipStreamSynchronize(c->tail_stream));
@@ -428,12 +498,21 @@
     return ICELK_OK;
 }
 
+int icelk_seg_archive_stats(icelk_t* h, long long* out)
+{
+    if (!h || !out) return ICELK_EARG;
+    out[0] = C(h)->archives_carried;
+    out[1] = C(h)->archives_standalone;
+    return ICELK_OK;
+}
+
 int icelk_seg_flush(icelk_t* h)
 {
     if (!h) return ICELK_EARG;
     Ctx* c = C(h);
     HIPCHK(c, hipSetDevice(c->device));
-    return flush_deferred(c);
+    int rc = flush_deferred(c);
+    return rc ? rc : archive_flush(c);
 }
 
 static int seg_pick(Ctx* c, bool closed, int* set)
@@ -445,6 +524,7 @@
         int rc = flush_deferred(c);
         if (rc) return rc;
     }
+    if (int rc = archive_flush_set(c, *set)) return rc;
     return closed ? ICELK_OK : seg_wait(c);
 }
 
@@ -535,12 +615,26 @@
     if (cap_rows < S.upper) FAIL(c, ICELK_ECAP, "archive rows < tracks of the segment");
     const int nv = S.vert;
     if (out_vertices) *out_vertices = nv;
+    rc = archive_flush(c);
+    if (rc) return rc;
+    float* const out_quality = dev_quality ? reinterpret_cast<float*>(dev_quality) : c->d_out_quality;
+    if (closed && S.upper > 0) {
+        Ctx::ArchivePending& a = c->arch;
+        a.pending = true;
+        a.set = set;
+        a.tracks = reinterpret_cast<float*>(dev_tracks);
+        a.quality = out_quality;
+        a.count = reinterpret_cast<int*>(dev_count);
+        a.nvert = nv;
+        return ICELK_OK;
+    }
     launch_seg_gather(c->stream, S.alive, S.upper, S.tracks, S.quality, nv, kMaxVert, reinterpret_cast<float*>(dev_tracks),
-                      dev_quality ? reinterpret_cast<float*>(dev_quality) : c->d_out_quality, reinterpret_cast<int*>(dev_count));
+                      out_quality, reinterpret_cast<int*>(dev_count));
     rc = check_launch(c, "seg_archive");
     if (rc) return rc;
     HIPCHK(c, hipEventRecord(S.used_own, c->stream));
     S.used = S.used_own;
+    c->archives_standalone++;
     return ICELK_OK;
 }
 
diff --git a/iceberg_tracking_code_amd/csrc/icelk_ctx.h b/iceberg_tracking_code_amd/csrc/icelk_ctx.h
--- a/iceberg_tracking_code_amd/csrc/icelk_ctx.h
+++ b/iceberg_tracking_code_amd/csrc/icelk_ctx.h
@@ -170,6 +170,14 @@
     unsigned long long* d_tracked = nullptr;
     unsigned long long* h_seg = nullptr;
     float *d_out_tracks = nullptr, *d_out_quality = nullptr;
+    struct ArchivePending {
+        bool pending = false;
+        int set = 0;
+        float *tracks = nullptr, *quality = nullptr;
+        int* count = nullptr;
+        int nvert = 0;
+    } arch;
+    long long archives_carried = 0, archives_standalone = 0;
 
     struct Post {
         double* d_proj = nullptr;
@@ -357,6 +365,10 @@
 int detect_counts_arrived(Ctx* c, bool* arrived);
 int flush_deferred(Ctx* c);
 int flush_deferred_slot(Ctx* c, int slot);
+int archive_flush(Ctx* c);
+int archive_flush_set(Ctx* c, int set);
+int archive_for_launch(Ctx* c, const LKParams& P, int n, bool diag, LKArchive* store, const LKArchive** out);
+int archive_launched(Ctx* c, const LKArchive* carried, hipEvent_t ev);
 int check_projection_args(Ctx* c, const icelk_camera_t* cam, const icelk_utm_filter_t* filt);
 int project_core(Ctx* c, const float* d_tracks_in, int n, int nv, const icelk_camera_t* cam, const icelk_utm_filter_t* filt,
                  int host_pitch, double* x, double* y, double* u, double* v, double* speed, uint8_t* keep);
diff --git a/iceberg_tracking_code_amd/csrc/icelk_internal.h b/iceberg_tracking_code_amd/csrc/icelk_internal.h
--- a/iceberg_tracking_code_amd/csrc/icelk_internal.h
+++ b/iceberg_tracking_code_amd/csrc/icelk_internal.h
@@ -169,10 +169,19 @@
     LKBuffers B;
     int n;
 };
+struct LKArchive {
+    const uint8_t* alive;
+    const float* tracks;
+    const float* quality;
+    float* out_tracks;
+    float* out_quality;
+    int* out_count;
+    int n, nvert, max_vert;
+};
 size_t lk_lds_bytes(const LKParams& P);
 int launch_lk(hipStream_t s, const Pyramid& I, const Pyramid& J, const LKBuffers& B, int n, const LKParams& P,
-              bool fb);
-bool launch_lk_pair(hipStream_t s, const LKJob& a, const LKJob& b, const LKParams& P);
+              bool fb, const LKArchive* arch = nullptr);
+bool launch_lk_pair(hipStream_t s, const LKJob& a, const LKJob& b, const LKParams& P, const LKArchive* arch = nullptr);
 
 struct DetectScratch {
     float* eig;
diff --git a/iceberg_tracking_code_amd/csrc/k_lk.hip b/iceberg_tracking_code_amd/csrc/k_lk.hip
--- a/iceberg_tracking_code_amd/csrc/k_lk.hip
+++ b/iceberg_tracking_code_amd/csrc/k_lk.hip
@@ -3,7 +3,7 @@
 namespace icelk {
 
 bool launch_lk_fast(hipStream_t s, const Pyramid& I, const Pyramid& J, const LKBuffers& B, int n, const LKParams& P,
-                    bool fb);
+                    bool fb, const LKArchive* arch);
 bool launch_lk_multi(hipStream_t s, const Pyramid& I, const Pyramid& J, const LKBuffers& B, int n, const LKParams& P,
                      bool fb);
 
@@ -342,13 +342,13 @@
 }
 
 int launch_lk(hipStream_t s, const Pyramid& I, const Pyramid& J, const LKBuffers& B, int n, const LKParams& P,
-              bool fb)
+              bool fb, const LKArchive* arch)
 {
     if (n <= 0) return ICELK_OK;
     const bool generic = (P.flags & ICELK_FLAG_GENERIC_KERNEL) != 0;
     if ((P.flags & ICELK_FLAG_MULTI_PER_WAVE) && !generic && !P.sum_mode && launch_lk_multi(s, I, J, B, n, P, fb))
         return ICELK_OK;
-    if (!generic && launch_lk_fast(s, I, J, B, n, P, fb)) return ICELK_OK;
+    if (!generic && launch_lk_fast(s, I, J, B, n, P, fb, arch)) return ICELK_OK;
     const int npx = P.win_w * P.win_h;
     const int ppl = (npx + 63) / 64;
     const size_t lds = lk_lds_bytes(P);
diff --git a/iceberg_tracking_code_amd/csrc/k_lk_fast.hip b/iceberg_tracking_code_amd/csrc/k_lk_fast.hip
--- a/iceberg_tracking_code_amd/csrc/k_lk_fast.hip
+++ b/iceberg_tracking_code_amd/csrc/k_lk_fast.hip
@@ -1,4 +1,5 @@
 #include "lk_fast_tiles.h"
+#include "seg_gather.h"
 
 namespace icelk {
 
@@ -450,6 +451,8 @@
 struct LKJobs {
     LKJob job[2];
     int g0, g1;
+    int ga;
+    LKArchive arch;
 };
 
 template <int WW, int WH, bool FB, bool SM = false>
@@ -461,7 +464,13 @@
     uint4* const tlds = lds_q + kTileQ;
     __shared__ float fs_[SM ? 3 * WW * WH : 1];
     float* const fsum = SM ? fs_ : nullptr;
-    int which = 0, b = blockIdx.x;
+    if ((int)blockIdx.x < JJ.ga) {
+        const LKArchive& A = JJ.arch;
+        segg::gather_wave_tile(A.alive, A.n, A.tracks, A.quality, A.nvert, A.max_vert, A.out_tracks, A.out_quality, A.out_count,
+                               blockIdx.x, threadIdx.x);
+        return;
+    }
+    int which = 0, b = blockIdx.x - JJ.ga;
     if (JJ.g1 > 0) {
         const int G = b >> 3, m = (JJ.g0 < JJ.g1 ? JJ.g0 : JJ.g1) >> 3;
         const int mb = m & ~31;
@@ -539,14 +548,16 @@
 int grid_of(const LKBuffers& B, int n) { return B.order ? (n + 15) & ~7 : (n + 7) & ~7; }
 
 template <int WW, int WH>
-void launch_fast(hipStream_t s, const LKJob& a, const LKJob* b, const LKParams& P, bool fb)
+void launch_fast(hipStream_t s, const LKJob& a, const LKJob* b, const LKParams& P, bool fb, const LKArchive* arch)
 {
     LKJobs JJ;
     JJ.job[0] = a;
     JJ.job[1] = b ? *b : a;
     JJ.g0 = grid_of(a.B, a.n);
     JJ.g1 = b ? grid_of(b->B, b->n) : 0;
-    const int grid = JJ.g0 + JJ.g1;
+    JJ.ga = arch ? ((arch->n + segg::kWaveTile - 1) / segg::kWaveTile + 7) & ~7 : 0;
+    JJ.arch = arch ? *arch : LKArchive{};
+    const int grid = JJ.ga + JJ.g0 + JJ.g1;
     if (P.sum_mode) {
         if (fb) hipLaunchKernelGGL((k_lk_fast_sums<WW, WH, true>), dim3(grid), dim3(64), 0, s, JJ, P);
         else hipLaunchKernelGGL((k_lk_fast_sums<WW, WH, false>), dim3(grid), dim3(64), 0, s, JJ, P);
@@ -561,13 +572,13 @@
     }
 }
 
-bool dispatch_fast(hipStream_t s, const LKJob& a, const LKJob* b, const LKParams& P, bool fb)
+bool dispatch_fast(hipStream_t s, const LKJob& a, const LKJob* b, const LKParams& P, bool fb, const LKArchive* arch)
 {
     if (P.flags & ICELK_FLAG_INITIAL_FLOW) return false;
-    if (P.win_w == 21 && P.win_h == 21) launch_fast<21, 21>(s, a, b, P, fb);
-    else if (P.win_w == 31 && P.win_h == 31) launch_fast<31, 31>(s, a, b, P, fb);
-    else if (P.win_w == 35 && P.win_h == 35) launch_fast<35, 35>(s, a, b, P, fb);
-    else if (P.win_w == 15 && P.win_h == 15) launch_fast<15, 15>(s, a, b, P, fb);
+    if (P.win_w == 21 && P.win_h == 21) launch_fast<21, 21>(s, a, b, P, fb, arch);
+    else if (P.win_w == 31 && P.win_h == 31) launch_fast<31, 31>(s, a, b, P, fb, arch);
+    else if (P.win_w == 35 && P.win_h == 35) launch_fast<35, 35>(s, a, b, P, fb, arch);
+    else if (P.win_w == 15 && P.win_h == 15) launch_fast<15, 15>(s, a, b, P, fb, arch);
     else return false;
     return true;
 }
@@ -590,21 +601,21 @@
 }
 
 bool launch_lk_fast(hipStream_t s, const Pyramid& I, const Pyramid& J, const LKBuffers& B, int n, const LKParams& P,
-                    bool fb)
+                    bool fb, const LKArchive* arch)
 {
     LKJob a;
     a.I = I;
     a.J = J;
     a.B = B;
     a.n = n;
-    return dispatch_fast(s, a, nullptr, P, fb);
-}
-
-bool launch_lk_pair(hipStream_t s, const LKJob& a, const LKJob& b, const LKParams& P)
+    return dispatch_fast(s, a, nullptr, P, fb, arch);
+}
+
+bool launch_lk_pair(hipStream_t s, const LKJob& a, const LKJob& b, const LKParams& P, const LKArchive* arch)
 {
     if (P.flags & (ICELK_FLAG_GENERIC_KERNEL | ICELK_FLAG_MULTI_PER_WAVE)) return false;
     if (a.n <= 0 || b.n <= 0) return false;
-    return dispatch_fast(s, a, &b, P, true);
-}
-
-}
+    return dispatch_fast(s, a, &b, P, true, arch);
+}
+
+}
diff --git a/iceberg_tracking_code_amd/csrc/k_tracks.hip b/iceberg_tracking_code_amd/csrc/k_tracks.hip
--- a/iceberg_tracking_code_amd/csrc/k_tracks.hip
+++ b/iceberg_tracking_code_amd/csrc/k_tracks.hip
@@ -1,4 +1,5 @@
 #include "lk_common.h"
+#include "seg_gather.h"
 
 namespace icelk {
 
@@ -97,11 +98,7 @@
     __shared__ int wave_before[NW];
     const int tid = threadIdx.x, lane = tid & 63, wave = tid >> 6;
     const int base = blockIdx.x * kGatherTile;
-    int mine = 0;
-    const uint32_t* a32 = reinterpret_cast<const uint32_t*>(alive);
-    for (int i = tid; i < (base >> 2); i += kGatherTile) mine += __builtin_popcount(a32[i] & 0x01010101u);
-#pragma unroll
-    for (int d = 32; d > 0; d >>= 1) mine += __shfl_xor(mine, d, 64);
+    const int mine = segg::alive_before(alive, base, tid, kGatherTile);
     const int i = base + tid;
     const bool keep = i < n && alive[i];
     const unsigned long long m = __ballot(keep);
@@ -119,17 +116,8 @@
         tile_total += t;
     }
     if (keep) {
-        const int j = before + wbase + __popcll(m & ((1ull << lane) - 1ull));
-        const float2* src = reinterpret_cast<const float2*>(tracks) + (size_t)i * max_vert;
-        if ((reinterpret_cast<uintptr_t>(out_tracks) & 7u) == 0) {
-            float2* dst = reinterpret_cast<float2*>(out_tracks) + (size_t)j * nvert;
-            for (int v = 0; v < nvert; v++) dst[v] = src[v];
-        } else {
-            float* dst = out_tracks + (size_t)j * nvert * 2;
-            for (int v = 0; v < nvert; v++) { const float2 p = src[v]; dst[2 * v] = p.x; dst[2 * v + 1] = p.y; }
-        }
-        for (int v = 0; v + 1 < nvert; v++)
-            out_quality[(size_t)j * (nvert - 1) + v] = quality[(size_t)i * (max_vert - 1) + v];
+        segg::copy_row(tracks, quality, i, before + wbase + __popcll(m & ((1ull << lane) - 1ull)), nvert, max_vert,
+                       out_tracks, out_quality);
     }
     if (out_count && tid == 0 && base + kGatherTile >= n) *out_count = before + tile_total;
 }
diff --git a/iceberg_tracking_code_amd/csrc/seg_gather.h b/iceberg_tracking_code_amd/csrc/seg_gather.h
--- /dev/null
+++ b/iceberg_tracking_code_amd/csrc/seg_gather.h
@@ -0,0 +1,53 @@
+#pragma once
+#include <hip/hip_runtime.h>
+#include <stdint.h>
+
+namespace icelk {
+namespace segg {
+
+__device__ __forceinline__ int alive_before(const uint8_t* __restrict__ alive, int base, int tid, int nthr)
+{
+    const uint32_t* a32 = reinterpret_cast<const uint32_t*>(alive);
+    int mine = 0;
+    for (int i = tid; i < (base >> 2); i += nthr) mine += __builtin_popcount(a32[i] & 0x01010101u);
+#pragma unroll
+    for (int d = 32; d > 0; d >>= 1) mine += __shfl_xor(mine, d, 64);
+    return mine;
+}
+
+__device__ __forceinline__ void copy_row(const float* __restrict__ tracks, const float* __restrict__ quality, int i, int j,
+                                         int nvert, int max_vert, float* __restrict__ out_tracks,
+                                         float* __restrict__ out_quality)
+{
+    const float2* src = reinterpret_cast<const float2*>(tracks) + (size_t)i * max_vert;
+    if ((reinterpret_cast<uintptr_t>(out_tracks) & 7u) == 0) {
+        float2* dst = reinterpret_cast<float2*>(out_tracks) + (size_t)j * nvert;
+        for (int v = 0; v < nvert; v++) dst[v] = src[v];
+    } else {
+        float* dst = out_tracks + (size_t)j * nvert * 2;
+        for (int v = 0; v < nvert; v++) { const float2 p = src[v]; dst[2 * v] = p.x; dst[2 * v + 1] = p.y; }
+    }
+    for (int v = 0; v + 1 < nvert; v++)
+        out_quality[(size_t)j * (nvert - 1) + v] = quality[(size_t)i * (max_vert - 1) + v];
+}
+
+constexpr int kWaveTile = 64;
+
+__device__ __forceinline__ void gather_wave_tile(const uint8_t* __restrict__ alive, int n, const float* __restrict__ tracks,
+                                                 const float* __restrict__ quality, int nvert, int max_vert,
+                                                 float* __restrict__ out_tracks, float* __restrict__ out_quality,
+                                                 int* __restrict__ out_count, int tile, int lane)
+{
+    const int base = tile * kWaveTile;
+    if (base >= n) return;
+    const int before = alive_before(alive, base, lane, kWaveTile);
+    const int i = base + lane;
+    const bool keep = i < n && alive[i];
+    const unsigned long long m = __ballot(keep);
+    if (keep)
+        copy_row(tracks, quality, i, before + __popcll(m & ((1ull << lane) - 1ull)), nvert, max_vert, out_tracks, out_quality);
+    if (out_count && lane == 0 && base + kWaveTile >= n) *out_count = before + __popcll(m);
+}
+
+}
+}
diff --git a/include/icelk.h b/include/icelk.h
--- a/include/icelk.h
+++ b/include/icelk.h
@@ -101,6 +101,7 @@
 int icelk_seg_template_stats(icelk_t* h, long long* out);
 int icelk_seg_template_info(icelk_t* h, long long* bytes_per_table, long long* rows, int* state);
 int icelk_seg_tail_stats(icelk_t* h, long long* out);
+int icelk_seg_archive_stats(icelk_t* h, long long* out);
 int icelk_seg_read_closed(icelk_t* h, float* tracks, float* quality, int cap, int max_vertices, int* out_n,
                           int* out_vertices);
 int icelk_seg_archive_closed(icelk_t* h, void* dev_tracks, void* dev_quality, void* dev_count, int cap_rows,
```

New measurement: 7452. -1.9%, worse.
